# linyicheng1/keypoint_bench

Hardware: AMD Instinct MI355X
Metric: image-pairs/sec (extract+NMS+BF-match, 640x480, top_k=1000) (higher is better)
Workload: dtype f32

## Files before the change

include/kpb.h:

```cpp
#ifndef KPB_H
#define KPB_H

#include <stddef.h>
#include <stdint.h>

#ifdef __cplusplus
extern "C" {
#endif

#define KPB_VERSION 1

#define KPB_OK 0
#define KPB_E_INVALID (-1)
#define KPB_E_HIP (-2)
#define KPB_E_NOMEM (-3)
#define KPB_E_NEGATIVE (-4)
#define KPB_E_NOT_CONVERGED (-5)
#define KPB_E_WEIGHTS (-6)
#define KPB_E_UNSUPPORTED (-7)

#define KPB_MAX_NMS_DIST 16
#define KPB_MAX_TOPK 8192

typedef struct kpb_ctx kpb_ctx;
typedef struct kpb_net kpb_net;

typedef struct kpb_detect_params {
    int32_t nms_dist;
    float threshold;
    int32_t border_dist;
    int32_t top_k;
    float min_score;
} kpb_detect_params;

typedef struct kpb_match_params {
    double max_distance;
    int32_t cross_check;
} kpb_match_params;

int kpb_version(void);
const char* kpb_last_error(const kpb_ctx* ctx);

int kpb_ctx_create(int device, void* stream, kpb_ctx** out);
int kpb_ctx_set_stream(kpb_ctx* ctx, void* stream);
void kpb_ctx_destroy(kpb_ctx* ctx);
int kpb_sync(kpb_ctx* ctx);

#define KPB_OPT_COVIS_STORE_BYTES 1
int kpb_ctx_set_option(kpb_ctx* ctx, int option, int64_t value);

int kpb_prof_enable(kpb_ctx* ctx, int on);
int kpb_prof_report(kpb_ctx* ctx, char* buf, size_t cap);

int kpb_fast_nms(kpb_ctx* ctx, const float* score_dev, int batch, int H, int W, int nms_dist,
                 float* out_map_dev);

int kpb_detect(kpb_ctx* ctx, const float* score_dev, int batch, int H, int W,
               const kpb_detect_params* params, float* out_kps_dev, int32_t* out_idx_dev,
               int32_t* out_n_dev, int sync);
int kpb_detect_check(kpb_ctx* ctx);
int kpb_detect_counts(kpb_ctx* ctx, int32_t* out_n_host, int batch);

int kpb_sample(kpb_ctx* ctx, const float* desc_dev, int batch, int C, int Hd, int Wd, int64_t sb,
               int64_t sc, int64_t sh, int64_t sw, const float* pts_dev, int pts_cols, int max_n,
               const int32_t* n_dev, float* out_dev);

int kpb_match(kpb_ctx* ctx, const float* d0_dev, const float* d1_dev, int batch, int C, int max_n,
              int max_m, const int32_t* n_dev, const int32_t* m_dev, const kpb_match_params* params,
              int32_t* out_pairs_dev, double* out_dist_dev, int32_t* out_k_dev);

int kpb_match_counts(kpb_ctx* ctx, int32_t* out_k_host, int batch);

int kpb_gather_rows(kpb_ctx* ctx, const float* src_dev, int batch, int src_rows, int cols,
                    const int32_t* idx_dev, int idx_rows, int idx_stride, int idx_col,
                    const int32_t* k_dev, float* out_dev);

int kpb_warp_homography(kpb_ctx* ctx, const float* kps_dev, int batch, int max_n, int stride,
                        const int32_t* n_dev, const float* hmat_dev, const int32_t* wh_dev,
                        float* out_kps0_dev, float* out_kps01_dev, int32_t* out_ids_dev,
                        int32_t* out_n_dev);

int kpb_warp_se3(kpb_ctx* ctx, const float* kps_dev, int n, int stride, const float* depth0_dev, int H0, int W0,
                 const float* depth1_dev, int H1, int W1, const float* cam_dev, float* out_kps0_dev,
                 float* out_kps01_dev, int32_t* out_ids_dev, int32_t* out_ids_out_dev, int32_t* out_counts_dev);

int kpb_val_keypoints(kpb_ctx* ctx, const float* k0_dev, const float* k01_dev, const float* k1_dev,
                      const float* k10_dev, int batch, int max_m, int max_n, const int32_t* m_dev,
                      const int32_t* n_dev, const float* scale_dev, float th, int32_t* out_pairs_dev,
                      float* out_dist_dev, int cap, float* out_errors_dev, int32_t* out_counts_dev);

typedef struct kpb_lk_params {
    float distance;
    int32_t win_size, levels, iterations;
} kpb_lk_params;
int kpb_lk_track(kpb_ctx* ctx, const float* img1_dev, const float* img2_dev, int C, int H, int W,
                 const float* pts1_dev, const float* pts2_dev, int pts_stride, const float* unit_dev,
                 int n, const kpb_lk_params* params, float* out_pts_dev, float* out_err_dev);

int kpb_epipolar_error(kpb_ctx* ctx, const float* kps0_dev, int cols0, const float* kps1_dev, int cols1, int batch,
                       int max_k, const int32_t* k_dev, const float* fmat_dev, int W, int H, int mode1, float th,
                       float* out_err_dev, float* out_stats_dev);

typedef struct kpb_ransac_params {
    double threshold;
    double confidence;
    int32_t max_iters;
    int32_t refine;
} kpb_ransac_params;
int kpb_find_homography(kpb_ctx* ctx, const float* m0_dev, int cols0, const float* m1_dev, int cols1, int batch, int max_k,
                        const int32_t* k_dev, const float* scale_dev, const uint32_t* seed_dev, uint32_t seed,
                        const kpb_ransac_params* params, double* out_h_dev, uint8_t* out_mask_dev, int32_t* out_info_dev);

int kpb_find_essential(kpb_ctx* ctx, const float* m0_dev, int cols0, const float* m1_dev, int cols1, int batch, int max_k,
                       const int32_t* k_dev, const float* scale_dev, const double* cam_dev, int cam_f32, const double* thr_dev,
                       const uint32_t* seed_dev, uint32_t seed, double prob, int max_iters, double* out_e_dev,
                       uint8_t* out_mask_dev, int32_t* out_info_dev, double* out_pts_dev);
int kpb_recover_pose(kpb_ctx* ctx, const double* e_dev, const double* pts_dev, const uint8_t* mask_dev, int batch, int max_k,
                     const int32_t* k_dev, const int32_t* info_dev, double dist, double* out_rt_dev, uint8_t* out_mask_dev,
                     int32_t* out_good_dev);

int kpb_find_fundamental(kpb_ctx* ctx, const float* m0_dev, int cols0, const float* m1_dev, int cols1, int batch, int max_k,
                         const int32_t* k_dev, const float* scale_dev, const uint32_t* seed_dev, uint32_t seed,
                         const kpb_ransac_params* params, double* out_f_dev, uint8_t* out_mask_dev, int32_t* out_info_dev);

int kpb_preprocess(kpb_ctx* ctx, const uint8_t* src_dev, int batch, int Hs, int Ws, int swap_rb,
                   int Hd, int Wd, float* out_dev);

#define KPB_ARCH_ALIKE 1
#define KPB_ARCH_SUPERPOINT 2
#define KPB_ARCH_XFEAT 3
#define KPB_ARCH_DISK 4
#define KPB_ARCH_R2D2 6
int kpb_net_create(kpb_ctx* ctx, int arch, const void* blob, size_t len, kpb_net** out);
void kpb_net_destroy(kpb_net* net);
int kpb_net_desc_dim(const kpb_net* net);
int kpb_net_desc_div(const kpb_net* net);
int kpb_net_forward(kpb_net* net, const float* img_dev, int batch, int H, int W,
                    float* score_out_dev, float* desc_out_dev);
int kpb_net_desc_at(kpb_net* net, const float* pts_dev, int pts_cols, int max_n,
                    const int32_t* n_dev, float* out_dev);

#define KPB_ARCH_LIGHTGLUE 5
typedef struct kpb_lg kpb_lg;
typedef struct kpb_lg_params {
    float depth_confidence;
    float width_confidence;
    float filter_threshold;
    int32_t prune_min_kpts;
} kpb_lg_params;
int kpb_lg_create(kpb_ctx* ctx, const void* blob, size_t len, float desc_scale, kpb_lg** out);
void kpb_lg_destroy(kpb_lg* lg);
int kpb_lg_input_dim(const kpb_lg* lg);
int kpb_lg_set_attention(kpb_lg* lg, int mode);
int kpb_lg_match(kpb_lg* lg, const float* pts0_dev, const float* pts1_dev, const int32_t* n0_dev, const int32_t* n1_dev,
                 int batch, int max_k, const float* desc0_dev, const float* desc1_dev, int C, int Hd, int Wd,
                 int64_t sb, int64_t sc, int64_t sh, int64_t sw, int img_w, int img_h, const kpb_lg_params* params,
                 int32_t* out_pairs_dev, float* out_scores_dev, int32_t* out_k_dev, int32_t* out_stop_dev);

#ifdef __cplusplus
}
#endif
#endif
```

keypoint_bench_amd/_lib.py:

```python
import ctypes
import os

_HERE = os.path.dirname(os.path.abspath(__file__))
SO_PATH = os.environ.get("KPB_LIB_PATH") or os.path.join(_HERE, "libkpb.so")

c_int, c_float, c_double, c_void_p, c_int64, c_size_t = (ctypes.c_int, ctypes.c_float, ctypes.c_double,
                                                       ctypes.c_void_p, ctypes.c_int64, ctypes.c_size_t)


class DetectParams(ctypes.Structure):
    _fields_ = [("nms_dist", ctypes.c_int32), ("threshold", c_float), ("border_dist", ctypes.c_int32),
                ("top_k", ctypes.c_int32), ("min_score", c_float)]


class LgParams(ctypes.Structure):
    _fields_ = [("depth_confidence", c_float), ("width_confidence", c_float), ("filter_threshold", c_float),
                ("prune_min_kpts", ctypes.c_int32)]


class LkParams(ctypes.Structure):
    _fields_ = [("distance", ctypes.c_float), ("win_size", ctypes.c_int32), ("levels", ctypes.c_int32), ("iterations", ctypes.c_int32)]


class RansacParams(ctypes.Structure):
    _fields_ = [("threshold", ctypes.c_double), ("confidence", ctypes.c_double), ("max_iters", ctypes.c_int32), ("refine", ctypes.c_int32)]


class MatchParams(ctypes.Structure):
    _fields_ = [("max_distance", c_double), ("cross_check", ctypes.c_int32)]


SIGNATURES = {
    "kpb_version": (c_int, []),
    "kpb_last_error": (ctypes.c_char_p, [c_void_p]),
    "kpb_ctx_create": (c_int, [c_int, c_void_p, ctypes.POINTER(c_void_p)]),
    "kpb_ctx_set_stream": (c_int, [c_void_p, c_void_p]),
    "kpb_ctx_destroy": (None, [c_void_p]),
    "kpb_sync": (c_int, [c_void_p]),
    "kpb_ctx_set_option": (c_int, [c_void_p, c_int, c_int64]),
    "kpb_prof_enable": (c_int, [c_void_p, c_int]),
    "kpb_prof_report": (c_int, [c_void_p, ctypes.c_char_p, c_size_t]),
    "kpb_fast_nms": (c_int, [c_void_p, c_void_p, c_int, c_int, c_int, c_int, c_void_p]),
    "kpb_detect": (c_int, [c_void_p, c_void_p, c_int, c_int, c_int, ctypes.POINTER(DetectParams), c_void_p, c_void_p,
                           c_void_p, c_int]),
    "kpb_detect_check": (c_int, [c_void_p]),
    "kpb_detect_counts": (c_int, [c_void_p, c_void_p, c_int]),
    "kpb_match_counts": (c_int, [c_void_p, c_void_p, c_int]),
    "kpb_sample": (c_int, [c_void_p, c_void_p, c_int, c_int, c_int, c_int, c_int64, c_int64, c_int64, c_int64,
                           c_void_p, c_int, c_int, c_void_p, c_void_p]),
    "kpb_match": (c_int, [c_void_p, c_void_p, c_void_p, c_int, c_int, c_int, c_int, c_void_p, c_void_p,
                          ctypes.POINTER(MatchParams), c_void_p, c_void_p, c_void_p]),
    "kpb_gather_rows": (c_int, [c_void_p, c_void_p, c_int, c_int, c_int, c_void_p, c_int, c_int, c_int, c_void_p,
                                c_void_p]),
    "kpb_warp_homography": (c_int, [c_void_p, c_void_p, c_int, c_int, c_int, c_void_p, c_void_p, c_void_p, c_void_p,
                                    c_void_p, c_void_p, c_void_p]),
    "kpb_warp_se3": (c_int, [c_void_p, c_void_p, c_int, c_int, c_void_p, c_int, c_int, c_void_p, c_int, c_int, c_void_p, c_void_p,
                             c_void_p, c_void_p, c_void_p, c_void_p]),
    "kpb_val_keypoints": (c_int, [c_void_p, c_void_p, c_void_p, c_void_p, c_void_p, c_int, c_int, c_int, c_void_p, c_void_p,
                                  c_void_p, c_float, c_void_p, c_void_p, c_int, c_void_p, c_void_p]),
    "kpb_lk_track": (c_int, [c_void_p, c_void_p, c_void_p, c_int, c_int, c_int, c_void_p, c_void_p, c_int, c_void_p, c_int,
                             c_void_p, c_void_p, c_void_p]),
    "kpb_epipolar_error": (c_int, [c_void_p, c_void_p, c_int, c_void_p, c_int, c_int, c_int, c_void_p, c_void_p, c_int, c_int, c_int,
                                   c_float, c_void_p, c_void_p]),
    "kpb_find_homography": (c_int, [c_void_p, c_void_p, c_int, c_void_p, c_int, c_int, c_int, c_void_p, c_void_p, c_void_p, ctypes.c_uint32,
                                    ctypes.POINTER(RansacParams), c_void_p, c_void_p, c_void_p]),
    "kpb_find_fundamental": (c_int, [c_void_p, c_void_p, c_int, c_void_p, c_int, c_int, c_int, c_void_p, c_void_p, c_void_p, ctypes.c_uint32,
                                     ctypes.POINTER(RansacParams), c_void_p, c_void_p, c_void_p]),
    "kpb_find_essential": (c_int, [c_void_p, c_void_p, c_int, c_void_p, c_int, c_int, c_int, c_void_p, c_void_p, c_void_p, c_int, c_void_p, c_void_p,
                                   ctypes.c_uint32, c_double, c_int, c_void_p, c_void_p, c_void_p, c_void_p]),
    "kpb_recover_pose": (c_int, [c_void_p, c_void_p, c_void_p, c_void_p, c_int, c_int, c_void_p, c_void_p, c_double, c_void_p, c_void_p,
                                 c_void_p]),
    "kpb_preprocess": (c_int, [c_void_p, c_void_p, c_int, c_int, c_int, c_int, c_int, c_int, c_void_p]),
    "kpb_net_create": (c_int, [c_void_p, c_int, c_void_p, c_size_t, ctypes.POINTER(c_void_p)]),
    "kpb_net_destroy": (None, [c_void_p]),
    "kpb_net_desc_dim": (c_int, [c_void_p]),
    "kpb_net_desc_div": (c_int, [c_void_p]),
    "kpb_net_forward": (c_int, [c_void_p, c_void_p, c_int, c_int, c_int, c_void_p, c_void_p]),
    "kpb_net_desc_at": (c_int, [c_void_p, c_void_p, c_int, c_int, c_void_p, c_void_p]),
    "kpb_lg_create": (c_int, [c_void_p, c_void_p, c_size_t, c_float, ctypes.POINTER(c_void_p)]),
    "kpb_lg_destroy": (None, [c_void_p]),
    "kpb_lg_input_dim": (c_int, [c_void_p]),
    "kpb_lg_set_attention": (c_int, [c_void_p, c_int]),
    "kpb_lg_match": (c_int, [c_void_p, c_void_p, c_void_p, c_void_p, c_void_p, c_int, c_int, c_void_p, c_void_p, c_int, c_int, c_int,
                             c_int64, c_int64, c_int64, c_int64, c_int, c_int, ctypes.POINTER(LgParams), c_void_p, c_void_p,
                             c_void_p, c_void_p]),
}

_lib = None


class KpbError(RuntimeError):
    def __init__(self, code, msg):
        super().__init__("libkpb error %d: %s" % (code, msg))
        self.code = code


def load():
    global _lib
    if _lib is None:
        import torch
        if not os.path.exists(SO_PATH):
            raise RuntimeError("%s is missing: run `python -m keypoint_bench_amd.build` (hipcc, gfx950). "
                               "keypoint_bench_amd has no CPU fallback." % SO_PATH)
        L = ctypes.CDLL(SO_PATH)
        for name, (res, args) in SIGNATURES.items():
            fn = getattr(L, name)
            fn.restype = res
            fn.argtypes = args
        _lib = L
    return _lib


class Context:
    _instances = {}

    def __init__(self, device_index: int):
        import torch
        if not torch.cuda.is_available():
            raise RuntimeError("keypoint_bench_amd needs an MI355X (gfx950) GPU; none is visible and there is no "
                               "CPU fallback")
        self.lib = load()
        self.device_index = device_index
        stream = torch.cuda.current_stream(device_index).cuda_stream
        self.stream = stream
        h = c_void_p()
        rc = self.lib.kpb_ctx_create(device_index, c_void_p(stream), ctypes.byref(h))
        if rc != 0:
            raise KpbError(rc, self.lib.kpb_last_error(None).decode())
        self.handle = h

    @classmethod
    def get(cls, device):
        import torch
        idx = device.index if isinstance(device, torch.device) else int(device)
        if idx is None:
            idx = torch.cuda.current_device()
        if idx not in cls._instances:
            cls._instances[idx] = cls(idx)
        inst = cls._instances[idx]
        stream = torch.cuda.current_stream(idx).cuda_stream
        if stream != inst.stream:
            inst.check(inst.lib.kpb_ctx_set_stream(inst.handle, c_void_p(stream)))
            inst.stream = stream
        return inst

    def check(self, rc):
        if rc != 0:
            raise KpbError(rc, self.lib.kpb_last_error(self.handle).decode())

    def sync(self):
        self.check(self.lib.kpb_sync(self.handle))

    OPT_COVIS_STORE_BYTES = 1

    def set_option(self, option: int, value: int):
        self.check(self.lib.kpb_ctx_set_option(self.handle, int(option), int(value)))

    def prof_enable(self, on: bool):
        self.check(self.lib.kpb_prof_enable(self.handle, 1 if on else 0))

    def prof_report(self):
        buf = ctypes.create_string_buffer(1 << 16)
        self.check(self.lib.kpb_prof_report(self.handle, buf, len(buf)))
        out = {}
        for line in buf.value.decode().splitlines():
            name, calls, ms = line.split()
            out[name] = (int(calls), float(ms))
        return out


def ptr(t):
    return c_void_p(t.data_ptr()) if t is not None else c_void_p(0)
```

keypoint_bench_amd/csrc/alike.hip:

```cpp
#include "conv_mfma.h"

namespace {

typedef _Float16 h8v __attribute__((ext_vector_type(8)));
typedef _Float16 h2v __attribute__((ext_vector_type(2)));
typedef float f32x4v __attribute__((ext_vector_type(4)));

__device__ __forceinline__ float relu(float v);

__device__ __forceinline__ void split4(const float4 v, uint2& hi, uint2& lo) { cm_split4(v, hi, lo); }

__device__ __forceinline__ void amax_commit(float lane_max, float* slots, int slot, int lane)
{
    const float m = cm_wave_max(lane_max);
    if (lane == 0) slots[slot] = m;
}

__global__ __launch_bounds__(256) void amax_reduce(const float* slots, int n, unsigned* out)
{
    __shared__ float s[4];
    const int b = blockIdx.x, tid = threadIdx.x;
    float m = 0.0f;
    for (int i = tid; i < n; i += 256) {
        const float v = slots[(size_t)b * n + i];
        m = fmaxf(m, v < INFINITY ? v : 0.0f);
    }
    m = cm_wave_max(m);
    if ((tid & 63) == 0) s[tid >> 6] = m;
    __syncthreads();
    if (tid == 0) out[b] = __float_as_uint(fmaxf(fmaxf(s[0], s[1]), fmaxf(s[2], s[3])));
}

constexpr int B1_TH = 32, B1_TW = 32;

struct Block1Args {
    const float* img;
    float* x1;
    float* p1;
    const float* w1;
    const float* b1;
    const float* w2;
    const float* b2;
    int H, W;
};

__global__ __launch_bounds__(256) void alike_block1(Block1Args a)
{
    constexpr int IH = B1_TH + 4, IW = B1_TW + 4, MH = B1_TH + 2, MW = B1_TW + 2;
    __shared__ float in[3][IH][IW];
    __shared__ __attribute__((aligned(16))) float4 mid[2][MH][MW];
    const int tid = threadIdx.x, b = blockIdx.z;
    const int ty0 = blockIdx.y * B1_TH, tx0 = blockIdx.x * B1_TW;
    const size_t P = (size_t)a.H * a.W;
    const float* img = a.img + (size_t)b * 3 * P;
    {
        constexpr int N = 3 * IH * IW, PER = (N + 255) / 256;
        float buf[PER];
#pragma unroll
        for (int k = 0; k < PER; ++k) {
            const int i = tid + k * 256;
            const int c = i / (IH * IW), rem = i - c * IH * IW;
            const int y = rem / IW, x = rem - y * IW;
            const int gy = ty0 - 2 + y, gx = tx0 - 2 + x;
            buf[k] = 0.0f;
            if (i < N && gy >= 0 && gy < a.H && gx >= 0 && gx < a.W) buf[k] = img[c * P + (size_t)gy * a.W + gx];
        }
#pragma unroll
        for (int k = 0; k < PER; ++k) {
            const int i = tid + k * 256;
            if (i < N) (&in[0][0][0])[i] = buf[k];
        }
    }
    __syncthreads();
    for (int it = tid; it < MH * (MW / 2); it += 256) {
        const int my = it / (MW / 2), mx = (it - my * (MW / 2)) * 2;
        float acc[2][8];
#pragma unroll
        for (int q = 0; q < 2; ++q)
#pragma unroll
            for (int j = 0; j < 8; ++j) acc[q][j] = a.b1[j];
#pragma unroll 1
        for (int cky = 0; cky < 9; ++cky) {
                const int c = cky / 3, ky = cky - 3 * c;
                float v[4];
#pragma unroll
                for (int k = 0; k < 4; ++k) v[k] = in[c][my + ky][mx + k];
#pragma unroll
                for (int kx = 0; kx < 3; ++kx)
#pragma unroll
                    for (int j = 0; j < 8; ++j) {
                        const float w = a.w1[((c * 3 + ky) * 3 + kx) * 8 + j];
                        acc[0][j] = fmaf(v[kx], w, acc[0][j]);
                        acc[1][j] = fmaf(v[kx + 1], w, acc[1][j]);
                    }
            }
        const int gy = ty0 - 1 + my;
#pragma unroll
        for (int q = 0; q < 2; ++q) {
            const int gx = tx0 - 1 + mx + q;
            const bool inside = gy >= 0 && gy < a.H && gx >= 0 && gx < a.W;
            float4 lo = make_float4(0.f, 0.f, 0.f, 0.f), hi = lo;
            if (inside) {
                lo = make_float4(relu(acc[q][0]), relu(acc[q][1]), relu(acc[q][2]), relu(acc[q][3]));
                hi = make_float4(relu(acc[q][4]), relu(acc[q][5]), relu(acc[q][6]), relu(acc[q][7]));
            }
            mid[0][my][mx + q] = lo;
            mid[1][my][mx + q] = hi;
        }
    }
    __syncthreads();
    const int oy = tid >> 5, ox = tid & 31;
    float acc[4][8];
#pragma unroll
    for (int q = 0; q < 4; ++q)
#pragma unroll
        for (int j = 0; j < 8; ++j) acc[q][j] = a.b2[j];
#pragma unroll 1
    for (int tap = 0; tap < 9; ++tap) {
        const int ky = tap / 3, kx = tap - 3 * ky;
        float v[4][8];
#pragma unroll
        for (int q = 0; q < 4; ++q) {
            const float4 lo = mid[0][oy + 8 * q + ky][ox + kx];
            const float4 hi = mid[1][oy + 8 * q + ky][ox + kx];
            v[q][0] = lo.x; v[q][1] = lo.y; v[q][2] = lo.z; v[q][3] = lo.w;
            v[q][4] = hi.x; v[q][5] = hi.y; v[q][6] = hi.z; v[q][7] = hi.w;
        }
#pragma unroll
        for (int c = 0; c < 8; ++c)
#pragma unroll
            for (int j = 0; j < 8; ++j) {
                const float w = a.w2[(tap * 8 + c) * 8 + j];
#pragma unroll
                for (int q = 0; q < 4; ++q) acc[q][j] = fmaf(v[q][c], w, acc[q][j]);
            }
    }
    __syncthreads();
    float* stage = reinterpret_cast<float*>(&mid[0][0][0]);
#pragma unroll
    for (int q = 0; q < 4; ++q) {
        *reinterpret_cast<float4*>(stage + ((oy + 8 * q) * B1_TW + ox) * 8) = make_float4(relu(acc[q][0]), relu(acc[q][1]), relu(acc[q][2]), relu(acc[q][3]));
        *reinterpret_cast<float4*>(stage + ((oy + 8 * q) * B1_TW + ox) * 8 + 4) = make_float4(relu(acc[q][4]), relu(acc[q][5]), relu(acc[q][6]), relu(acc[q][7]));
    }
    __syncthreads();
#pragma unroll
    for (int k = 0; k < B1_TH * B1_TW * 8 / 4 / 256; ++k) {
        const int i = tid + k * 256;
        const int ry = i >> 6, rx4 = i & 63;
        const int gy = ty0 + ry, gx = tx0 + (rx4 >> 1);
        if (gy < a.H && gx < a.W)
            *reinterpret_cast<float4*>(a.x1 + ((size_t)b * P + (size_t)gy * a.W + tx0) * 8 + rx4 * 4) =
                *reinterpret_cast<const float4*>(stage + i * 4);
    }
    {
        const int H2 = a.H / 2, W2 = a.W / 2;
#pragma unroll
        for (int k = 0; k < (B1_TH / 2) * (B1_TW / 2) * 2 / 256; ++k) {
            const int i = tid + k * 256;
            const int q = i & 1, px = (i >> 1) & (B1_TW / 2 - 1), py = i >> 5;
            const float* s0 = stage + ((2 * py) * B1_TW + 2 * px) * 8 + 4 * q;
            const float4 v00 = *reinterpret_cast<const float4*>(s0), v01 = *reinterpret_cast<const float4*>(s0 + 8);
            const float4 v10 = *reinterpret_cast<const float4*>(s0 + B1_TW * 8), v11 = *reinterpret_cast<const float4*>(s0 + B1_TW * 8 + 8);
            const int gy = ty0 / 2 + py, gx = tx0 / 2 + px;
            if (gy < H2 && gx < W2)
                *reinterpret_cast<float4*>(a.p1 + (((size_t)b * H2 + gy) * W2 + gx) * 8 + 4 * q) =
                    make_float4(fmaxf(fmaxf(v00.x, v01.x), fmaxf(v10.x, v11.x)), fmaxf(fmaxf(v00.y, v01.y), fmaxf(v10.y, v11.y)),
                                fmaxf(fmaxf(v00.z, v01.z), fmaxf(v10.z, v11.z)), fmaxf(fmaxf(v00.w, v01.w), fmaxf(v10.w, v11.w)));
        }
    }
}

struct Block1HArgs {
    Block1Args b;
    const uint4* w1pk;
    const uint4* w2pk;
    float inv_ws1, inv_ws2;
    float l1_c1, bmax_c1;
    float* wmax_x1;
    int xcd_map;
};

constexpr int B1H_TH = 16;

__global__ __launch_bounds__(256) void alike_block1_h(Block1HArgs ha)
{
    const Block1Args& a = ha.b;
    constexpr int TH = B1H_TH, IH = TH + 4, IW = B1_TW + 4, MH = TH + 2, MW = B1_TW + 2, HW = MW / 2;
    constexpr int PLANE = MH * HW, REGION = 2 * PLANE, NIN = IH * IW;
    __shared__ __attribute__((aligned(16))) uint2 inh[2 * NIN + 2];
    __shared__ __attribute__((aligned(16))) uint4 mid[2 * REGION];
    const kpb_tile3 tile = kpb_xcd_tile(ha.xcd_map);
    const int tid = threadIdx.x, lane = tid & 63, wv = tid >> 6, b = tile.z;
    const int ty0 = tile.y * TH, tx0 = tile.x * B1_TW;
    const size_t P = (size_t)a.H * a.W;
    const float* img = a.img + (size_t)b * 3 * P;
    h8v c1hi[2], c1lo[2], bhi[3], blo[3];
#pragma unroll
    for (int kb = 0; kb < 2; ++kb) {
        c1hi[kb] = __builtin_bit_cast(h8v, ha.w1pk[(kb * 2 + 0) * 64 + lane]);
        c1lo[kb] = __builtin_bit_cast(h8v, ha.w1pk[(kb * 2 + 1) * 64 + lane]);
    }
#pragma unroll
    for (int kb = 0; kb < 3; ++kb) {
        bhi[kb] = __builtin_bit_cast(h8v, ha.w2pk[(kb * 2 + 0) * 64 + lane]);
        blo[kb] = __builtin_bit_cast(h8v, ha.w2pk[(kb * 2 + 1) * 64 + lane]);
    }
    const float4 bias1 = *reinterpret_cast<const float4*>(a.b1 + 4 * ((lane >> 4) & 1));
    const float4 bias2 = *reinterpret_cast<const float4*>(a.b2 + 4 * ((lane >> 4) & 1));
    __shared__ __attribute__((aligned(16))) float s_amax[4];
    int e_img;
    {
        constexpr int PER = (NIN + 255) / 256;
        float buf[PER][3];
        float am = 0.0f;
#pragma unroll
        for (int k = 0; k < PER; ++k) {
            const int i = tid + k * 256;
            const int y = i / IW, x = i - y * IW;
            const int gy = ty0 - 2 + y, gx = tx0 - 2 + x;
            const bool ok = i < NIN && gy >= 0 && gy < a.H && gx >= 0 && gx < a.W;
#pragma unroll
            for (int c = 0; c < 3; ++c) buf[k][c] = ok ? img[c * P + (size_t)gy * a.W + gx] : 0.0f;
            am = kpb_pmax(kpb_pmax(am, fabsf(buf[k][0])), kpb_pmax(fabsf(buf[k][1]), fabsf(buf[k][2])));
        }
        am = cm_wave_max(am);
        if (lane == 0) s_amax[wv] = am;
        __syncthreads();
        float4 q = *reinterpret_cast<const float4*>(s_amax);
        if (!(q.x < INFINITY && q.y < INFINITY && q.z < INFINITY && q.w < INFINITY)) {
            float fm = 0.0f;
#pragma unroll
            for (int k = 0; k < PER; ++k)
#pragma unroll
                for (int c = 0; c < 3; ++c) { const float v = fabsf(buf[k][c]); fm = fmaxf(fm, v < INFINITY ? v : 0.0f); }
            fm = cm_wave_max(fm);
            __syncthreads();
            if (lane == 0) s_amax[wv] = fm;
            __syncthreads();
            q = *reinterpret_cast<const float4*>(s_amax);
        }
        e_img = cm_exp_of(fmaxf(fmaxf(q.x, q.y), fmaxf(q.z, q.w)));
        const float sc = cm_scale_of(e_img);
#pragma unroll
        for (int k = 0; k < PER; ++k) {
            const int i = tid + k * 256;
            uint2 hi, lo;
            split4(make_float4(buf[k][0] * sc, buf[k][1] * sc, buf[k][2] * sc, 0.0f), hi, lo);
            if (i < NIN) { inh[i] = hi; inh[NIN + i] = lo; }
        }
        if (tid < 2) inh[2 * NIN + tid] = make_uint2(0u, 0u);
    }
    __syncthreads();
    const int e_mid = cm_exp_of(fmaf(__uint_as_float((unsigned)(e_img - 126 + 127) << 23), ha.l1_c1, ha.bmax_c1));
    const float un1 = ha.inv_ws1 * cm_unscale_of(e_img), sc_mid = cm_scale_of(e_mid), un2 = ha.inv_ws2 * cm_unscale_of(e_mid);
    const int pr = lane & 15, g = lane >> 4;
    const int sN = g >> 1, c0 = 4 * (g & 1);
    {
        const uint4* inq = reinterpret_cast<const uint4*>(inh);
        uint2* midh = reinterpret_cast<uint2*>(mid);
        static_assert((MH + 2) % 4 == 0 && MH % 4 == 2, "alike_block1_h: waves 2 and 3 take the two extra groups");
        {
            const int gxl = tx0 - 1 + 2 * pr + sN;
            const bool xin = gxl >= 0 && gxl < a.W;
            const float unm = xin ? un1 * sc_mid : 0.0f;
            const float4 bm = xin ? make_float4(bias1.x * sc_mid, bias1.y * sc_mid, bias1.z * sc_mid, bias1.w * sc_mid) : make_float4(0.f, 0.f, 0.f, 0.f);
            const bool has1 = g < 2;
            int at0 = (wv + (g >> 1)) * (IW / 2) + pr + (g & 1);
            int at1 = has1 ? (wv + 2) * (IW / 2) + pr + g : NIN;
            const int st1 = has1 ? 4 * (IW / 2) : 0, lo1 = has1 ? NIN / 2 : 0;
            int h8 = ((sN * PLANE + wv * HW + pr) << 1) + (g & 1);
#pragma unroll 1
            for (int y = wv; y < MH; y += 4, at0 += 4 * (IW / 2), at1 += st1, h8 += 8 * HW) {
                f32x4v acc = {0.f, 0.f, 0.f, 0.f};
                const h8v i0h = __builtin_bit_cast(h8v, inq[at0]), i0l = __builtin_bit_cast(h8v, inq[at0 + NIN / 2]);
                const h8v i1h = __builtin_bit_cast(h8v, inq[at1]), i1l = __builtin_bit_cast(h8v, inq[at1 + lo1]);
                acc = __builtin_amdgcn_mfma_f32_16x16x32_f16(c1hi[0], i0l, acc, 0, 0, 0);
                acc = __builtin_amdgcn_mfma_f32_16x16x32_f16(c1lo[0], i0h, acc, 0, 0, 0);
                acc = __builtin_amdgcn_mfma_f32_16x16x32_f16(c1hi[0], i0h, acc, 0, 0, 0);
                acc = __builtin_amdgcn_mfma_f32_16x16x32_f16(c1hi[1], i1l, acc, 0, 0, 0);
                acc = __builtin_amdgcn_mfma_f32_16x16x32_f16(c1lo[1], i1h, acc, 0, 0, 0);
                acc = __builtin_amdgcn_mfma_f32_16x16x32_f16(c1hi[1], i1h, acc, 0, 0, 0);
                const bool yin = (unsigned)(ty0 - 1 + y) < (unsigned)a.H;
                float4 v = make_float4(0.f, 0.f, 0.f, 0.f);
                if (yin) v = make_float4(relu(fmaf(acc[0], unm, bm.x)), relu(fmaf(acc[1], unm, bm.y)), relu(fmaf(acc[2], unm, bm.z)), relu(fmaf(acc[3], unm, bm.w)));
                uint2 hi, lo;
                split4(v, hi, lo);
                midh[h8] = hi;
                midh[h8 + 2 * REGION] = lo;
            }
        }
        if (wv >= 2) {
            const int gi = MH + wv - 2;
            const bool extra = true;
            const int y = extra ? 16 * (gi - MH) + pr : gi, pc = extra ? 16 : pr;
            const int my = min(y, MH - 1);
            f32x4v acc = {0.f, 0.f, 0.f, 0.f};
#pragma unroll
            for (int kb = 0; kb < 2; ++kb) {
                const int piece = 4 * kb + g;
                const int at = piece < 6 ? ((my + (piece >> 1)) * IW + 2 * pc + 2 * (piece & 1)) >> 1 : NIN;
                const h8v ihi = __builtin_bit_cast(h8v, inq[at]);
                const h8v ilo = __builtin_bit_cast(h8v, inq[piece < 6 ? at + NIN / 2 : NIN]);
                acc = __builtin_amdgcn_mfma_f32_16x16x32_f16(c1hi[kb], ilo, acc, 0, 0, 0);
                acc = __builtin_amdgcn_mfma_f32_16x16x32_f16(c1lo[kb], ihi, acc, 0, 0, 0);
                acc = __builtin_amdgcn_mfma_f32_16x16x32_f16(c1hi[kb], ihi, acc, 0, 0, 0);
            }
            const int gy = ty0 - 1 + y, gx = tx0 - 1 + 2 * pc + sN;
            const bool inside = gy >= 0 && gy < a.H && gx >= 0 && gx < a.W;
            float4 v = make_float4(relu(fmaf(acc[0], un1, bias1.x)) * sc_mid, relu(fmaf(acc[1], un1, bias1.y)) * sc_mid,
                                   relu(fmaf(acc[2], un1, bias1.z)) * sc_mid, relu(fmaf(acc[3], un1, bias1.w)) * sc_mid);
            if (!inside) v = make_float4(0.f, 0.f, 0.f, 0.f);
            uint2 hi, lo;
            split4(v, hi, lo);
            if (y < MH) {
                const int h8 = ((sN * PLANE + y * HW + pc) << 1) + (g & 1);
                midh[h8] = hi;
                midh[h8 + 2 * REGION] = lo;
            }
        }
    }
    __syncthreads();
    const int abase = (g & 1) * PLANE + pr + (g >> 1);
    const int H2 = a.H / 2, W2 = a.W / 2;
    float4 keep = make_float4(0.f, 0.f, 0.f, 0.f);
    float xmax = 0.0f;
    const int gx = tx0 + 2 * pr + sN;
#pragma unroll 1
    for (int rr = 0; rr < TH / 4; ++rr) {
        const int row = (TH / 4) * wv + rr;
        f32x4v acc = {0.f, 0.f, 0.f, 0.f};
#pragma unroll
        for (int kb = 0; kb < 3; ++kb) {
            const int at = abase + (row + kb) * HW;
            const h8v ihi = __builtin_bit_cast(h8v, mid[at]);
            const h8v ilo = __builtin_bit_cast(h8v, mid[REGION + at]);
            acc = __builtin_amdgcn_mfma_f32_16x16x32_f16(bhi[kb], ilo, acc, 0, 0, 0);
            acc = __builtin_amdgcn_mfma_f32_16x16x32_f16(blo[kb], ihi, acc, 0, 0, 0);
            acc = __builtin_amdgcn_mfma_f32_16x16x32_f16(bhi[kb], ihi, acc, 0, 0, 0);
        }
        const int gy = ty0 + row;
        const float4 v = make_float4(relu(fmaf(acc[0], un2, bias2.x)), relu(fmaf(acc[1], un2, bias2.y)), relu(fmaf(acc[2], un2, bias2.z)), relu(fmaf(acc[3], un2, bias2.w)));
        if (gy < a.H && gx < a.W) {
            {
                typedef float f4v __attribute__((ext_vector_type(4)));
                __builtin_nontemporal_store((f4v){v.x, v.y, v.z, v.w}, reinterpret_cast<f4v*>(a.x1 + ((size_t)b * P + (size_t)gy * a.W + gx) * 8 + c0));
            }
            xmax = kpb_pmax(kpb_pmax(xmax, kpb_pmax(v.x, v.y)), kpb_pmax(v.z, v.w));
        }
        if ((rr & 1) == 0) {
            keep = v;
        } else {
            float4 m = make_float4(kpb_pmax(keep.x, v.x), kpb_pmax(keep.y, v.y), kpb_pmax(keep.z, v.z), kpb_pmax(keep.w, v.w));
            m.x = kpb_pmax32(m.x); m.y = kpb_pmax32(m.y);
            m.z = kpb_pmax32(m.z); m.w = kpb_pmax32(m.w);
            const int py = gy >> 1, pxl = (tx0 >> 1) + pr;
            if (sN == 0 && py < H2 && pxl < W2) *reinterpret_cast<float4*>(a.p1 + (((size_t)b * H2 + py) * W2 + pxl) * 8 + c0) = m;
        }
    }
    amax_commit(xmax, ha.wmax_x1, ((b * gridDim.y + tile.y) * gridDim.x + tile.x) * 4 + wv, lane);
}

std::vector<float> pack_b1c1_pairs(const float* w, float scale)
{
    std::vector<uint16_t> hl((size_t)2 * 2 * 64 * 8, 0);
    for (int kb = 0; kb < 2; ++kb)
        for (int l = 0; l < 64; ++l)
            for (int j = 0; j < 8; ++j) {
                const int n = l & 15, g = l >> 4, s2 = n >> 3, co = n & 7, piece = 4 * kb + g;
                const int ky = piece >> 1, kx = 2 * (piece & 1) + (j >> 2) - s2, c = j & 3;
                const float v = (piece < 6 && c < 3 && kx >= 0 && kx <= 2) ? w[((size_t)co * 3 + c) * 9 + ky * 3 + kx] * scale : 0.0f;
                _Float16 hi = (_Float16)v;
                const _Float16 lo = (_Float16)(v - (float)hi);
                memcpy(&hl[(((size_t)kb * 2 + 0) * 64 + l) * 8 + j], &hi, 2);
                memcpy(&hl[(((size_t)kb * 2 + 1) * 64 + l) * 8 + j], &lo, 2);
            }
    std::vector<float> out(hl.size() / 2);
    memcpy(out.data(), hl.data(), hl.size() * 2);
    return out;
}

std::vector<float> pack_b1c2_pairs(const float* w, float scale)
{
    std::vector<uint16_t> hl((size_t)3 * 2 * 64 * 8, 0);
    for (int kb = 0; kb < 3; ++kb)
        for (int l = 0; l < 64; ++l)
            for (int j = 0; j < 8; ++j) {
                const int n = l & 15, g = l >> 4, s2 = n >> 3, co = n & 7, kx = g - s2;
                const float v = (kx >= 0 && kx <= 2) ? w[((size_t)co * 8 + j) * 9 + kb * 3 + kx] * scale : 0.0f;
                _Float16 hi = (_Float16)v;
                const _Float16 lo = (_Float16)(v - (float)hi);
                memcpy(&hl[(((size_t)kb * 2 + 0) * 64 + l) * 8 + j], &hi, 2);
                memcpy(&hl[(((size_t)kb * 2 + 1) * 64 + l) * 8 + j], &lo, 2);
            }
    std::vector<float> out(hl.size() / 2);
    memcpy(out.data(), hl.data(), hl.size() * 2);
    return out;
}

struct ConvArgs {
    const float* in;
    float* out;
    const float* w;
    const float* bias;
    const float* res_in;
    const float* ds_w;
    const float* ds_b;
    float* res_out;
    int H, W;
};

template <int CIN, int COUT, int POOL, bool RES, int CDS, int RPOOL, bool RELU, bool DSOUT = false, int TW = 32>
__global__ __launch_bounds__(256) void conv3x3_k(ConvArgs a)
{
    constexpr int G = COUT / 16, PG = 4 / G, RW = 64 / TW, TH = RW * PG, C4 = CIN / 4;
    constexpr int RP = TW == 16 ? 32 : TW + 2;
    constexpr int NPOS = (TH + 2) * RP, NPOSP = NPOS + ((4 - NPOS % 8) + 8) % 8;
    static_assert(COUT % 16 == 0 && (G == 1 || G == 2 || G == 4) && CIN % 4 == 0 && (TW == 16 || TW == 32), "channel config");
    __shared__ __attribute__((aligned(16))) float4 tile[C4 * NPOSP];
    const int tid = threadIdx.x, b = blockIdx.z;
    const int wv = __builtin_amdgcn_readfirstlane(tid >> 6), lane = tid & 63;
    const int cg = wv % G, pg = wv / G;
    const int ty0 = blockIdx.y * TH, tx0 = blockIdx.x * TW;
    const int Hi = a.H * POOL, Wi = a.W * POOL;
    const float* in = a.in + (size_t)b * Hi * Wi * CIN;

    for (int i = tid; i < (TH + 2) * (TW + 2) * C4; i += 256) {
        const int pos = i / C4, c4 = i - pos * C4;
        const int y = pos / (TW + 2), x = pos - y * (TW + 2);
        const int gy = ty0 - 1 + y, gx = tx0 - 1 + x;
        float4 v = make_float4(0.f, 0.f, 0.f, 0.f);
        if (gy >= 0 && gy < a.H && gx >= 0 && gx < a.W) {
            const float* p = in + ((size_t)(gy * POOL) * Wi + (size_t)gx * POOL) * CIN + c4 * 4;
            v = *reinterpret_cast<const float4*>(p);
#pragma unroll
            for (int dy = 0; dy < POOL; ++dy)
#pragma unroll
                for (int dx = 0; dx < POOL; ++dx) {
                    if (dy == 0 && dx == 0) continue;
                    const float4 q = *reinterpret_cast<const float4*>(p + ((size_t)dy * Wi + dx) * CIN);
                    v.x = fmaxf(v.x, q.x); v.y = fmaxf(v.y, q.y); v.z = fmaxf(v.z, q.z); v.w = fmaxf(v.w, q.w);
                }
        }
        tile[c4 * NPOSP + y * RP + x] = v;
    }
    __syncthreads();

    const int row = pg * RW + lane / TW, col = lane % TW;
    const int gy = ty0 + row, gx = tx0 + col;
    float acc[16];
    const float* bias = a.bias + cg * 16;
#pragma unroll
    for (int j = 0; j < 16; ++j) acc[j] = bias[j];
#pragma unroll
    for (int ky = 0; ky < 3; ++ky)
#pragma unroll
        for (int kx = 0; kx < 3; ++kx) {
            const float4* t = &tile[(row + ky) * RP + col + kx];
            const float* w = a.w + (size_t)((ky * 3 + kx) * CIN) * COUT + cg * 16;
#pragma unroll 2
            for (int c4 = 0; c4 < C4; ++c4) {
                const float4 v4 = t[c4 * NPOSP];
                const float v[4] = {v4.x, v4.y, v4.z, v4.w};
#pragma unroll
                for (int c = 0; c < 4; ++c)
#pragma unroll
                    for (int j = 0; j < 16; ++j) acc[j] = fmaf(v[c], w[(c4 * 4 + c) * COUT + j], acc[j]);
            }
        }
    if (gy >= a.H || gx >= a.W) return;
    if (DSOUT) {
        float ds[16];
        const float* db = a.ds_b + cg * 16;
#pragma unroll
        for (int j = 0; j < 16; ++j) ds[j] = db[j];
        const float4* t = &tile[(row + 1) * RP + col + 1];
        const float* dw = a.ds_w + cg * 16;
#pragma unroll 2
        for (int c4 = 0; c4 < C4; ++c4) {
            const float4 v4 = t[c4 * NPOSP];
            const float v[4] = {v4.x, v4.y, v4.z, v4.w};
#pragma unroll
            for (int c = 0; c < 4; ++c)
#pragma unroll
                for (int j = 0; j < 16; ++j) ds[j] = fmaf(v[c], dw[(c4 * 4 + c) * COUT + j], ds[j]);
        }
        float* ro = a.res_out + ((size_t)b * a.H * a.W + (size_t)gy * a.W + gx) * COUT + cg * 16;
#pragma unroll
        for (int q = 0; q < 4; ++q) *reinterpret_cast<float4*>(ro + 4 * q) = make_float4(ds[4 * q], ds[4 * q + 1], ds[4 * q + 2], ds[4 * q + 3]);
    }
    if (RES) {
        constexpr int D4 = CDS / 4;
        const int Hr = a.H * RPOOL, Wr = a.W * RPOOL;
        const float* p = a.res_in + ((size_t)b * Hr * Wr + (size_t)(gy * RPOOL) * Wr + (size_t)gx * RPOOL) * CDS;
        const float* dw = a.ds_w + cg * 16;
        const float* db = a.ds_b + cg * 16;
#pragma unroll
        for (int j = 0; j < 16; ++j) acc[j] += db[j];
        for (int c4 = 0; c4 < D4; ++c4) {
            float4 v4 = *reinterpret_cast<const float4*>(p + c4 * 4);
#pragma unroll
            for (int dy = 0; dy < RPOOL; ++dy)
#pragma unroll
                for (int dx = 0; dx < RPOOL; ++dx) {
                    if (dy == 0 && dx == 0) continue;
                    const float4 q = *reinterpret_cast<const float4*>(p + ((size_t)dy * Wr + dx) * CDS + c4 * 4);
                    v4.x = fmaxf(v4.x, q.x); v4.y = fmaxf(v4.y, q.y); v4.z = fmaxf(v4.z, q.z); v4.w = fmaxf(v4.w, q.w);
                }
            const float v[4] = {v4.x, v4.y, v4.z, v4.w};
#pragma unroll
            for (int c = 0; c < 4; ++c)
#pragma unroll
                for (int j = 0; j < 16; ++j) acc[j] = fmaf(v[c], dw[(c4 * 4 + c) * COUT + j], acc[j]);
        }
    }
    float* o = a.out + ((size_t)b * a.H * a.W + (size_t)gy * a.W + gx) * COUT + cg * 16;
#pragma unroll
    for (int q = 0; q < 4; ++q) {
        float4 v = make_float4(acc[4 * q], acc[4 * q + 1], acc[4 * q + 2], acc[4 * q + 3]);
        if (RELU) { v.x = relu(v.x); v.y = relu(v.y); v.z = relu(v.z); v.w = relu(v.w); }
        *reinterpret_cast<float4*>(o + 4 * q) = v;
    }
}

struct Block2Args {
    const float* p1;
    float* x2; float* a2; float* S2;
    float* p2;
    const uint4* w1pk;
    const uint4* w2pk;
    const uint4* wapk;
    const float* b1; const float* bsum; const float* wsg;
    int H, W;
    float inv_ws1, inv_ws2, inv_wsa, l1_c1, bmax_c1, l1_c2, l1_ds, bmax_sum;
    const unsigned* amax_x1;
    float* wmax_a2;
    int xcd_map;
};


__global__ __launch_bounds__(256, 4) void alike_block2(Block2Args a)
{
    constexpr int TH = 8, TW = 32, PH = TH + 4, PW = TW + 4, NP = PH * PW, MH = TH + 2, MW = TW + 2, NM = MH * MW;
    __shared__ __attribute__((aligned(16))) uint4 pin[2 * NP];
    __shared__ __attribute__((aligned(16))) uint4 mid[4 * NM];
    __shared__ __attribute__((aligned(16))) uint4 xs[4][2][2][16];
    __shared__ __attribute__((aligned(16))) uint4 zslot;
    const kpb_tile3 tile = kpb_xcd_tile(a.xcd_map);
    const int tid = threadIdx.x, lane = tid & 63, wv = tid >> 6, b = tile.z;
    const int ty0 = tile.y * TH, tx0 = tile.x * TW;
    const size_t P = (size_t)a.H * a.W;
    h8v w1h[3], w1l[3], w2h[5], w2l[5];
#pragma unroll
    for (int kb = 0; kb < 3; ++kb) { w1h[kb] = __builtin_bit_cast(h8v, a.w1pk[(kb * 2) * 64 + lane]); w1l[kb] = __builtin_bit_cast(h8v, a.w1pk[(kb * 2 + 1) * 64 + lane]); }
    const float4 b1v = *reinterpret_cast<const float4*>(a.b1 + 4 * (lane >> 4));
    const float4 bsum = *reinterpret_cast<const float4*>(a.bsum + 4 * (lane >> 4)), wsg = *reinterpret_cast<const float4*>(a.wsg + 4 * (lane >> 4));
    const float am_p = __uint_as_float(a.amax_x1[b]);
    const float bound1 = fmaf(am_p, a.l1_c1, a.bmax_c1);
    const int e1 = cm_exp_of(fmaxf(am_p, bound1));
    const int ex = cm_exp_of(fmaf(bound1, a.l1_c2, fmaf(am_p, a.l1_ds, a.bmax_sum)));
    const float sc1 = cm_scale_of(e1), un_c1s = a.inv_ws1, un_c2 = a.inv_ws2 * cm_unscale_of(e1);
    const bool edge = ty0 == 0 || tx0 == 0 || ty0 + TH >= a.H || tx0 + TW >= a.W;
    const float scx = cm_scale_of(ex), un_a = a.inv_wsa * cm_unscale_of(ex);
    {
        const float* in = a.p1 + (size_t)b * P * 8;
        constexpr int PER = (NP * 2 + 255) / 256;
        float4 ld[PER];
        unsigned okm = 0;
#pragma unroll
        for (int k = 0; k < PER; ++k) {
            const int i = min(tid + 256 * k, NP * 2 - 1);
            const int pos = i >> 1, q = i & 1;
            const int y = pos / PW, x = pos - y * PW;
            const int gy = ty0 - 2 + y, gx = tx0 - 2 + x;
            if (gy >= 0 && gy < a.H && gx >= 0 && gx < a.W) okm |= 1u << k;
            ld[k] = *reinterpret_cast<const float4*>(in + ((size_t)min(max(gy, 0), a.H - 1) * a.W + min(max(gx, 0), a.W - 1)) * 8 + 4 * q);
        }
#pragma unroll
        for (int k = 0; k < PER; ++k) {
            const int i = tid + 256 * k;
            const int pos = i >> 1, q = i & 1;
            float4 v = ((okm >> k) & 1u) ? ld[k] : make_float4(0.f, 0.f, 0.f, 0.f);
            v.x *= sc1; v.y *= sc1; v.z *= sc1; v.w *= sc1;
            uint2 hi, lo;
            split4(v, hi, lo);
            if (i < NP * 2) {
                uint2* d = reinterpret_cast<uint2*>(&pin[pos]) + q;
                d[0] = hi;
                d[2 * NP] = lo;
            }
        }
        if (tid == 0) zslot = make_uint4(0u, 0u, 0u, 0u);
    }
    __syncthreads();
    const int px = lane & 15, g = lane >> 4;
    const uint4* zp = &zslot;
    {
        float4 bias1 = b1v;
        bias1.x *= sc1; bias1.y *= sc1; bias1.z *= sc1; bias1.w *= sc1;
        uint2* midh = reinterpret_cast<uint2*>(mid);
        static_assert((2 * MH) % 4 == 0, "alike_block2: the regular conv1 groups split evenly over the four waves");
        {
            const int xl = 16 * (wv & 1) + px, y0 = wv >> 1;
            const int gxl = tx0 - 1 + xl;
            const bool xin = gxl >= 0 && gxl < a.W;
            const float unm = xin ? un_c1s : 0.0f;
            const float4 bm = xin ? bias1 : make_float4(0.f, 0.f, 0.f, 0.f);
            const bool has2 = 8 + g < 9;
            const uint4* q0 = &pin[(y0 + g / 3) * PW + xl + g % 3];
            const uint4* q1 = &pin[(y0 + (4 + g) / 3) * PW + xl + (4 + g) % 3];
            const uint4* q2 = has2 ? &pin[(y0 + 2) * PW + xl + 2] : zp;
            const int st2 = has2 ? 2 * PW : 0, lo2 = has2 ? NP : 0;
            int h8 = (((g >> 1) * NM + y0 * MW + xl) << 1) + (g & 1);
            constexpr int NIT = 2 * MH / 4;
            h8v i0h = __builtin_bit_cast(h8v, q0[0]), i0l = __builtin_bit_cast(h8v, q0[NP]);
            h8v i1h = __builtin_bit_cast(h8v, q1[0]), i1l = __builtin_bit_cast(h8v, q1[NP]);
            h8v i2h = __builtin_bit_cast(h8v, q2[0]), i2l = __builtin_bit_cast(h8v, q2[lo2]);
#pragma unroll 1
            for (int it = 0; it < NIT; ++it, h8 += 4 * MW) {
                f32x4v acc = {0.f, 0.f, 0.f, 0.f};
                __builtin_amdgcn_sched_barrier(0);
                acc = __builtin_amdgcn_mfma_f32_16x16x32_f16(w1h[0], i0l, acc, 0, 0, 0);
                acc = __builtin_amdgcn_mfma_f32_16x16x32_f16(w1l[0], i0h, acc, 0, 0, 0);
                acc = __builtin_amdgcn_mfma_f32_16x16x32_f16(w1h[0], i0h, acc, 0, 0, 0);
                acc = __builtin_amdgcn_mfma_f32_16x16x32_f16(w1h[1], i1l, acc, 0, 0, 0);
                acc = __builtin_amdgcn_mfma_f32_16x16x32_f16(w1l[1], i1h, acc, 0, 0, 0);
                acc = __builtin_amdgcn_mfma_f32_16x16x32_f16(w1h[1], i1h, acc, 0, 0, 0);
                acc = __builtin_amdgcn_mfma_f32_16x16x32_f16(w1h[2], i2l, acc, 0, 0, 0);
                acc = __builtin_amdgcn_mfma_f32_16x16x32_f16(w1l[2], i2h, acc, 0, 0, 0);
                acc = __builtin_amdgcn_mfma_f32_16x16x32_f16(w1h[2], i2h, acc, 0, 0, 0);
                __builtin_amdgcn_sched_barrier(0);
                if (it + 1 < NIT) {
                    q0 += 2 * PW; q1 += 2 * PW; q2 += st2;
                    i0h = __builtin_bit_cast(h8v, q0[0]); i0l = __builtin_bit_cast(h8v, q0[NP]);
                    i1h = __builtin_bit_cast(h8v, q1[0]); i1l = __builtin_bit_cast(h8v, q1[NP]);
                    i2h = __builtin_bit_cast(h8v, q2[0]); i2l = __builtin_bit_cast(h8v, q2[lo2]);
                }
                __builtin_amdgcn_sched_barrier(0);
                const bool yin = (unsigned)(ty0 - 1 + y0 + 2 * it) < (unsigned)a.H;
                float4 v = make_float4(0.f, 0.f, 0.f, 0.f);
                if (yin) v = make_float4(relu(fmaf(acc[0], unm, bm.x)), relu(fmaf(acc[1], unm, bm.y)), relu(fmaf(acc[2], unm, bm.z)), relu(fmaf(acc[3], unm, bm.w)));
                uint2 hi, lo;
                split4(v, hi, lo);
                midh[h8] = hi;
                midh[h8 + 4 * NM] = lo;
            }
        }
        if (wv < 2) {
            const int gi = 2 * MH + wv;
            const int k = 16 * (gi - 2 * MH) + px;
            const int y = k >> 1, x = 32 + (k & 1);
            const int my = min(y, MH - 1);
            f32x4v acc = {0.f, 0.f, 0.f, 0.f};
#pragma unroll
            for (int kb = 0; kb < 3; ++kb) {
                const int tap = 4 * kb + g;
                const bool has = tap < 9;
                const uint4* ph = has ? &pin[(my + tap / 3) * PW + x + tap % 3] : zp;
                const h8v ihi = __builtin_bit_cast(h8v, ph[0]);
                const h8v ilo = __builtin_bit_cast(h8v, has ? ph[NP] : zp[0]);
                acc = __builtin_amdgcn_mfma_f32_16x16x32_f16(w1h[kb], ilo, acc, 0, 0, 0);
                acc = __builtin_amdgcn_mfma_f32_16x16x32_f16(w1l[kb], ihi, acc, 0, 0, 0);
                acc = __builtin_amdgcn_mfma_f32_16x16x32_f16(w1h[kb], ihi, acc, 0, 0, 0);
            }
            const int gy = ty0 - 1 + y, gx = tx0 - 1 + x;
            const bool inside = gy >= 0 && gy < a.H && gx >= 0 && gx < a.W;
            float4 v = make_float4(relu(fmaf(acc[0], un_c1s, bias1.x)), relu(fmaf(acc[1], un_c1s, bias1.y)), relu(fmaf(acc[2], un_c1s, bias1.z)), relu(fmaf(acc[3], un_c1s, bias1.w)));
            if (edge && !inside) v = make_float4(0.f, 0.f, 0.f, 0.f);
            uint2 hi, lo;
            split4(v, hi, lo);
            if (y < MH) {
                const int h8 = (((g >> 1) * NM + y * MW + x) << 1) + (g & 1);
                midh[h8] = hi;
                midh[h8 + 4 * NM] = lo;
            }
        }
    }
    __builtin_amdgcn_sched_barrier(0);
#pragma unroll
    for (int kb = 0; kb < 5; ++kb) { w2h[kb] = __builtin_bit_cast(h8v, a.w2pk[(kb * 2) * 64 + lane]); w2l[kb] = __builtin_bit_cast(h8v, a.w2pk[(kb * 2 + 1) * 64 + lane]); }
    const h8v wah = __builtin_bit_cast(h8v, a.wapk[lane]), wal = __builtin_bit_cast(h8v, a.wapk[64 + lane]);
    __syncthreads();
    float* x2 = a.x2 + (size_t)b * P * 16;
    float* a2 = a.a2 + (size_t)b * P * 16;
    float* S2 = a.S2 + (size_t)b * P;
    uint2* xh = reinterpret_cast<uint2*>(&xs[wv][0][0][0]);
    float4 pm = make_float4(0.f, 0.f, 0.f, 0.f);
    float amx = 0.0f;
#pragma unroll 1
    for (int k4 = 0; k4 < 4; ++k4) {
        const int row = 4 * (wv >> 1) + k4, col0 = (wv & 1) * 16;
        const int mbase = row * MW + col0 + px;
        f32x4v acc = {0.f, 0.f, 0.f, 0.f};
        h8v ihi[5], ilo[5];
        auto fetch = [&](int kb) {
            const int kidx = 4 * kb + g;
            const uint4* ph;
            int lo_off;
            if (kidx < 18) { const int tap = kidx >> 1; ph = &mid[(kidx & 1) * NM + mbase + (tap / 3) * MW + tap % 3]; lo_off = 2 * NM; }
            else if (kidx == 18) { ph = &pin[(row + 2) * PW + col0 + px + 2]; lo_off = NP; }
            else { ph = zp; lo_off = 0; }
            ihi[kb] = __builtin_bit_cast(h8v, ph[0]);
            ilo[kb] = __builtin_bit_cast(h8v, ph[lo_off]);
        };
        auto mm = [&](int kb) {
            acc = __builtin_amdgcn_mfma_f32_16x16x32_f16(w2h[kb], ilo[kb], acc, 0, 0, 0);
            acc = __builtin_amdgcn_mfma_f32_16x16x32_f16(w2l[kb], ihi[kb], acc, 0, 0, 0);
            acc = __builtin_amdgcn_mfma_f32_16x16x32_f16(w2h[kb], ihi[kb], acc, 0, 0, 0);
        };
        fetch(0); fetch(1); fetch(2);
        __builtin_amdgcn_sched_barrier(0);
        mm(0); mm(1);
        __builtin_amdgcn_sched_barrier(0);
        fetch(3); fetch(4);
        __builtin_amdgcn_sched_barrier(0);
        mm(2);
        __builtin_amdgcn_sched_barrier(0);
        mm(3); mm(4);
        const int gy = ty0 + row, gx = tx0 + col0 + px;
        const bool ok = gy < a.H && gx < a.W;
        const float4 v = make_float4(relu(fmaf(acc[0], un_c2, bsum.x)), relu(fmaf(acc[1], un_c2, bsum.y)), relu(fmaf(acc[2], un_c2, bsum.z)), relu(fmaf(acc[3], un_c2, bsum.w)));
        if (ok && !a.p2) *reinterpret_cast<float4*>(x2 + ((size_t)gy * a.W + gx) * 16 + 4 * g) = v;
        pm = make_float4(kpb_pmax(pm.x, v.x), kpb_pmax(pm.y, v.y), kpb_pmax(pm.z, v.z), kpb_pmax(pm.w, v.w));
        {
            uint2 hi, lo;
            split4(make_float4(v.x * scx, v.y * scx, v.z * scx, v.w * scx), hi, lo);
            const int h8 = (((g >> 1) * 16 + px) << 1) + (g & 1);
            xh[h8] = hi;
            xh[h8 + 64] = lo;
        }
        f32x4v ag = {0.f, 0.f, 0.f, 0.f};
        {
            const uint4* ph = g < 2 ? &xs[wv][0][g][px] : zp;
            const h8v ihi = __builtin_bit_cast(h8v, ph[0]);
            const h8v ilo = __builtin_bit_cast(h8v, g < 2 ? ph[32] : zp[0]);
            ag = __builtin_amdgcn_mfma_f32_16x16x32_f16(wah, ilo, ag, 0, 0, 0);
            ag = __builtin_amdgcn_mfma_f32_16x16x32_f16(wal, ihi, ag, 0, 0, 0);
            ag = __builtin_amdgcn_mfma_f32_16x16x32_f16(wah, ihi, ag, 0, 0, 0);
        }
        const float4 av = make_float4(relu(ag[0] * un_a), relu(ag[1] * un_a), relu(ag[2] * un_a), relu(ag[3] * un_a));
        if (ok) {
            *reinterpret_cast<float4*>(a2 + ((size_t)gy * a.W + gx) * 16 + 4 * g) = av;
            amx = kpb_pmax(kpb_pmax(amx, kpb_pmax(av.x, av.y)), kpb_pmax(av.z, av.w));
        }
        float sg = fmaf(av.w, wsg.w, fmaf(av.z, wsg.z, fmaf(av.y, wsg.y, av.x * wsg.x)));
        sg = kpb_sum16(sg);
        sg = kpb_sum32(sg);
        if (g == 0 && ok) S2[(size_t)gy * a.W + gx] = sg;
    }
    if (a.p2) {
        pm.x = kpb_pmax(pm.x, kpb_xor1(pm.x)); pm.y = kpb_pmax(pm.y, kpb_xor1(pm.y));
        pm.z = kpb_pmax(pm.z, kpb_xor1(pm.z)); pm.w = kpb_pmax(pm.w, kpb_xor1(pm.w));
        pm.x = kpb_pmax(pm.x, kpb_xor2(pm.x)); pm.y = kpb_pmax(pm.y, kpb_xor2(pm.y));
        pm.z = kpb_pmax(pm.z, kpb_xor2(pm.z)); pm.w = kpb_pmax(pm.w, kpb_xor2(pm.w));
        const int gy = ty0 + 4 * (wv >> 1), gx = tx0 + (wv & 1) * 16 + px;
        if ((px & 3) == 0 && gy < a.H && gx < a.W)
            *reinterpret_cast<float4*>(a.p2 + (size_t)b * (P / 16) * 16 + ((size_t)(gy >> 2) * (a.W >> 2) + (gx >> 2)) * 16 + 4 * g) = pm;
    }
    amax_commit(amx, a.wmax_a2, ((b * gridDim.y + tile.y) * gridDim.x + tile.x) * 4 + wv, lane);
}

std::vector<float> pack_1x1_h16(const float* w, float scale)
{
    std::vector<uint16_t> hl((size_t)2 * 64 * 8, 0);
    for (int l = 0; l < 64; ++l)
        for (int j = 0; j < 8; ++j) {
            const int n = l & 15, g = l >> 4;
            const float v = g < 2 ? w[n * 16 + 8 * g + j] * scale : 0.0f;
            _Float16 hi = (_Float16)v;
            const _Float16 lo = (_Float16)(v - (float)hi);
            memcpy(&hl[((size_t)0 * 64 + l) * 8 + j], &hi, 2);
            memcpy(&hl[((size_t)1 * 64 + l) * 8 + j], &lo, 2);
        }
    std::vector<float> out(hl.size() / 2);
    memcpy(out.data(), hl.data(), hl.size() * 2);
    return out;
}

std::vector<float> pack_h16(const float* w, int CIN, const float* ds_w, float scale)
{
    const int OCT = CIN / 8, NK = 9 * OCT + (ds_w ? 1 : 0), KB = (NK + 3) / 4;
    std::vector<uint16_t> hl((size_t)KB * 2 * 64 * 8, 0);
    for (int kb = 0; kb < KB; ++kb)
        for (int l = 0; l < 64; ++l)
            for (int j = 0; j < 8; ++j) {
                const int n = l & 15, g = l >> 4, kidx = 4 * kb + g;
                float v = 0.0f;
                if (kidx < 9 * OCT) { const int tap = kidx / OCT, o = kidx - tap * OCT; v = w[((size_t)n * CIN + 8 * o + j) * 9 + tap]; }
                else if (ds_w && kidx == 9 * OCT) v = ds_w[n * 8 + j];
                v *= scale;
                _Float16 hi = (_Float16)v;
                const _Float16 lo = (_Float16)(v - (float)hi);
                memcpy(&hl[(((size_t)kb * 2 + 0) * 64 + l) * 8 + j], &hi, 2);
                memcpy(&hl[(((size_t)kb * 2 + 1) * 64 + l) * 8 + j], &lo, 2);
            }
    std::vector<float> out(hl.size() / 2);
    memcpy(out.data(), hl.data(), hl.size() * 2);
    return out;
}

constexpr int ESTRIDE = 68;

template <int CIN>
__device__ __forceinline__ void conv1x1_relu_body(const float* __restrict__ in, float* __restrict__ out, const float* __restrict__ w ,
                                                  const float* __restrict__ wsg , float* __restrict__ smap, size_t npix,
                                                  const float* __restrict__ wproj , float* __restrict__ E ,
                                                  const unsigned bx )
{
    const size_t p = (size_t)bx * 256 + threadIdx.x;
    const bool live = p < npix;
    constexpr bool STAGE_IN = CIN <= 32;
    constexpr int XP = CIN + 4;
    constexpr int WREG = STAGE_IN && 64 * XP > 16 * ESTRIDE ? 64 * XP : 16 * ESTRIDE;
    __shared__ __attribute__((aligned(16))) float wlds[4][WREG];
    float* wreg = wlds[threadIdx.x >> 6];
    float acc[16];
#pragma unroll
    for (int j = 0; j < 16; ++j) acc[j] = 0.0f;
    const float* x = in + (live ? p : 0) * CIN;
    if (STAGE_IN) {
        const int ln = threadIdx.x & 63;
        const size_t pw = (size_t)bx * 256 + (threadIdx.x >> 6) * 64;
        float4 ld[CIN / 4];
#pragma unroll
        for (int i = 0; i < CIN / 4; ++i) {
            const int j = ln + 64 * i, px = j / (CIN / 4);
            ld[i] = pw + px < npix ? *reinterpret_cast<const float4*>(in + pw * CIN + 4 * (size_t)j) : make_float4(0.f, 0.f, 0.f, 0.f);
        }
#pragma unroll
        for (int i = 0; i < CIN / 4; ++i) {
            const int j = ln + 64 * i, px = j / (CIN / 4), q = j - px * (CIN / 4);
            *reinterpret_cast<float4*>(wreg + px * XP + 4 * q) = ld[i];
        }
        x = wreg + ln * XP;
    }
#pragma unroll 2
    for (int c4 = 0; c4 < CIN / 4; ++c4) {
        const float4 v4 = *reinterpret_cast<const float4*>(x + c4 * 4);
        const float v[4] = {v4.x, v4.y, v4.z, v4.w};
#pragma unroll
        for (int c = 0; c < 4; ++c)
#pragma unroll
            for (int j = 0; j < 16; ++j) acc[j] = fmaf(v[c], w[(c4 * 4 + c) * 16 + j], acc[j]);
    }
    float sg = 0.0f;
#pragma unroll
    for (int j = 0; j < 16; ++j) { acc[j] = relu(acc[j]); sg = fmaf(acc[j], wsg[j], sg); }
    if (live) {
        float* o = out + p * 16;
#pragma unroll
        for (int q = 0; q < 4; ++q)
            *reinterpret_cast<float4*>(o + 4 * q) = make_float4(acc[4 * q], acc[4 * q + 1], acc[4 * q + 2], acc[4 * q + 3]);
        smap[p] = sg;
    }
    if (E) {
        const int lane = threadIdx.x & 63, wv = threadIdx.x >> 6;
        float* st = wreg;
        const size_t p0 = (size_t)bx * 256 + wv * 64;
        float4 r[17];
#pragma unroll
        for (int q = 0; q < 16; ++q) {
            r[q] = make_float4(0.f, 0.f, 0.f, 0.f);
#pragma unroll
            for (int c = 0; c < 16; ++c) {
                const float* wr = wproj + c * 64 + 4 * q;
                r[q].x = fmaf(acc[c], wr[0], r[q].x); r[q].y = fmaf(acc[c], wr[1], r[q].y);
                r[q].z = fmaf(acc[c], wr[2], r[q].z); r[q].w = fmaf(acc[c], wr[3], r[q].w);
            }
        }
        r[16] = make_float4(sg, 0.f, 0.f, 0.f);
        for (int g = 0; g < 4; ++g) {
            if ((lane >> 4) == g) {
                float* e = st + (lane & 15) * ESTRIDE;
#pragma unroll
                for (int q = 0; q < 17; ++q) *reinterpret_cast<float4*>(e + 4 * q) = r[q];
            }
            const size_t base = p0 + 16 * g;
            for (int j = lane; j < 16 * (ESTRIDE / 4); j += 64)
                if (base + j / (ESTRIDE / 4) < npix)
                    *reinterpret_cast<float4*>(E + base * ESTRIDE + 4 * j) = *reinterpret_cast<const float4*>(st + 4 * j);
        }
    }
}

template <int CIN>
__global__ __launch_bounds__(256) void conv1x1_relu(const float* __restrict__ in, float* __restrict__ out, const float* __restrict__ w,
                                                    const float* __restrict__ wsg, float* __restrict__ smap, size_t npix,
                                                    const float* __restrict__ wproj, float* __restrict__ E)
{
    conv1x1_relu_body<CIN>(in, out, w, wsg, smap, npix, wproj, E, blockIdx.x);
}

struct AggArgs { const float* in; float* out; const float* w; const float* wsg; float* smap; size_t npix; const float* wproj; float* E; };
__global__ __launch_bounds__(256) void conv1x1_relu_34(AggArgs a3, AggArgs a4, unsigned nb3)
{
    if (blockIdx.x < nb3) conv1x1_relu_body<32>(a3.in, a3.out, a3.w, a3.wsg, a3.smap, a3.npix, a3.wproj, a3.E, blockIdx.x);
    else conv1x1_relu_body<64>(a4.in, a4.out, a4.w, a4.wsg, a4.smap, a4.npix, a4.wproj, a4.E, blockIdx.x - nb3);
}

struct HeadArgs {
    const float* x1;
    const float* a2;
    const float* a3;
    const float* a4;
    const float* agg1;
    const float* whT;
    const float* wsc;
    float* score;
    float* desc;
    int H, W;
};


__device__ __forceinline__ void up8ch(const float* m, int Hs, int Ws, float sy, float sx, int y, int x, int c0, float* f)
{
    const float fy = sy * (float)y, fx = sx * (float)x;
    const int y0 = (int)fy, x0 = (int)fx;
    const int y1 = y0 + (y0 < Hs - 1 ? 1 : 0), x1 = x0 + (x0 < Ws - 1 ? 1 : 0);
    const float ly = fy - (float)y0, lx = fx - (float)x0, hy = 1.0f - ly, hx = 1.0f - lx;
    const float* p00 = m + ((size_t)y0 * Ws + x0) * 16 + c0;
    const float* p01 = m + ((size_t)y0 * Ws + x1) * 16 + c0;
    const float* p10 = m + ((size_t)y1 * Ws + x0) * 16 + c0;
    const float* p11 = m + ((size_t)y1 * Ws + x1) * 16 + c0;
#pragma unroll
    for (int q = 0; q < 2; ++q) {
        const float4 a = *reinterpret_cast<const float4*>(p00 + 4 * q), b = *reinterpret_cast<const float4*>(p01 + 4 * q);
        const float4 c = *reinterpret_cast<const float4*>(p10 + 4 * q), d = *reinterpret_cast<const float4*>(p11 + 4 * q);
        f[4 * q + 0] = hy * (hx * a.x + lx * b.x) + ly * (hx * c.x + lx * d.x);
        f[4 * q + 1] = hy * (hx * a.y + lx * b.y) + ly * (hx * c.y + lx * d.y);
        f[4 * q + 2] = hy * (hx * a.z + lx * b.z) + ly * (hx * c.z + lx * d.z);
        f[4 * q + 3] = hy * (hx * a.w + lx * b.w) + ly * (hx * c.w + lx * d.w);
    }
}

struct Up8Taps { float4 t[8]; float ly, lx; };
__device__ __forceinline__ void up8ch_lerp4(const Up8Taps& u, float* f, float sc)
{
    const float lx = u.lx, hx = 1.0f - lx, hy = (1.0f - u.ly) * sc, ly = u.ly * sc;
    const float w00 = hy * hx, w01 = hy * lx, w10 = ly * hx, w11 = ly * lx;
#pragma unroll
    for (int q = 0; q < 2; ++q) {
        const float4 a = u.t[4 * q], b = u.t[4 * q + 1], c = u.t[4 * q + 2], d = u.t[4 * q + 3];
        f[4 * q + 0] = fmaf(w11, d.x, fmaf(w10, c.x, fmaf(w01, b.x, w00 * a.x)));
        f[4 * q + 1] = fmaf(w11, d.y, fmaf(w10, c.y, fmaf(w01, b.y, w00 * a.y)));
        f[4 * q + 2] = fmaf(w11, d.z, fmaf(w10, c.z, fmaf(w01, b.z, w00 * a.z)));
        f[4 * q + 3] = fmaf(w11, d.w, fmaf(w10, c.w, fmaf(w01, b.w, w00 * a.w)));
    }
}

struct HybArgs {
    const float* x1;
    const float* a2;
    const float* E3;
    const float* E4;
    const float* agg1;
    const float* whT;
    const float* wsc;
    float* score; float* desc;
    int H, W;
    const unsigned* amax_x1; const unsigned* amax_a2;
    float l1_agg1;
    float ws_h, inv_ws_h;
    const uint4* a1h16;
    float inv_wa;
};

constexpr int SEG_TILES = 4;
constexpr int NT3 = 18, NT4 = 7;

template <int NT>
struct StripRegs { float4 u[(NT * (ESTRIDE / 4) + 63) / 64], d[(NT * (ESTRIDE / 4) + 63) / 64]; };

template <int NT>
__device__ __forceinline__ void strip_load(StripRegs<NT>& r, const float* E, int Hs, int Ws, float sy, int y, int tb, int lane)
{
    const float fy = sy * (float)y;
    const int y0 = (int)fy, y1 = y0 + (y0 < Hs - 1 ? 1 : 0);
#pragma unroll
    for (int k = 0; k < (NT * (ESTRIDE / 4) + 63) / 64; ++k) {
        const int i = min(lane + 64 * k, NT * (ESTRIDE / 4) - 1);
        const int t = i / (ESTRIDE / 4), q = i - t * (ESTRIDE / 4);
        const int xt = min(tb + t, Ws - 1);
        r.u[k] = *reinterpret_cast<const float4*>(E + ((size_t)y0 * Ws + xt) * ESTRIDE + 4 * q);
        r.d[k] = *reinterpret_cast<const float4*>(E + ((size_t)y1 * Ws + xt) * ESTRIDE + 4 * q);
    }
}

template <int NT>
__device__ __forceinline__ void strip_store(const StripRegs<NT>& r, float* V, int Hs, float sy, int y, int lane, float c)
{
    const float fy = sy * (float)y;
    const int y0 = (int)fy;
    const float ly = fy - (float)y0, hy = 1.0f - ly;
#pragma unroll
    for (int k = 0; k < (NT * (ESTRIDE / 4) + 63) / 64; ++k) {
        const int i = lane + 64 * k;
        const int t = i / (ESTRIDE / 4), q = i - t * (ESTRIDE / 4);
        const float cq = q < 16 ? c : 1.0f;
        const float4 u = r.u[k], d = r.d[k];
        float4 o;
        o.x = (hy * u.x + ly * d.x) * cq; o.y = (hy * u.y + ly * d.y) * cq; o.z = (hy * u.z + ly * d.z) * cq; o.w = (hy * u.w + ly * d.w) * cq;
        if (i < NT * (ESTRIDE / 4)) *reinterpret_cast<float4*>(V + t * ESTRIDE + 4 * q) = o;
    }
}

template <int NT>
__device__ __forceinline__ void build_strip(float* V, const float* E, int Hs, int Ws, float sy, int y, int tb, int lane, float c = 1.0f)
{
    StripRegs<NT> r;
    strip_load<NT>(r, E, Hs, Ws, sy, y, tb, lane);
    strip_store<NT>(r, V, Hs, sy, y, lane, c);
}

__global__ __launch_bounds__(256) void alike_head_hyb(HybArgs a)
{
    __shared__ __attribute__((aligned(16))) float Bl[16 * 2 * 64];
    __shared__ __attribute__((aligned(16))) float A1[2 * 8 * 8];
    __shared__ __attribute__((aligned(16))) float Ws[2 * 16];
    __shared__ __attribute__((aligned(16))) float V3[4][NT3 * ESTRIDE];
    __shared__ __attribute__((aligned(16))) float V4[4][NT4 * ESTRIDE];
    const int tid = threadIdx.x, lane = tid & 63, wv = tid >> 6;
    const int p = lane & 31, h = lane >> 5;
    const int b = blockIdx.y;
    for (int i = tid; i < 16 * 2 * 64; i += 256) {
        const int o = i & 63, hh = (i >> 6) & 1, s = i >> 7;
        Bl[i] = a.whT[(16 * (s >> 3) + 8 * hh + (s & 7)) * 64 + o];
    }
    if (tid < 128) { const int j = tid & 7, c = (tid >> 3) & 7, hh = tid >> 6; A1[tid] = a.agg1[c * 16 + 8 * hh + j]; }
    if (tid < 32) { const int s = tid & 15, hh = tid >> 4; Ws[tid] = a.wsc[16 * (s >> 3) + 8 * hh + (s & 7)]; }

    const int H2 = a.H / 2, W2 = a.W / 2, H8 = a.H / 8, W8 = a.W / 8, H32 = a.H / 32, W32 = a.W / 32;
    const float* a2 = a.a2 + (size_t)b * H2 * W2 * 16;
    const float* E3 = a.E3 + (size_t)b * H8 * W8 * ESTRIDE;
    const float* E4 = a.E4 + (size_t)b * H32 * W32 * ESTRIDE;
    const float sy2 = (float)(H2 - 1) / (float)(a.H - 1), sx2 = (float)(W2 - 1) / (float)(a.W - 1);
    const float sy8 = (float)(H8 - 1) / (float)(a.H - 1), sx8 = (float)(W8 - 1) / (float)(a.W - 1);
    const float sy32 = (float)(H32 - 1) / (float)(a.H - 1), sx32 = (float)(W32 - 1) / (float)(a.W - 1);
    const int tiles_per_row = a.W / 32, segs_per_row = (tiles_per_row + SEG_TILES - 1) / SEG_TILES;
    int y, xs;
    bool live;
    {
        const int w = blockIdx.x, band = w % segs_per_row, grp = w / segs_per_row;
        y = 4 * grp + wv; xs = band * (32 * SEG_TILES);
        live = y < a.H;
        if (!live) { y = 0; xs = 0; }
    }
    const int ntile = live ? min(SEG_TILES, tiles_per_row - xs / 32) : 0;
    const int tb3 = (int)(sx8 * (float)xs), tb4 = (int)(sx32 * (float)xs);
    if (live) {
        build_strip<NT3>(V3[wv], E3, H8, W8, sy8, y, tb3, lane);
        build_strip<NT4>(V4[wv], E4, H32, W32, sy32, y, tb4, lane);
    }
    __syncthreads();

    for (int t = 0; t < ntile; ++t) {
        const int x0 = xs + 32 * t, x = x0 + p;
        const size_t pix = (size_t)b * a.H * a.W + (size_t)y * a.W + x;
        int z = 0;
        asm volatile("" : "+v"(z));
        const float* Blz = Bl + z; const float* A1z = A1 + z; const float* Wsz = Ws + z;
        float f[16];
        {
            const float4 lo = *reinterpret_cast<const float4*>(a.x1 + pix * 8), hi = *reinterpret_cast<const float4*>(a.x1 + pix * 8 + 4);
            const float v[8] = {lo.x, lo.y, lo.z, lo.w, hi.x, hi.y, hi.z, hi.w};
#pragma unroll
            for (int j = 0; j < 8; ++j) f[j] = 0.0f;
#pragma unroll
            for (int c = 0; c < 8; ++c) {
                const float4 w0 = *reinterpret_cast<const float4*>(&A1z[(h * 8 + c) * 8]), w1 = *reinterpret_cast<const float4*>(&A1z[(h * 8 + c) * 8 + 4]);
                f[0] = fmaf(v[c], w0.x, f[0]); f[1] = fmaf(v[c], w0.y, f[1]); f[2] = fmaf(v[c], w0.z, f[2]); f[3] = fmaf(v[c], w0.w, f[3]);
                f[4] = fmaf(v[c], w1.x, f[4]); f[5] = fmaf(v[c], w1.y, f[5]); f[6] = fmaf(v[c], w1.z, f[6]); f[7] = fmaf(v[c], w1.w, f[7]);
            }
#pragma unroll
            for (int j = 0; j < 8; ++j) f[j] = relu(f[j]);
        }
        up8ch(a2, H2, W2, sy2, sx2, y, x, 8 * h, f + 8);

        const float fx3 = sx8 * (float)x, fx4 = sx32 * (float)x;
        const int rb3 = (int)(sx8 * (float)x0) - tb3, rb4 = (int)(sx32 * (float)x0) - tb4;
        const int t3 = (int)fx3 - tb3 - rb3, t4 = (int)fx4 - tb4 - rb4;
        const float lx3 = fx3 - (float)(int)fx3, lx4 = fx4 - (float)(int)fx4;
        const float* v3 = V3[wv] + rb3 * ESTRIDE;
        const float* v4 = V4[wv] + rb4 * ESTRIDE;

        float sc = 0.0f;
#pragma unroll
        for (int q = 0; q < 4; ++q) {
            const float4 w = *reinterpret_cast<const float4*>(&Wsz[h * 16 + 4 * q]);
            sc = fmaf(f[4 * q], w.x, sc); sc = fmaf(f[4 * q + 1], w.y, sc); sc = fmaf(f[4 * q + 2], w.z, sc); sc = fmaf(f[4 * q + 3], w.w, sc);
        }
        sc = kpb_sum32(sc);
        sc += (1.0f - lx3) * v3[t3 * ESTRIDE + 64] + lx3 * v3[(t3 + 1) * ESTRIDE + 64];
        sc += (1.0f - lx4) * v4[t4 * ESTRIDE + 64] + lx4 * v4[(t4 + 1) * ESTRIDE + 64];
        if (h == 0) a.score[pix] = __fdiv_rn(1.0f, 1.0f + expf(-sc));

        f32x16 acc0 = {0}, acc1 = {0};
#define HEAD_MFMA(fv, w0, w1)                                                       \
        acc0 = __builtin_amdgcn_mfma_f32_32x32x2f32(fv, w0, acc0, 0, 0, 0);            \
        acc1 = __builtin_amdgcn_mfma_f32_32x32x2f32(fv, w1, acc1, 0, 0, 0);
#pragma unroll
        for (int s = 0; s < 16; ++s) {
            const float b0 = Blz[(s * 2 + h) * 64 + p], b1 = Blz[(s * 2 + h) * 64 + 32 + p];
            HEAD_MFMA(f[s], b0, b1)
        }
#pragma unroll
        for (int s = 0; s < 3; ++s) {
            const int k = 2 * s + h;
            const float w = k == t3 ? 1.0f - lx3 : (k == t3 + 1 ? lx3 : 0.0f);
            const float b0 = v3[k * ESTRIDE + p], b1 = v3[k * ESTRIDE + 32 + p];
            HEAD_MFMA(w, b0, b1)
        }
#pragma unroll
        for (int s = 0; s < 2; ++s) {
            const int k = 2 * s + h;
            const float w = k == t4 ? 1.0f - lx4 : (k == t4 + 1 ? lx4 : 0.0f);
            const float b0 = v4[k * ESTRIDE + p], b1 = v4[k * ESTRIDE + 32 + p];
            HEAD_MFMA(w, b0, b1)
        }
#undef HEAD_MFMA
        float* d = a.desc + ((size_t)b * a.H * a.W + (size_t)y * a.W + x0) * 64;
#pragma unroll
        for (int r = 0; r < 16; ++r) {
            const int rowp = (r & 3) + 8 * (r >> 2) + 4 * h;
            __builtin_nontemporal_store(acc0[r], d + (size_t)rowp * 64 + p);
            __builtin_nontemporal_store(acc1[r], d + (size_t)rowp * 64 + 32 + p);
        }
    }
}

__device__ __forceinline__ void split8(const float* f, h8v& hi, h8v& lo)
{
    uint4 a, b;
    cm_split2(f[0], f[1], a.x, b.x); cm_split2(f[2], f[3], a.y, b.y);
    cm_split2(f[4], f[5], a.z, b.z); cm_split2(f[6], f[7], a.w, b.w);
    hi = __builtin_bit_cast(h8v, a); lo = __builtin_bit_cast(h8v, b);
}

constexpr int HP_TILES = 2, HP_BW = 32 * HP_TILES;
constexpr int HP_A2C = 34, HP_A2R = 8, HP_A2S = HP_A2C * 4;
constexpr int HP_NT3 = 10, HP_NT4 = 5, HP_ER = 4;
constexpr int HP_E3S = HP_NT3 * (ESTRIDE / 4), HP_E4S = HP_NT4 * (ESTRIDE / 4);
constexpr int HP_LA = 2;

inline bool hp_ring_rows_ok(int H, int Hs, int ring_rows)
{
    const float s = (float)(Hs - 1) / (float)(H - 1);
    for (int g = 0; g < H / 4; ++g) {
        const int lo = (int)(s * (float)(4 * g));
        const int last = std::min(H / 4 - 1, g + HP_LA);
        const int r = (int)(s * (float)(4 * last + 3));
        const int hi = r + (r < Hs - 1 ? 1 : 0);
        if (hi - lo + 1 > ring_rows) return false;
    }
    return true;
}

template <bool NT = false>
__device__ __forceinline__ void hp_dma16(const void* gsrc, const void* lds_wave_base)
{
    const unsigned m0v = __builtin_amdgcn_readfirstlane((unsigned)reinterpret_cast<uintptr_t>(lds_wave_base));
    unsigned keep;
    if (NT)
        asm volatile("s_mov_b32 %0, m0\n\ts_mov_b32 m0, %1\n\ts_nop 0\n\tglobal_load_lds_dwordx4 %2, off nt\n\ts_mov_b32 m0, %0"
                     : "=&s"(keep) : "s"(m0v), "v"(gsrc) : "memory");
    else
        asm volatile("s_mov_b32 %0, m0\n\ts_mov_b32 m0, %1\n\ts_nop 0\n\tglobal_load_lds_dwordx4 %2, off\n\ts_mov_b32 m0, %0"
                     : "=&s"(keep) : "s"(m0v), "v"(gsrc) : "memory");
}

__device__ __forceinline__ void hp_dma16s(const void* sbase, unsigned voff_bytes, const void* lds_wave_base)
{
    const unsigned m0v = __builtin_amdgcn_readfirstlane((unsigned)reinterpret_cast<uintptr_t>(lds_wave_base));
    const unsigned long long sb = (unsigned long long)reinterpret_cast<uintptr_t>(sbase);
    const unsigned lo = __builtin_amdgcn_readfirstlane((unsigned)sb), hi = __builtin_amdgcn_readfirstlane((unsigned)(sb >> 32));
    const unsigned long long sbu = ((unsigned long long)hi << 32) | lo;
    unsigned keep;
    asm volatile("s_mov_b32 %0, m0\n\ts_mov_b32 m0, %1\n\ts_nop 0\n\tglobal_load_lds_dwordx4 %2, %3\n\ts_mov_b32 m0, %0"
                 : "=&s"(keep) : "s"(m0v), "v"(voff_bytes), "s"(sbu) : "memory");
}

#ifdef KPB_STAMPS
__device__ unsigned long long kpb_stamp_buf[256 * 32];
__device__ unsigned kpb_stamp_slots;
#define KPB_STAMP(i) do { if (stamp_on) { unsigned long long t_; asm volatile("s_memtime %0\n\ts_waitcnt lgkmcnt(0)" : "=s"(t_) :: "memory"); \
                          if (lane == 0) kpb_stamp_buf[stamp_slot * 32 + (i)] = t_; } } while (0)
extern "C" __attribute__((visibility("default"))) int kpb_debug_head_stamps(unsigned long long* out_host, unsigned* slots_host)
{
    if (hipMemcpyFromSymbol(out_host, HIP_SYMBOL(kpb_stamp_buf), sizeof(unsigned long long) * 256 * 32) != hipSuccess) return -1;
    if (hipMemcpyFromSymbol(slots_host, HIP_SYMBOL(kpb_stamp_slots), sizeof(unsigned)) != hipSuccess) return -1;
    const unsigned zero = 0;
    return hipMemcpyToSymbol(HIP_SYMBOL(kpb_stamp_slots), &zero, sizeof(unsigned)) == hipSuccess ? 0 : -1;
}
#else
#define KPB_STAMP(i) do { } while (0)
#endif

__global__ __launch_bounds__(256, 3) void alike_head_f16p(HybArgs a, const uint4* __restrict__ wh16, int groups_per_wg)
{
    __shared__ __attribute__((aligned(16))) uint4 Bh[2][256];
    __shared__ __attribute__((aligned(16))) uint4 A1h[2][64];
    __shared__ __attribute__((aligned(16))) float Ws[2 * 16];
    __shared__ __attribute__((aligned(16))) float4 A2r[HP_A2R * HP_A2S];
    __shared__ __attribute__((aligned(16))) float E3r[HP_ER][HP_NT3 * ESTRIDE];
    __shared__ __attribute__((aligned(16))) float E4r[HP_ER][HP_NT4 * ESTRIDE];
    __shared__ __attribute__((aligned(16))) float4 X1r[4][2][64];
    const int tid = threadIdx.x, lane = tid & 63, wv = __builtin_amdgcn_readfirstlane(tid >> 6);
    const int p = lane & 31, h = lane >> 5;
    const int b = blockIdx.y;
    const int ef = cm_exp_of(fmaxf(__uint_as_float(a.amax_x1[b]) * a.l1_agg1, __uint_as_float(a.amax_a2[b])));
    auto uf = [](float v) { return __int_as_float(__builtin_amdgcn_readfirstlane(__float_as_int(v))); };
    auto ui = [](int v) { return __builtin_amdgcn_readfirstlane(v); };
    const float scf = uf(cm_scale_of(ef)), unf = cm_unscale_of(ef);
    const float cacc = uf(scf * a.ws_h), unacc = uf(unf * a.inv_ws_h);
    Bh[0][tid] = wh16[tid];
    Bh[1][tid] = wh16[256 + tid];
    if (tid < 128) A1h[tid >> 6][tid & 63] = a.a1h16[tid];
    if (tid < 32) { const int s = tid & 15, hh = tid >> 4; Ws[tid] = a.wsc[s < 8 ? (s < 4 ? s : s + 4) + 4 * hh : 16 + 8 * hh + (s & 7)] * unf; }
    const int ex1 = cm_exp_of(__uint_as_float(a.amax_x1[b]));
    const float sx1 = uf(cm_scale_of(ex1)), una1 = uf((cm_unscale_of(ex1) * scf) * a.inv_wa);

    const int H2 = a.H / 2, W2 = a.W / 2, H8 = a.H / 8, W8 = a.W / 8, H32 = a.H / 32, W32 = a.W / 32;
    const float* a2 = a.a2 + (size_t)b * H2 * W2 * 16;
    const float* E3 = a.E3 + (size_t)b * H8 * W8 * ESTRIDE;
    const float* E4 = a.E4 + (size_t)b * H32 * W32 * ESTRIDE;
    const float sy2 = uf((float)(H2 - 1) / (float)(a.H - 1)), sx2 = uf((float)(W2 - 1) / (float)(a.W - 1));
    const float sy8 = uf((float)(H8 - 1) / (float)(a.H - 1)), sx8 = uf((float)(W8 - 1) / (float)(a.W - 1));
    const float sy32 = uf((float)(H32 - 1) / (float)(a.H - 1)), sx32 = uf((float)(W32 - 1) / (float)(a.W - 1));
    const int tiles_per_row = a.W / 32, bands = (tiles_per_row + HP_TILES - 1) / HP_TILES, ngroups = a.H / 4;
    const int band = (int)blockIdx.x % bands, seg = (int)blockIdx.x / bands;
    const int g0 = seg * groups_per_wg, g1 = min(g0 + groups_per_wg, ngroups);
    const int xs = band * HP_BW;
    const int ntile = min(HP_TILES, tiles_per_row - xs / 32);
    const int c_lo = ui((int)(sx2 * (float)xs)), tb3 = ui((int)(sx8 * (float)xs)), tb4 = ui((int)(sx32 * (float)xs));

    auto hi_row = [&](float s, int G, int Hs) { const int r = ui((int)(s * (float)(4 * G + 3))); return r + (r < Hs - 1 ? 1 : 0); };
    int a2next = ui((int)(sy2 * (float)(4 * g0))), e3next = ui((int)(sy8 * (float)(4 * g0))), e4next = ui((int)(sy32 * (float)(4 * g0)));
    unsigned offA[(HP_A2S + 63) / 64], off3[(HP_E3S + 63) / 64], off4[(HP_E4S + 63) / 64];
#pragma unroll
    for (int j = 0; j < (HP_A2S + 63) / 64; ++j) {
        const int q = min(64 * j + lane, HP_A2S - 1), col = q >> 2, sl = (q & 3) ^ ((col >> 2) & 3), gc = min(c_lo + col, W2 - 1);
        offA[j] = (unsigned)(gc * 16 + 4 * sl) * 4u;
    }
#pragma unroll
    for (int j = 0; j < (HP_E3S + 63) / 64; ++j) {
        const int q = min(64 * j + lane, HP_E3S - 1), t = q / (ESTRIDE / 4), quad = q - t * (ESTRIDE / 4);
        off3[j] = (unsigned)(min(tb3 + t, W8 - 1) * ESTRIDE + 4 * quad) * 4u;
    }
#pragma unroll
    for (int j = 0; j < (HP_E4S + 63) / 64; ++j) {
        const int q = min(64 * j + lane, HP_E4S - 1), t = q / (ESTRIDE / 4), quad = q - t * (ESTRIDE / 4);
        off4[j] = (unsigned)(min(tb4 + t, W32 - 1) * ESTRIDE + 4 * quad) * 4u;
    }
    auto request = [&](const int G) {
        int u = 0;
        const int h2 = hi_row(sy2, G, H2), h3 = hi_row(sy8, G, H8), h4 = hi_row(sy32, G, H32);
        for (int r = a2next; r <= h2; ++r) {
            const float* row = a2 + (size_t)r * W2 * 16;
#pragma unroll
            for (int j = 0; j < (HP_A2S + 63) / 64; ++j, ++u)
                if ((u & 3) == wv && 64 * j + lane < HP_A2S) hp_dma16s(row, offA[j], &A2r[(r & (HP_A2R - 1)) * HP_A2S + 64 * j]);
        }
        a2next = max(a2next, h2 + 1);
        for (int r = e3next; r <= h3; ++r) {
            const float* row = E3 + (size_t)r * W8 * ESTRIDE;
#pragma unroll
            for (int j = 0; j < (HP_E3S + 63) / 64; ++j, ++u)
                if ((u & 3) == wv && 64 * j + lane < HP_E3S) hp_dma16s(row, off3[j], &E3r[r & (HP_ER - 1)][64 * j * 4]);
        }
        e3next = max(e3next, h3 + 1);
        for (int r = e4next; r <= h4; ++r) {
            const float* row = E4 + (size_t)r * W32 * ESTRIDE;
#pragma unroll
            for (int j = 0; j < (HP_E4S + 63) / 64; ++j, ++u)
                if ((u & 3) == wv && 64 * j + lane < HP_E4S) hp_dma16s(row, off4[j], &E4r[r & (HP_ER - 1)][64 * j * 4]);
        }
        e4next = max(e4next, h4 + 1);
    };

    f32x16 pend = {0}, pendB = {0};
    float* pend_d = nullptr;
    auto fetch = [&](int y, int t, int slot) {
        const size_t pix = (size_t)b * a.H * a.W + (size_t)y * a.W + (xs + 32 * t + p);
        hp_dma16<true>(a.x1 + pix * 8 + 4 * h, &X1r[wv][slot][0]);
    };
    if (g0 < g1) {
        fetch(4 * g0 + wv, 0, 0);
        if (ntile == 2) fetch(4 * g0 + wv, 1, 1);
        else if (g0 + 1 < g1) fetch(4 * (g0 + 1) + wv, 0, 1);
    }
    for (int G = g0; G < min(g0 + HP_LA, g1); ++G) request(G);
    int ktile = 0;
#ifdef KPB_STAMPS
    bool stamp_on = false;
    unsigned stamp_slot = 0;
    const bool stamp_wg = (blockIdx.x % 61) == 7 && (blockIdx.y % 16) == 3 && ntile == 2;
#endif

    int U3 = 0, D3 = 0, U4 = 0, D4 = 0;
    float hy3 = 0.f, ly3 = 0.f, hy4 = 0.f, ly4 = 0.f, hy3c = 0.f, ly3c = 0.f, hy4c = 0.f, ly4c = 0.f;

    float w3t[HP_TILES][3], w4t[HP_TILES][2], lx3t[HP_TILES], lx4t[HP_TILES];
#pragma unroll
    for (int t = 0; t < HP_TILES; ++t) {
        const int x0 = xs + 32 * t, x = x0 + p;
        const float fx3 = sx8 * (float)x, fx4 = sx32 * (float)x;
        const int rb3 = (int)(sx8 * (float)x0) - tb3, rb4 = (int)(sx32 * (float)x0) - tb4;
        const int t3 = (int)fx3 - tb3 - rb3, t4 = (int)fx4 - tb4 - rb4;
        lx3t[t] = fx3 - (float)(int)fx3; lx4t[t] = fx4 - (float)(int)fx4;
#pragma unroll
        for (int s = 0; s < 3; ++s) { const int kk = 2 * s + h; w3t[t][s] = kk == t3 ? 1.0f - lx3t[t] : (kk == t3 + 1 ? lx3t[t] : 0.0f); }
#pragma unroll
        for (int s = 0; s < 2; ++s) { const int kk = 2 * s + h; w4t[t][s] = kk == t4 ? 1.0f - lx4t[t] : (kk == t4 + 1 ? lx4t[t] : 0.0f); }
    }
    int xso = xs;
    auto body = [&](auto first_tag, const int y, const int t, const int ny, const int nt) {
        constexpr bool FIRST = decltype(first_tag)::value;
        const int x0 = xso + 32 * t, x = x0 + p;
        const size_t pix = (size_t)b * a.H * a.W + (size_t)y * a.W + x;
        if (ktile < 3) asm volatile("s_waitcnt vmcnt(0)" ::: "memory"); else asm volatile("s_waitcnt vmcnt(63)" ::: "memory");
        KPB_STAMP(4 + 8 * t);
        const int slot = ktile & 1;
        const float4 x1lo = X1r[wv][slot][p], x1hi = X1r[wv][slot][32 + p];
        asm volatile("s_waitcnt lgkmcnt(0)" ::: "memory");
        if (ny >= 0) fetch(ny, nt, slot);
        ++ktile;
        KPB_STAMP(5 + 8 * t);
        Up8Taps taps;
        {
            const float fy = sy2 * (float)y, fx = sx2 * (float)x;
            const int gy0 = (int)fy, gx0 = (int)fx;
            const int gy1 = gy0 + (gy0 < H2 - 1 ? 1 : 0);
            const int rx0 = gx0 - c_lo, rx1 = rx0 + (gx0 < W2 - 1 ? 1 : 0);
            taps.ly = fy - (float)gy0; taps.lx = fx - (float)gx0;
            const float4* r0 = A2r + (gy0 & (HP_A2R - 1)) * HP_A2S;
            const float4* r1 = A2r + (gy1 & (HP_A2R - 1)) * HP_A2S;
            const int s0 = (rx0 >> 2) & 3, s1 = (rx1 >> 2) & 3;
#pragma unroll
            for (int q = 0; q < 2; ++q) {
                taps.t[4 * q + 0] = r0[rx0 * 4 + ((2 * h + q) ^ s0)]; taps.t[4 * q + 1] = r0[rx1 * 4 + ((2 * h + q) ^ s1)];
                taps.t[4 * q + 2] = r1[rx0 * 4 + ((2 * h + q) ^ s0)]; taps.t[4 * q + 3] = r1[rx1 * 4 + ((2 * h + q) ^ s1)];
            }
        }
        if constexpr (!FIRST) {
#pragma unroll
            for (int r = 0; r < 16; ++r) __builtin_nontemporal_store(pend[r], pend_d + ((r & 3) + 8 * (r >> 2)) * 64);
        }
        KPB_STAMP(6 + 8 * t);
        int z = 0;
        asm volatile("" : "+v"(z));
        const uint4* Bhz = &Bh[0][0] + z; const uint4* A1z = &A1h[0][0] + z; const float* Wsz = Ws + z;
        float f[16];
        {
            const float xs[8] = {x1lo.x * sx1, x1lo.y * sx1, x1lo.z * sx1, x1lo.w * sx1, x1hi.x * sx1, x1hi.y * sx1, x1hi.z * sx1, x1hi.w * sx1};
            h8v xh, xl;
            split8(xs, xh, xl);
            const h8v wh = __builtin_bit_cast(h8v, A1z[lane]), wl = __builtin_bit_cast(h8v, A1z[64 + lane]);
            f32x16 aa = {0};
            aa = __builtin_amdgcn_mfma_f32_32x32x16_f16(wl, xh, aa, 0, 0, 0);
            aa = __builtin_amdgcn_mfma_f32_32x32x16_f16(wh, xl, aa, 0, 0, 0);
            aa = __builtin_amdgcn_mfma_f32_32x32x16_f16(wh, xh, aa, 0, 0, 0);
#pragma unroll
            for (int j = 0; j < 8; ++j) f[j] = relu(aa[j] * una1);
        }
        up8ch_lerp4(taps, f + 8, scf);

        const float fx3 = sx8 * (float)x, fx4 = sx32 * (float)x;
        const int rb3 = (int)(sx8 * (float)x0) - tb3, rb4 = (int)(sx32 * (float)x0) - tb4;
        const int t3 = (int)fx3 - tb3 - rb3, t4 = (int)fx4 - tb4 - rb4;
        const float lx3 = t == 0 ? lx3t[0] : lx3t[1], lx4 = t == 0 ? lx4t[0] : lx4t[1];
        const float *u3 = &E3r[0][0] + (U3 + rb3 * ESTRIDE + z), *d3 = &E3r[0][0] + (D3 + rb3 * ESTRIDE + z);
        const float *u4 = &E4r[0][0] + (U4 + rb4 * ESTRIDE + z), *d4 = &E4r[0][0] + (D4 + rb4 * ESTRIDE + z);
        auto e3 = [&](int k, int c) { return fmaf(ly3c, d3[k * ESTRIDE + c], hy3c * u3[k * ESTRIDE + c]); };
        auto e4 = [&](int k, int c) { return fmaf(ly4c, d4[k * ESTRIDE + c], hy4c * u4[k * ESTRIDE + c]); };

        float sc = 0.0f;
#pragma unroll
        for (int q = 0; q < 4; ++q) {
            const float4 w = *reinterpret_cast<const float4*>(&Wsz[h * 16 + 4 * q]);
            sc = fmaf(f[4 * q], w.x, sc); sc = fmaf(f[4 * q + 1], w.y, sc); sc = fmaf(f[4 * q + 2], w.z, sc); sc = fmaf(f[4 * q + 3], w.w, sc);
        }
        sc = kpb_sum32(sc);
        sc += (1.0f - lx3) * (hy3 * u3[t3 * ESTRIDE + 64] + ly3 * d3[t3 * ESTRIDE + 64]) + lx3 * (hy3 * u3[(t3 + 1) * ESTRIDE + 64] + ly3 * d3[(t3 + 1) * ESTRIDE + 64]);
        sc += (1.0f - lx4) * (hy4 * u4[t4 * ESTRIDE + 64] + ly4 * d4[t4 * ESTRIDE + 64]) + lx4 * (hy4 * u4[(t4 + 1) * ESTRIDE + 64] + ly4 * d4[(t4 + 1) * ESTRIDE + 64]);
        if (h == 0) a.score[pix] = __fdiv_rn(1.0f, 1.0f + expf(-sc));
        KPB_STAMP(7 + 8 * t);

        float* d = a.desc + ((size_t)b * a.H * a.W + (size_t)y * a.W + x0) * 64;
        f32x16 acc0 = {0}, acc1 = {0};
        h8v ahi[2], alo[2];
        split8(f, ahi[0], alo[0]);
        split8(f + 8, ahi[1], alo[1]);
        float w3[3], w4[2];
#pragma unroll
        for (int s = 0; s < 3; ++s) w3[s] = t == 0 ? w3t[0][s] : w3t[1][s];
#pragma unroll
        for (int s = 0; s < 2; ++s) w4[s] = t == 0 ? w4t[0][s] : w4t[1][s];
#pragma unroll
        for (int kb = 0; kb < 2; ++kb) {
            const h8v b0h = __builtin_bit_cast(h8v, Bhz[((kb * 2 + 0) * 2 + h) * 32 + p]), b0l = __builtin_bit_cast(h8v, Bhz[256 + ((kb * 2 + 0) * 2 + h) * 32 + p]);
            acc0 = __builtin_amdgcn_mfma_f32_32x32x16_f16(alo[kb], b0h, acc0, 0, 0, 0);
            acc0 = __builtin_amdgcn_mfma_f32_32x32x16_f16(ahi[kb], b0l, acc0, 0, 0, 0);
            acc0 = __builtin_amdgcn_mfma_f32_32x32x16_f16(ahi[kb], b0h, acc0, 0, 0, 0);
        }
#pragma unroll
        for (int s = 0; s < 3; ++s) acc0 = __builtin_amdgcn_mfma_f32_32x32x2f32(w3[s], e3(2 * s + h, p), acc0, 0, 0, 0);
#pragma unroll
        for (int s = 0; s < 2; ++s) acc0 = __builtin_amdgcn_mfma_f32_32x32x2f32(w4[s], e4(2 * s + h, p), acc0, 0, 0, 0);
        KPB_STAMP(8 + 8 * t);
        h8v b1h[2], b1l[2];
        float t3b[3], t4b[2];
#pragma unroll
        for (int kb = 0; kb < 2; ++kb) { b1h[kb] = __builtin_bit_cast(h8v, Bhz[((kb * 2 + 1) * 2 + h) * 32 + p]); b1l[kb] = __builtin_bit_cast(h8v, Bhz[256 + ((kb * 2 + 1) * 2 + h) * 32 + p]); }
#pragma unroll
        for (int s = 0; s < 3; ++s) t3b[s] = e3(2 * s + h, 32 + p);
#pragma unroll
        for (int s = 0; s < 2; ++s) t4b[s] = e4(2 * s + h, 32 + p);
        int r = 0;
        float* pb = pend_d + 4 * 64;
#define HP_ST1() { if constexpr (!FIRST) __builtin_nontemporal_store(pendB[r], pb + ((r & 3) + 8 * (r >> 2)) * 64); ++r; }
#define HP_ST2() { HP_ST1() HP_ST1() }
        acc1 = __builtin_amdgcn_mfma_f32_32x32x16_f16(alo[0], b1h[0], acc1, 0, 0, 0); HP_ST2()
        acc1 = __builtin_amdgcn_mfma_f32_32x32x16_f16(ahi[0], b1l[0], acc1, 0, 0, 0); HP_ST2()
        acc1 = __builtin_amdgcn_mfma_f32_32x32x16_f16(ahi[0], b1h[0], acc1, 0, 0, 0); HP_ST2()
        acc1 = __builtin_amdgcn_mfma_f32_32x32x16_f16(alo[1], b1h[1], acc1, 0, 0, 0); HP_ST2()
        acc1 = __builtin_amdgcn_mfma_f32_32x32x16_f16(ahi[1], b1l[1], acc1, 0, 0, 0); HP_ST2()
        acc1 = __builtin_amdgcn_mfma_f32_32x32x16_f16(ahi[1], b1h[1], acc1, 0, 0, 0); HP_ST2()
        acc1 = __builtin_amdgcn_mfma_f32_32x32x2f32(w3[0], t3b[0], acc1, 0, 0, 0); HP_ST2()
        acc1 = __builtin_amdgcn_mfma_f32_32x32x2f32(w3[1], t3b[1], acc1, 0, 0, 0); HP_ST2()
        acc1 = __builtin_amdgcn_mfma_f32_32x32x2f32(w3[2], t3b[2], acc1, 0, 0, 0);
        acc1 = __builtin_amdgcn_mfma_f32_32x32x2f32(w4[0], t4b[0], acc1, 0, 0, 0);
        acc1 = __builtin_amdgcn_mfma_f32_32x32x2f32(w4[1], t4b[1], acc1, 0, 0, 0);
#undef HP_ST2
#undef HP_ST1
        if constexpr (!FIRST) {
            __builtin_amdgcn_sched_group_barrier(0x008, 11, 0);
#pragma unroll
            for (int g = 0; g < 8; ++g) { __builtin_amdgcn_sched_group_barrier(0x008, 1, 0); __builtin_amdgcn_sched_group_barrier(0x040, 2, 0); }
            __builtin_amdgcn_sched_group_barrier(0x008, 3, 0);
        }
        KPB_STAMP(9 + 8 * t);
#pragma unroll
        for (int q = 0; q < 16; ++q) {
            const auto sw = __builtin_amdgcn_permlane32_swap(__float_as_uint(acc0[q] * unacc), __float_as_uint(acc1[q] * unacc), false, false);
            pend[q] = __uint_as_float(sw[0]); pendB[q] = __uint_as_float(sw[1]);
        }
        pend_d = d + lane;
        KPB_STAMP(10 + 8 * t);
    };

    for (int g = g0; g < g1; ++g) {
#ifdef KPB_STAMPS
        stamp_on = false;
        if (stamp_wg && g == g0 + 10) {
            unsigned sl = 0;
            if (lane == 0) sl = atomicAdd(&kpb_stamp_slots, 1u);
            stamp_slot = __builtin_amdgcn_readfirstlane(sl);
            stamp_on = stamp_slot < 256;
        }
#endif
        KPB_STAMP(0);
        if (ktile < 3) asm volatile("s_waitcnt vmcnt(0)" ::: "memory"); else asm volatile("s_waitcnt vmcnt(63)" ::: "memory");
        KPB_STAMP(1);
        __syncthreads();
        KPB_STAMP(2);
        if (g + HP_LA < g1) request(g + HP_LA);
        KPB_STAMP(3);
        const int y = 4 * g + wv;
        {
            const float fy3 = sy8 * (float)y, fy4 = sy32 * (float)y;
            const int y03 = (int)fy3, y04 = (int)fy4;
            const int y13 = y03 + (y03 < H8 - 1 ? 1 : 0), y14 = y04 + (y04 < H32 - 1 ? 1 : 0);
            ly3 = uf(fy3 - (float)y03); hy3 = uf(1.0f - ly3); ly4 = uf(fy4 - (float)y04); hy4 = uf(1.0f - ly4);
            hy3c = uf(hy3 * cacc); ly3c = uf(ly3 * cacc); hy4c = uf(hy4 * cacc); ly4c = uf(ly4 * cacc);
            U3 = ui((y03 & (HP_ER - 1)) * (HP_NT3 * ESTRIDE)); D3 = ui((y13 & (HP_ER - 1)) * (HP_NT3 * ESTRIDE));
            U4 = ui((y04 & (HP_ER - 1)) * (HP_NT4 * ESTRIDE)); D4 = ui((y14 & (HP_ER - 1)) * (HP_NT4 * ESTRIDE));
        }
        asm volatile("" : "+s"(xso));
        if (ntile == 2) {
            const int ny = g + 1 < g1 ? y + 4 : -1;
            if (g == g0) body(std::true_type{}, y, 0, ny, 0);
            else body(std::false_type{}, y, 0, ny, 0);
            body(std::false_type{}, y, 1, ny, 1);
        } else {
            const int ny = g + 2 < g1 ? y + 8 : -1;
            if (g == g0) body(std::true_type{}, y, 0, ny, 0);
            else body(std::false_type{}, y, 0, ny, 0);
        }
        KPB_STAMP(20);
    }
    if (g0 < g1) {
#pragma unroll
        for (int r = 0; r < 16; ++r) __builtin_nontemporal_store(pend[r], pend_d + ((r & 3) + 8 * (r >> 2)) * 64);
#pragma unroll
        for (int r = 0; r < 16; ++r) __builtin_nontemporal_store(pendB[r], pend_d + ((r & 3) + 8 * (r >> 2) + 4) * 64);
    }
}

struct LinArgs {
    const float* x1;
    const float* S2; const float* S3; const float* S4;
    const float* agg1;
    const float* wsc;
    float* score;
    int H, W;
    float sy2, sx2, sy3, sx3, sy4, sx4;
};

__device__ __forceinline__ float lerp_scalar(const float* m, int Hs, int Ws, float sy, float sx, int y, int x)
{
    const float fy = sy * (float)y, fx = sx * (float)x;
    const int y0 = (int)fy, x0 = (int)fx;
    const int y1 = y0 + (y0 < Hs - 1 ? 1 : 0), x1 = x0 + (x0 < Ws - 1 ? 1 : 0);
    const float ly = fy - (float)y0, lx = fx - (float)x0, hy = 1.0f - ly, hx = 1.0f - lx;
    return hy * (hx * m[(size_t)y0 * Ws + x0] + lx * m[(size_t)y0 * Ws + x1]) + ly * (hx * m[(size_t)y1 * Ws + x0] + lx * m[(size_t)y1 * Ws + x1]);
}

__global__ __launch_bounds__(256) void alike_score_lin(LinArgs a)
{
    const int b = blockIdx.y;
    const int pix = blockIdx.x * 256 + threadIdx.x;
    const int P = a.H * a.W;
    if (pix >= P) return;
    const int y = pix / a.W, x = pix - y * a.W;
    const float* px = a.x1 + ((size_t)b * P + pix) * 8;
    const float4 lo = *reinterpret_cast<const float4*>(px), hi = *reinterpret_cast<const float4*>(px + 4);
    const float v[8] = {lo.x, lo.y, lo.z, lo.w, hi.x, hi.y, hi.z, hi.w};
    typedef float f2v __attribute__((ext_vector_type(2)));
    f2v f[8];
#pragma unroll
    for (int j = 0; j < 8; ++j) f[j] = (f2v){0.0f, 0.0f};
#pragma unroll
    for (int c = 0; c < 8; ++c)
#pragma unroll
        for (int j = 0; j < 8; ++j) {
            const f2v w = {a.agg1[c * 16 + 2 * j], a.agg1[c * 16 + 2 * j + 1]};
            f[j] = __builtin_elementwise_fma((f2v){v[c], v[c]}, w, f[j]);
        }
    float sc = 0.0f;
#pragma unroll
    for (int j = 0; j < 16; ++j) sc = fmaf(relu(f[j >> 1][j & 1]), a.wsc[j], sc);
    const int H2 = a.H / 2, W2 = a.W / 2, H8 = a.H / 8, W8 = a.W / 8, H32 = a.H / 32, W32 = a.W / 32;
    sc += lerp_scalar(a.S2 + (size_t)b * H2 * W2, H2, W2, a.sy2, a.sx2, y, x);
    sc += lerp_scalar(a.S3 + (size_t)b * H8 * W8, H8, W8, a.sy3, a.sx3, y, x);
    sc += lerp_scalar(a.S4 + (size_t)b * H32 * W32, H32, W32, a.sy4, a.sx4, y, x);
    a.score[(size_t)b * P + pix] = __fdiv_rn(1.0f, 1.0f + expf(-sc));
}

struct DescAtArgs {
    HeadArgs h;
    const float* pts; const int* n; float* out;
    int pts_cols, max_n;
    int kpw;
};

constexpr int DA_PITCH = 68;
__global__ __launch_bounds__(256) void alike_desc_at(DescAtArgs a)
{
    __shared__ __attribute__((aligned(16))) float wh[64 * DA_PITCH];
    __shared__ __attribute__((aligned(16))) float fs[4][64];
    const int b = blockIdx.y, lane = threadIdx.x & 63, wv = threadIdx.x >> 6;
    const int n = a.n ? min(a.n[b], a.max_n) : a.max_n;
    const int i0 = (blockIdx.x * 4 + wv) * a.kpw;
    if (blockIdx.x * 4 * a.kpw >= n) return;
#pragma unroll
    for (int k = 0; k < 16; ++k) {
        const int i = threadIdx.x + 256 * k;
        wh[(i & 63) * DA_PITCH + (i >> 6)] = a.h.whT[i];
    }
    __syncthreads();
    const int H = a.h.H, W = a.h.W;
    const int g = lane >> 4, j = lane & 15;
    for (int kk = 0; kk < a.kpw; ++kk) {
        const int i = i0 + kk;
        if (i >= n) break;
        const float* pt = a.pts + ((size_t)b * a.max_n + i) * a.pts_cols;
        const float gx = (pt[0] - 0.5f) * 2.0f, gy = (pt[1] - 0.5f) * 2.0f;
        const float x = (gx + 1.0f) * ((float)(W - 1) / 2.0f), y = (gy + 1.0f) * ((float)(H - 1) / 2.0f);
        const float xw = floorf(x), yn = floorf(y);
        const float w = x - xw, e = 1.0f - w, nn = y - yn, s = 1.0f - nn;
        const float cw[4] = {s * e, s * w, nn * e, nn * w};
        const int x0 = (int)xw, y0 = (int)yn;
        float acc = 0.0f;
#pragma unroll
        for (int t = 0; t < 4; ++t) {
            const int tx = x0 + (t & 1), ty = y0 + (t >> 1);
            if (tx < 0 || tx >= W || ty < 0 || ty >= H) continue;
            float v;
            if (g == 0) {
                const float* px = a.h.x1 + ((size_t)b * H * W + (size_t)ty * W + tx) * 8;
                v = 0.0f;
#pragma unroll
                for (int c = 0; c < 8; ++c) v = fmaf(px[c], a.h.agg1[c * 16 + j], v);
                v = relu(v);
            } else {
                const int sh = g == 1 ? 2 : (g == 2 ? 8 : 32);
                const int Hs = H / sh, Ws = W / sh;
                const float* m = (g == 1 ? a.h.a2 : (g == 2 ? a.h.a3 : a.h.a4)) + (size_t)b * Hs * Ws * 16;
                const float fy = ((float)(Hs - 1) / (float)(H - 1)) * (float)ty, fx = ((float)(Ws - 1) / (float)(W - 1)) * (float)tx;
                const int sy0 = (int)fy, sx0 = (int)fx;
                const int sy1 = sy0 + (sy0 < Hs - 1 ? 1 : 0), sx1 = sx0 + (sx0 < Ws - 1 ? 1 : 0);
                const float ly = fy - (float)sy0, lx = fx - (float)sx0, hy = 1.0f - ly, hx = 1.0f - lx;
                v = hy * (hx * m[((size_t)sy0 * Ws + sx0) * 16 + j] + lx * m[((size_t)sy0 * Ws + sx1) * 16 + j]) +
                    ly * (hx * m[((size_t)sy1 * Ws + sx0) * 16 + j] + lx * m[((size_t)sy1 * Ws + sx1) * 16 + j]);
            }
            acc = fmaf(cw[t], v, acc);
        }
        __builtin_amdgcn_wave_barrier();
        fs[wv][lane] = acc;
        __builtin_amdgcn_wave_barrier();
        float o = 0.0f;
        const float4* wr = reinterpret_cast<const float4*>(wh + lane * DA_PITCH);
        const float4* fr = reinterpret_cast<const float4*>(fs[wv]);
#pragma unroll
        for (int c4 = 0; c4 < 16; ++c4) {
            const float4 f4 = fr[c4], w4 = wr[c4];
            o = fmaf(f4.x, w4.x, o); o = fmaf(f4.y, w4.y, o); o = fmaf(f4.z, w4.z, o); o = fmaf(f4.w, w4.w, o);
        }
        a.out[((size_t)b * a.max_n + i) * 64 + lane] = o;
    }
}

}

namespace {

struct AlikeNet : kpb_net {
    float *p1 = nullptr, *x1 = nullptr, *t2 = nullptr, *x2 = nullptr, *a2 = nullptr, *t3 = nullptr, *x3 = nullptr, *a3 = nullptr,
          *t4 = nullptr, *x4 = nullptr, *a4 = nullptr, *S2 = nullptr, *S3 = nullptr, *S4 = nullptr, *E3 = nullptr, *E4 = nullptr;
    std::map<std::string, float> k;
    HeadArgs head_args(float* score, float* desc)
    {
        HeadArgs h;
        h.x1 = x1; h.a2 = a2; h.a3 = a3; h.a4 = a4;
        h.agg1 = wp("agg1.w"); h.whT = wp("head.wT"); h.wsc = wp("head.ws");
        h.score = score; h.desc = desc; h.H = H; h.W = W;
        return h;
    }
    int forward(const float* img_dev, int batch, int H_, int W_, float* score_out_dev, float* desc_out_dev) override;
    int desc_at(const float* pts_dev, int pts_cols, int max_n, const int32_t* n_dev, float* out_dev) override;
};

void repack3x3(const float* w, int co, int ci, std::vector<float>& out)
{
    out.resize((size_t)9 * ci * co);
    for (int o = 0; o < co; ++o)
        for (int c = 0; c < ci; ++c)
            for (int k = 0; k < 9; ++k) out[((size_t)k * ci + c) * co + o] = w[((size_t)o * ci + c) * 9 + k];
}
void transpose(const float* w, int co, int ci, std::vector<float>& out)
{
    out.resize((size_t)ci * co);
    for (int o = 0; o < co; ++o)
        for (int c = 0; c < ci; ++c) out[(size_t)c * co + o] = w[(size_t)o * ci + c];
}
float l1_rows(const float* w, int co, int per)
{
    float m = 0.0f;
    for (int o = 0; o < co; ++o) {
        double s = 0.0;
        for (int i = 0; i < per; ++i) s += std::fabs((double)w[(size_t)o * per + i]);
        m = std::max(m, (float)(s * (1.0 + 1e-6)));
    }
    return m;
}
float max_abs(const float* b, int n)
{
    float m = 0.0f;
    for (int i = 0; i < n; ++i) m = std::max(m, std::fabs(b[i]));
    return m;
}

constexpr CmForm CM_C16{.ks = 3, .s = 1, .cc = 16, .ntb = 1, .mt = 2, .wn = 2}, CM_C32{.ks = 3, .s = 1, .cc = 32, .ntb = 1, .mt = 4, .wn = 2},
                 CM_C32_1T{.ks = 3, .s = 1, .cc = 32, .ntb = 1}, CM_C16_LAT{.ks = 3, .s = 1, .cc = 16, .wpre = true},
                 CM_C32_LAT{.ks = 3, .s = 1, .cc = 32, .ntb = 1, .wpre = true}, CM_P4_LAT{.ks = 3, .s = 1, .cc = 32, .pool_in = true, .ntb = 1, .pf = 4, .wpre = true};

template <int CIN, int COUT, int POOL, bool RES, int CDS, int RPOOL, bool DSOUT = false, int TW = 32>
void launch_conv(kpb_ctx* ctx, const char* name, hipStream_t st, const ConvArgs& a, int B)
{
    constexpr int G = COUT / 16, TH = (64 / TW) * (4 / G);
    KPB_LAUNCH(ctx, name, (conv3x3_k<CIN, COUT, POOL, RES, CDS, RPOOL, true, DSOUT, TW>), dim3(cdiv(a.W, TW), cdiv(a.H, TH), B), dim3(256), 0, st, a);
}

__global__ __launch_bounds__(256) void maxpool4_nhwc(const float* __restrict__ in, float* __restrict__ out, int Ho, int Wo, int C)
{
    const int C4 = C / 4;
    const size_t i = (size_t)blockIdx.x * 256 + threadIdx.x, b = blockIdx.y;
    if (i >= (size_t)Ho * Wo * C4) return;
    const int c = (int)(i % C4) * 4;
    const size_t pix = i / C4;
    const int y = (int)(pix / Wo), x = (int)(pix - (size_t)y * Wo);
    const float* s = in + ((b * 4 * Ho + 4 * y) * (size_t)(4 * Wo) + 4 * x) * C + c;
    float4 m = *reinterpret_cast<const float4*>(s);
#pragma unroll
    for (int py = 0; py < 4; ++py)
#pragma unroll
        for (int px = 0; px < 4; ++px) {
            if (py == 0 && px == 0) continue;
            const float4 v = *reinterpret_cast<const float4*>(s + ((size_t)py * 4 * Wo + px) * C);
            m.x = fmaxf(m.x, v.x); m.y = fmaxf(m.y, v.y); m.z = fmaxf(m.z, v.z); m.w = fmaxf(m.w, v.w);
        }
    *reinterpret_cast<float4*>(out + ((b * Ho + y) * (size_t)Wo + x) * C + c) = m;
}

int AlikeNet::forward(const float* img_dev, int batch, int H_, int W_, float* score_out_dev, float* desc_out_dev)
{
    if ((H_ % 32) || (W_ % 32))
        return kpb_fail(ctx, KPB_E_INVALID, "kpb_net_forward: ALIKE needs H and W multiples of 32 (got %dx%d)", H_, W_);
    const int H = H_, W = W_;
    const size_t P = (size_t)H * W, B = batch;
    const bool h16 = conv_mfma_use_h16();
    const size_t n_x1 = B * P * 8, n_2 = B * (P / 4) * 16, n_3 = B * (P / 64) * 32, n_a3 = B * (P / 64) * 16,
                 n_4 = B * (P / 1024) * 64, n_a4 = B * (P / 1024) * 16;
    const size_t n_s = B * (P / 4 + P / 64 + P / 1024) + 64;
    const size_t n_e = desc_out_dev ? B * (P / 64 + P / 1024) * ESTRIDE : 0;
    const size_t n_p1 = B * (P / 4) * 8;
    const int nw1 = cdiv(W, B1_TW) * cdiv(H, B1H_TH) * 4, nw2 = cdiv(W / 2, 32) * cdiv(H / 2, 8) * 4;
    const size_t n_rng = (2 * B + B * (nw1 + nw2) + 63) / 64 * 64;
    const size_t total = n_x1 + n_p1 + 3 * n_2 + 6 * n_3 + n_a3 + 5 * n_4 + n_4 / 2 + n_a4 + n_s + n_e + n_rng;
    if (int rc = kpb_reserve(ctx, act, total * sizeof(float))) return rc;
    float* p = static_cast<float*>(act.p);
    x1 = p; p += n_x1;
    p1 = p; p += n_p1;
    t2 = p; p += n_2; x2 = p; p += n_2; a2 = p; p += n_2;
    t3 = p; p += n_3; x3 = p; p += n_3; a3 = p; p += n_a3;
    t4 = p; p += n_4; x4 = p; p += n_4; a4 = p; p += n_a4;
    float* r3 = p; p += n_3;
    float* r4 = p; p += n_4;
    float* t3r3 = p; p += 2 * n_3;
    float* t4r4 = p; p += 2 * n_4;
    float* p2 = p; p += n_3 / 2;
    float* p3 = p; p += n_4 / 2;
    S2 = p; p += B * (P / 4); S3 = p; p += B * (P / 64); S4 = p; p += B * (P / 1024) + 64;
    E3 = E4 = nullptr;
    if (desc_out_dev) { E3 = p; p += B * (P / 64) * ESTRIDE; E4 = p; p += B * (P / 1024) * ESTRIDE; }
    unsigned* amax_x1 = reinterpret_cast<unsigned*>(p);
    unsigned* amax_a2 = amax_x1 + B;
    float* wmax_x1 = p + 2 * B;
    float* wmax_a2 = wmax_x1 + B * nw1;
    p += n_rng;
    this->B = batch; this->H = H; this->W = W;
    hipStream_t st = ctx->stream;

    Block1Args b1{img_dev, x1, p1, wp("b1c1.w"), wp("b1c1.b"), wp("b1c2.w"), wp("b1c2.b"), H, W};
    ConvArgs c;
    if (h16) {
        Block1HArgs hb{b1, reinterpret_cast<const uint4*>(wp("b1c1.pairs")), reinterpret_cast<const uint4*>(wp("b1c2.pairs")),
                       k.at("b1c1.inv_ws"), k.at("b1c2.inv_ws"), k.at("b1c1.l1"), k.at("b1c1.bmax"), wmax_x1, 0};
        KPB_LAUNCH(ctx, "alike_block1", alike_block1_h, dim3(cdiv(W, B1_TW), cdiv(H, B1H_TH), batch), dim3(256), 0, st, hb);
        KPB_LAUNCH(ctx, "amax_reduce", amax_reduce, dim3(batch), dim3(256), 0, st, wmax_x1, nw1, amax_x1);
        Block2Args b2{p1, x2, a2, S2, p2, reinterpret_cast<const uint4*>(wp("b2c1.h16")), reinterpret_cast<const uint4*>(wp("b2c2.h16")),
                      reinterpret_cast<const uint4*>(wp("agg2.h16")), wp("b2c1.b"), wp("b2c2.bsum"), wp("head.ws") + 16, H / 2, W / 2,
                      k.at("b2c1.inv_ws"), k.at("b2c2.inv_ws"), k.at("agg2.inv_ws"), k.at("b2c1.l1"), k.at("b2c1.bmax"), k.at("b2c2.l1"), k.at("b2ds.l1"),
                      k.at("b2c2.bsummax"), amax_x1, wmax_a2, 1};
        KPB_LAUNCH(ctx, "alike_block2", alike_block2, dim3(cdiv(W / 2, 32), cdiv(H / 2, 8), batch), dim3(256), 0, st, b2);
        KPB_LAUNCH(ctx, "amax_reduce", amax_reduce, dim3(batch), dim3(256), 0, st, wmax_a2, nw2, amax_a2);
        auto block_h = [&](const char* n1, const char* n2, const float* in, float* tr, float* xo, int cin, int cout, int Hi, int Wi, bool prepooled) {
            const std::string k1 = std::string(n1) + ".h", k2 = std::string(n2) + ".wp";
            ConvM m{.in = in, .out = tr, .wp = wp(k1.c_str()), .bias = wp((std::string(n1) + ".hb").c_str()), .Hi = prepooled ? Hi / 4 : Hi, .Wi = prepooled ? Wi / 4 : Wi,
                    .H = Hi / 4, .W = Wi / 4, .CIN = cin, .COUT = 2 * cout, .NCH = 1, .relu = 2, .nblk = cout / 32, .istride = cin, .ostride = 2 * cout,
                    .unscale = 1.0f / wscale.at(k1), .relu_nt = cout / 32};
            auto launch = [&](const char* n, const CmForm& f, const ConvM& cm) {
                return launch_conv_mfma_h<CM_C16, CM_C32, CM_C32_1T, CM_C16_LAT, CM_C32_LAT, CM_P4_LAT>(ctx, ("conv3x3_" + std::string(n)).c_str(), f, cm, batch); };
            if (batch < 16 && !prepooled) m.nblk = 2 * cout / 32;
            const CmForm f1 = !prepooled ? CM_P4_LAT : batch < 16 ? CM_C16_LAT : cin == 32 ? CM_C32 : CM_C16;
            if (int rc = launch(n1, f1, m)) return rc;
            const ConvM c2{.in = tr, .out = xo, .wp = wp(k2.c_str()), .bias = wp((std::string(n2) + ".bp").c_str()), .res = tr + cout, .Hi = Hi / 4, .Wi = Wi / 4,
                           .H = Hi / 4, .W = Wi / 4, .CIN = cout, .COUT = cout, .NCH = cout / 32, .nblk = batch < 16 ? cout / 32 : 1, .istride = 2 * cout,
                           .ostride = cout, .unscale = 1.0f / wscale.at(k2), .rstride = 2 * cout};
            return launch(n2, batch < 16 ? CM_C32_LAT : cout == 32 ? CM_C32_1T : CM_C32, c2);
        };
        if (int rc = block_h("b3c1", "b3c2", p2, t3r3, x3, 16, 32, H / 2, W / 2, true)) return rc;
        if (batch >= 16) {
            KPB_LAUNCH(ctx, "maxpool4_x3", maxpool4_nhwc, dim3((unsigned)(((size_t)(H / 32) * (W / 32) * 8 + 255) / 256), batch), dim3(256), 0, st, x3, p3, H / 32, W / 32, 32);
            if (int rc = block_h("b4c1", "b4c2", p3, t4r4, x4, 32, 64, H / 8, W / 8, true)) return rc;
        } else if (int rc = block_h("b4c1", "b4c2", x3, t4r4, x4, 32, 64, H / 8, W / 8, false))
            return rc;
    } else {
        auto conv2 = [&](const char* n, const float* in, float* out, const float* res, int h, int w, int c) {
            const std::string k = n;
            const ConvM m{.in = in, .out = out, .wp = wp((k + ".wp").c_str()), .bias = wp((k + ".bp").c_str()), .res = res, .Hi = h, .Wi = w, .H = h, .W = w,
                          .CIN = c, .COUT = c, .NCH = c / 32, .nblk = 1, .istride = c, .ostride = c};
            return launch_conv_mfma<CmForm{.ks = 3, .s = 1, .cc = 32, .ntb = 1}, CmForm{.ks = 3, .s = 1, .cc = 32}>(
                ctx, ("conv3x3_" + k).c_str(), CmForm{.ks = 3, .s = 1, .cc = 32, .ntb = c / 32}, m, batch);
        };
        KPB_LAUNCH(ctx, "alike_block1", alike_block1, dim3(cdiv(W, B1_TW), cdiv(H, B1_TH), batch), dim3(256), 0, st, b1);
        c = ConvArgs{p1, t2, wp("b2c1.w"), wp("b2c1.b"), nullptr, nullptr, nullptr, nullptr, H / 2, W / 2};
        launch_conv<8, 16, 1, false, 4, 1>(ctx, "conv3x3_b2c1", st, c, batch);
        c = ConvArgs{t2, x2, wp("b2c2.w"), wp("b2c2.b"), p1, wp("b2ds.w"), wp("b2ds.b"), nullptr, H / 2, W / 2};
        launch_conv<16, 16, 1, true, 8, 1>(ctx, "conv3x3_b2c2", st, c, batch);
        c = ConvArgs{x2, t3, wp("b3c1.w"), wp("b3c1.b"), nullptr, wp("b3ds.w"), wp("b3ds.b"), r3, H / 8, W / 8};
        launch_conv<16, 32, 4, false, 4, 1, true, 16>(ctx, "conv3x3_b3c1", st, c, batch);
        if (int rc = conv2("b3c2", t3, x3, r3, H / 8, W / 8, 32)) return rc;
        c = ConvArgs{x3, t4, wp("b4c1.w"), wp("b4c1.b"), nullptr, wp("b4ds.w"), wp("b4ds.b"), r4, H / 32, W / 32};
        launch_conv<32, 64, 4, false, 4, 1, true, 16>(ctx, "conv3x3_b4c1", st, c, batch);
        if (int rc = conv2("b4c2", t4, x4, r4, H / 32, W / 32, 64)) return rc;
        KPB_LAUNCH(ctx, "conv1x1_agg2", conv1x1_relu<16>, dim3((unsigned)((B * P / 4 + 255) / 256)), dim3(256), 0, st, x2, a2, wp("agg2.w"), wp("head.ws") + 16, S2, B * P / 4, nullptr, nullptr);
    }
    if (batch < 16) {
        const AggArgs g3{x3, a3, wp("agg3.w"), wp("head.ws") + 32, S3, B * P / 64, wp("head.wT") + 32 * 64, E3};
        const AggArgs g4{x4, a4, wp("agg4.w"), wp("head.ws") + 48, S4, B * P / 1024, wp("head.wT") + 48 * 64, E4};
        const unsigned nb3 = (unsigned)((B * P / 64 + 255) / 256), nb4 = (unsigned)((B * P / 1024 + 255) / 256);
        KPB_LAUNCH(ctx, "conv1x1_agg34", conv1x1_relu_34, dim3(nb3 + nb4), dim3(256), 0, st, g3, g4, nb3);
    } else {
        KPB_LAUNCH(ctx, "conv1x1_agg3", conv1x1_relu<32>, dim3((unsigned)((B * P / 64 + 255) / 256)), dim3(256), 0, st, x3, a3, wp("agg3.w"), wp("head.ws") + 32, S3, B * P / 64, wp("head.wT") + 32 * 64, E3);
        KPB_LAUNCH(ctx, "conv1x1_agg4", conv1x1_relu<64>, dim3((unsigned)((B * P / 1024 + 255) / 256)), dim3(256), 0, st, x4, a4, wp("agg4.w"), wp("head.ws") + 48, S4, B * P / 1024, wp("head.wT") + 48 * 64, E4);
    }
    if (desc_out_dev) {
        HybArgs hy{x1, a2, E3, E4, wp("agg1.w"), wp("head.wT"), wp("head.ws"), score_out_dev, desc_out_dev, H, W, amax_x1, amax_a2, 0.f, 1.f, 1.f, nullptr, 1.f};
        const int work4 = cdiv(H, 4) * cdiv(W / 32, SEG_TILES);
        if (h16) {
            hy.l1_agg1 = k.at("agg1.l1"); hy.inv_ws_h = k.at("head.inv_ws"); hy.ws_h = 1.0f / hy.inv_ws_h;
            hy.a1h16 = reinterpret_cast<const uint4*>(wp("agg1.h16")); hy.inv_wa = k.at("agg1.inv_wa");
            if (!hp_ring_rows_ok(H, H / 2, HP_A2R) || !hp_ring_rows_ok(H, H / 8, HP_ER) || !hp_ring_rows_ok(H, H / 32, HP_ER))
                return kpb_fail(ctx, KPB_E_UNSUPPORTED, "alike head: the LDS rings cannot hold the source rows of %d row groups at height %d", HP_LA + 1, H);
            const int bands_ = cdiv(W / 32, HP_TILES), groups_ = H / 4;
            const int hp = std::max(2, std::min(30, (int)(((long long)bands_ * groups_ * batch) / 1536)));
            KPB_LAUNCH(ctx, "alike_head_dense", alike_head_f16p, dim3(cdiv(W / 32, HP_TILES) * cdiv(H / 4, hp), batch), dim3(256), 0, st, hy,
                       reinterpret_cast<const uint4*>(wp("head.wh16")), hp);
        } else
            KPB_LAUNCH(ctx, "alike_head_dense", alike_head_hyb, dim3(work4, batch), dim3(256), 0, st, hy);
    } else {
        LinArgs la{x1, S2, S3, S4, wp("agg1.w"), wp("head.ws"), score_out_dev, H, W,
                   (float)(H / 2 - 1) / (float)(H - 1), (float)(W / 2 - 1) / (float)(W - 1), (float)(H / 8 - 1) / (float)(H - 1), (float)(W / 8 - 1) / (float)(W - 1),
                   (float)(H / 32 - 1) / (float)(H - 1), (float)(W / 32 - 1) / (float)(W - 1)};
        KPB_LAUNCH(ctx, "alike_head_score", alike_score_lin, dim3(cdiv(H * W, 256), batch), dim3(256), 0, st, la);
    }
    KPB_HIP(ctx, hipGetLastError());
    return KPB_OK;
}

int AlikeNet::desc_at(const float* pts_dev, int pts_cols, int max_n, const int32_t* n_dev, float* out_dev)
{
    if (B == 0) return kpb_fail(ctx, KPB_E_INVALID, "kpb_net_desc_at: no forward has run");
    const int kpw = (long long)B * max_n >= 32768 ? 8 : 1;
    DescAtArgs a{head_args(nullptr, nullptr), pts_dev, n_dev, out_dev, pts_cols, max_n, kpw};
    KPB_LAUNCH(ctx, "alike_desc_at", alike_desc_at, dim3(cdiv(max_n, 4 * kpw), B), dim3(256), 0, ctx->stream, a);
    KPB_HIP(ctx, hipGetLastError());
    return KPB_OK;
}

}

int alike_create(kpb_ctx* ctx, const KpbwBlob& bl, kpb_net** out)
{
    const uint32_t c1 = 8, c2 = 16, c3 = 32, c4 = 64, dim = 64;
    struct { const char* n; std::vector<uint32_t> d; } need[] = {
        {"b1c1.w", {c1, 3, 3, 3}}, {"b1c1.b", {c1}}, {"b1c2.w", {c1, c1, 3, 3}}, {"b1c2.b", {c1}},
        {"b2c1.w", {c2, c1, 3, 3}}, {"b2c1.b", {c2}}, {"b2c2.w", {c2, c2, 3, 3}}, {"b2c2.b", {c2}}, {"b2ds.w", {c2, c1}}, {"b2ds.b", {c2}},
        {"b3c1.w", {c3, c2, 3, 3}}, {"b3c1.b", {c3}}, {"b3c2.w", {c3, c3, 3, 3}}, {"b3c2.b", {c3}}, {"b3ds.w", {c3, c2}}, {"b3ds.b", {c3}},
        {"b4c1.w", {c4, c3, 3, 3}}, {"b4c1.b", {c4}}, {"b4c2.w", {c4, c4, 3, 3}}, {"b4c2.b", {c4}}, {"b4ds.w", {c4, c3}}, {"b4ds.b", {c4}},
        {"agg1.w", {dim / 4, c1}}, {"agg2.w", {dim / 4, c2}}, {"agg3.w", {dim / 4, c3}}, {"agg4.w", {dim / 4, c4}},
        {"head.w", {dim + 1, dim}}};
    for (auto& nd : need)
        if (!bl.get(nd.n, nd.d))
            return kpb_fail(ctx, KPB_E_WEIGHTS, "kpb_net_create: tensor %s missing or not ALIKE-t shaped "
                            "(this build supports c1..c4 = 8,16,32,64, dim = 64)", nd.n);
    AlikeNet* net = new AlikeNet();
    net->ctx = ctx; net->arch = KPB_ARCH_ALIKE; net->dim = dim; net->desc_div = 1;
    WeightStage ws;
    std::vector<float> tmp;
    {
        const float* w = bl.get("b1c1.w", {c1, 3, 3, 3});
        tmp.assign(27 * 8, 0.f);
        for (int o = 0; o < 8; ++o) for (int k = 0; k < 27; ++k) tmp[k * 8 + o] = w[o * 27 + k];
        ws.put("b1c1.w", tmp);
        ws.put_raw("b1c1.b", bl.get("b1c1.b", {c1}), 8);
        repack3x3(bl.get("b1c2.w", {c1, c1, 3, 3}), 8, 8, tmp); ws.put("b1c2.w", tmp);
        {
            const float* w1 = bl.get("b1c1.w", {c1, 3, 3, 3});
            const float* w2 = bl.get("b1c2.w", {c1, c1, 3, 3});
            const float s1 = weight_scale_h(w1, 8 * 27), s2 = weight_scale_h(w2, 8 * 72);
            ws.put("b1c1.pairs", pack_b1c1_pairs(w1, s1));
            ws.put("b1c2.pairs", pack_b1c2_pairs(w2, s2));
            net->k["b1c1.inv_ws"] = 1.0f / s1; net->k["b1c2.inv_ws"] = 1.0f / s2;
            net->k["b1c1.l1"] = l1_rows(w1, 8, 27); net->k["b1c1.bmax"] = max_abs(bl.get("b1c1.b", {c1}), 8);
        }
        ws.put_raw("b1c2.b", bl.get("b1c2.b", {c1}), 8);
    }
    const uint32_t ch[5] = {0, c1, c2, c3, c4};
    for (int i = 2; i <= 4; ++i) {
        char nm[16];
        const uint32_t ci = ch[i - 1], co = ch[i];
        snprintf(nm, 16, "b%dc1.w", i); repack3x3(bl.get(nm, {co, ci, 3, 3}), co, ci, tmp); ws.put(nm, tmp);
        snprintf(nm, 16, "b%dc1.b", i); ws.put_raw(nm, bl.get(nm, {co}), co);
        snprintf(nm, 16, "b%dc2.w", i); repack3x3(bl.get(nm, {co, co, 3, 3}), co, co, tmp); ws.put(nm, tmp);
        snprintf(nm, 16, "b%dc2.b", i); ws.put_raw(nm, bl.get(nm, {co}), co);
        snprintf(nm, 16, "b%dds.w", i); transpose(bl.get(nm, {co, ci}), co, ci, tmp); ws.put(nm, tmp);
        snprintf(nm, 16, "b%dds.b", i); ws.put_raw(nm, bl.get(nm, {co}), co);
    }
    {
        const float* w1 = bl.get("b2c1.w", {c2, c1, 3, 3});
        const float* w2 = bl.get("b2c2.w", {c2, c2, 3, 3});
        const float* wd = bl.get("b2ds.w", {c2, c1});
        const float* wa = bl.get("agg2.w", {dim / 4, c2});
        const float s1 = weight_scale_h(w1, 16 * 72);
        const float s2 = std::min(weight_scale_h(w2, 16 * 144), weight_scale_h(wd, 16 * 8));
        const float sa = weight_scale_h(wa, 16 * 16);
        ws.put("b2c1.h16", pack_h16(w1, 8, nullptr, s1));
        ws.put("b2c2.h16", pack_h16(w2, 16, wd, s2));
        const float* b2 = bl.get("b2c2.b", {c2});
        const float* bd = bl.get("b2ds.b", {c2});
        tmp.assign(16, 0.f);
        for (int i = 0; i < 16; ++i) tmp[i] = b2[i] + bd[i];
        ws.put("b2c2.bsum", tmp);
        ws.put("agg2.h16", pack_1x1_h16(wa, sa));
        net->k["b2c1.inv_ws"] = 1.0f / s1; net->k["b2c2.inv_ws"] = 1.0f / s2; net->k["agg2.inv_ws"] = 1.0f / sa;
        net->k["b2c1.l1"] = l1_rows(w1, 16, 72); net->k["b2c1.bmax"] = max_abs(bl.get("b2c1.b", {c2}), 16);
        net->k["b2c2.l1"] = l1_rows(w2, 16, 144); net->k["b2ds.l1"] = l1_rows(wd, 16, 8); net->k["b2c2.bsummax"] = max_abs(tmp.data(), 16);
        net->k["agg1.l1"] = l1_rows(bl.get("agg1.w", {dim / 4, c1}), 16, 8);
    }
    auto put_mfma = [&](const char* name, const float* w, int cout, int cin, int ntb) {
        if (conv_mfma_use_h16()) {
            const float sc = weight_scale_h(w, (size_t)cout * cin * 9);
            ws.put(name, pack_mfma_h(w, cout, cin, 3, 32, ntb, sc));
            ws.wscale[name] = sc;
        } else {
            ws.put(name, pack_mfma(w, cout, cin, 3, 32, ntb));
        }
    };
    auto put_c1ds = [&](const char* name, const float* w1, const float* b1, const float* wds, const float* bds, int cout, int cin) {
        std::vector<float> w((size_t)2 * cout * cin * 9, 0.0f), bb(2 * cout);
        memcpy(w.data(), w1, (size_t)cout * cin * 9 * sizeof(float));
        for (int o = 0; o < cout; ++o) {
            for (int c = 0; c < cin; ++c) w[((size_t)(cout + o) * cin + c) * 9 + 4] = wds[(size_t)o * cin + c];
            bb[o] = b1[o]; bb[cout + o] = bds[o];
        }
        const float sc = weight_scale_h(w.data(), w.size());
        const std::string k = std::string(name) + ".h";
        ws.put(k, pack_mfma_h(w.data(), 2 * cout, cin, 3, cin == 16 ? 16 : 32, 2, sc));
        ws.wscale[k] = sc;
        ws.put(std::string(name) + ".hb", bb);
    };
    if (conv_mfma_use_h16()) {
        put_c1ds("b3c1", bl.get("b3c1.w", {c3, c2, 3, 3}), bl.get("b3c1.b", {c3}), bl.get("b3ds.w", {c3, c2}), bl.get("b3ds.b", {c3}), 32, 16);
        put_c1ds("b4c1", bl.get("b4c1.w", {c4, c3, 3, 3}), bl.get("b4c1.b", {c4}), bl.get("b4ds.w", {c4, c3}), bl.get("b4ds.b", {c4}), 64, 32);
    }
    put_mfma("b3c2.wp", bl.get("b3c2.w", {c3, c3, 3, 3}), 32, 32, 1);
    ws.put("b3c2.bp", pad_bias(bl.get("b3c2.b", {c3}), 32, 32));
    put_mfma("b4c2.wp", bl.get("b4c2.w", {c4, c4, 3, 3}), 64, 64, 2);
    ws.put("b4c2.bp", pad_bias(bl.get("b4c2.b", {c4}), 64, 64));
    for (int i = 1; i <= 4; ++i) {
        char nm[16];
        snprintf(nm, 16, "agg%d.w", i);
        transpose(bl.get(nm, {dim / 4, ch[i]}), dim / 4, ch[i], tmp); ws.put(nm, tmp);
    }
    {
        const float* hw = bl.get("head.w", {dim + 1, dim});
        transpose(hw, 64, 64, tmp); ws.put("head.wT", tmp);
        ws.put_raw("head.ws", hw + 64 * 64, 64);
        float hmax = 0.0f;
        for (int o = 0; o < 64; ++o) for (int cc = 0; cc < 32; ++cc) hmax = std::max(hmax, std::fabs(hw[o * 64 + cc]));
        const float sh = weight_scale_h(&hmax, 1);
        net->k["head.inv_ws"] = 1.0f / sh;
        std::vector<uint16_t> hl(2 * 2 * 2 * 2 * 32 * 8);
        for (int kb = 0; kb < 2; ++kb) for (int nh = 0; nh < 2; ++nh) for (int hh = 0; hh < 2; ++hh) for (int n = 0; n < 32; ++n) for (int j = 0; j < 8; ++j) {
            const int cch = kb == 0 ? (j < 4 ? j : j + 4) + 4 * hh : 16 + 8 * hh + j;
            const float w = hw[(32 * nh + n) * 64 + cch] * sh;
            const _Float16 hi = (_Float16)w;
            const _Float16 lo = (_Float16)(w - (float)hi);
            const size_t at = ((((size_t)kb * 2 + nh) * 2 + hh) * 32 + n) * 8 + j;
            memcpy(&hl[at], &hi, 2);
            memcpy(&hl[2048 + at], &lo, 2);
        }
        tmp.assign(2048, 0.f);
        memcpy(tmp.data(), hl.data(), 8192);
        ws.put("head.wh16", tmp);
        {
            const float* a1w = bl.get("agg1.w", {dim / 4, c1});
            const float sa1 = weight_scale_h(a1w, 16 * 8);
            net->k["agg1.inv_wa"] = 1.0f / sa1;
            std::vector<uint16_t> fr(2 * 64 * 8, 0);
            for (int o = 0; o < 16; ++o) for (int c = 0; c < 8; ++c) {
                const float w = a1w[o * 8 + c] * sa1;
                const _Float16 hi = (_Float16)w;
                const _Float16 lo = (_Float16)(w - (float)hi);
                memcpy(&fr[(size_t)o * 8 + c], &hi, 2);
                memcpy(&fr[(size_t)(64 + o) * 8 + c], &lo, 2);
            }
            tmp.assign(512, 0.f);
            memcpy(tmp.data(), fr.data(), 2048);
            ws.put("agg1.h16", tmp);
        }
    }
    if (int rc = ws.upload(net)) { delete net; return rc; }
    *out = net;
    return KPB_OK;
}
```

keypoint_bench_amd/csrc/api.hip:

```cpp
#include "kpb_common.h"

char g_kpb_err[512] = {0};

extern "C" __attribute__((visibility("default"))) int kpb_version(void) { return KPB_VERSION; }

extern "C" __attribute__((visibility("default"))) const char* kpb_last_error(const kpb_ctx* ctx) { return ctx ? ctx->err : g_kpb_err; }

extern "C" __attribute__((visibility("default"))) int kpb_ctx_create(int device, void* stream, kpb_ctx** out)
{
    if (!out) return kpb_fail(nullptr, KPB_E_INVALID, "kpb_ctx_create: null out pointer");
    *out = nullptr;
    int count = 0;
    if (hipGetDeviceCount(&count) != hipSuccess || count == 0)
        return kpb_fail(nullptr, KPB_E_HIP, "kpb_ctx_create: no HIP device visible (this library has no CPU path)");
    if (device < 0 || device >= count)
        return kpb_fail(nullptr, KPB_E_INVALID, "kpb_ctx_create: device %d out of range (0..%d)", device, count - 1);
    hipDeviceProp_t prop;
    KPB_HIP(nullptr, hipGetDeviceProperties(&prop, device));
    if (strncmp(prop.gcnArchName, "gfx950", 6) != 0)
        return kpb_fail(nullptr, KPB_E_HIP, "kpb_ctx_create: device %d is %s; libkpb.so is built for gfx950 only", device,
                        prop.gcnArchName);
    KPB_HIP(nullptr, hipSetDevice(device));
    kpb_ctx* c = new kpb_ctx();
    c->device = device;
    c->stream = static_cast<hipStream_t>(stream);
    *out = c;
    return KPB_OK;
}

extern "C" __attribute__((visibility("default"))) void kpb_ctx_destroy(kpb_ctx* ctx)
{
    if (!ctx) return;
    (void)hipSetDevice(ctx->device);
    (void)hipStreamSynchronize(ctx->stream);
    for (kpb_buf* b : {&ctx->ws_nms_state, &ctx->ws_nms_map, &ctx->ws_nms_list, &ctx->ws_cand, &ctx->ws_match, &ctx->ws_misc, &ctx->ws_sel})
        if (b->p) (void)hipFree(b->p);
    if (ctx->wait_ev) (void)hipEventDestroy(ctx->wait_ev);
    if (ctx->host_det) (void)hipHostFree(ctx->host_det);
    if (ctx->host_match) (void)hipHostFree(ctx->host_match);
    if (ctx->own_stream) (void)hipStreamDestroy(ctx->stream);
    if (ctx->det_state && ctx->det_state_free) ctx->det_state_free(ctx->det_state);
    for (hipEvent_t e : ctx->prof_pool) (void)hipEventDestroy(e);
    delete ctx;
}

extern "C" __attribute__((visibility("default"))) int kpb_ctx_set_stream(kpb_ctx* ctx, void* stream)
{
    if (!ctx) return kpb_fail(nullptr, KPB_E_INVALID, "kpb_ctx_set_stream: null context");
    KPB_HIP(ctx, hipStreamSynchronize(ctx->stream));
    ctx->stream = static_cast<hipStream_t>(stream);
    return KPB_OK;
}

extern "C" __attribute__((visibility("default"))) int kpb_ctx_set_option(kpb_ctx* ctx, int option, int64_t value)
{
    if (!ctx) return kpb_fail(nullptr, KPB_E_INVALID, "kpb_ctx_set_option: null context");
    if (value < 0) return kpb_fail(ctx, KPB_E_INVALID, "kpb_ctx_set_option: negative value");
    switch (option) {
    case KPB_OPT_COVIS_STORE_BYTES: ctx->covis_store_bytes = (size_t)value; return KPB_OK;
    default: return kpb_fail(ctx, KPB_E_INVALID, "kpb_ctx_set_option: unknown option %d", option);
    }
}

extern "C" __attribute__((visibility("default"))) int kpb_sync(kpb_ctx* ctx)
{
    if (!ctx) return kpb_fail(nullptr, KPB_E_INVALID, "kpb_sync: null context");
    KPB_HIP(ctx, hipStreamSynchronize(ctx->stream));
    return KPB_OK;
}

extern "C" __attribute__((visibility("default"))) int kpb_prof_enable(kpb_ctx* ctx, int on)
{
    if (!ctx) return kpb_fail(nullptr, KPB_E_INVALID, "kpb_prof_enable: null context");
    ctx->prof = on != 0;
    return KPB_OK;
}

extern "C" __attribute__((visibility("default"))) int kpb_prof_report(kpb_ctx* ctx, char* buf, size_t cap)
{
    if (!ctx || !buf || cap == 0) return kpb_fail(ctx, KPB_E_INVALID, "kpb_prof_report: bad argument");
    KPB_HIP(ctx, hipStreamSynchronize(ctx->stream));
    std::vector<std::string> names;
    std::vector<double> ms;
    std::vector<long> calls;
    for (auto& r : ctx->prof_recs) {
        float t = 0.f;
        (void)hipEventElapsedTime(&t, r.e0, r.e1);
        size_t i = 0;
        for (; i < names.size(); ++i) if (names[i] == r.name) break;
        if (i == names.size()) { names.push_back(r.name); ms.push_back(0.0); calls.push_back(0); }
        ms[i] += t; calls[i] += 1;
        ctx->prof_pool.push_back(r.e0);
        ctx->prof_pool.push_back(r.e1);
    }
    ctx->prof_recs.clear();
    size_t off = 0;
    buf[0] = 0;
    for (size_t i = 0; i < names.size(); ++i) {
        int n = snprintf(buf + off, cap - off, "%s %ld %.6f\n", names[i].c_str(), calls[i], ms[i]);
        if (n < 0 || (size_t)n >= cap - off) break;
        off += (size_t)n;
    }
    return KPB_OK;
}
```

keypoint_bench_amd/csrc/kpb_common.h:

```cpp
#pragma once
#include <hip/hip_runtime.h>

#include <cstdarg>
#include <cstdint>
#include <cstdio>
#include <cstdlib>
#include <cstring>
#include <set>
#include <string>
#include <vector>
#include <type_traits>

#include "../../include/kpb.h"
#include <chrono>

__device__ __forceinline__ void kpb_halves32(float v, float& lo, float& hi)
{
    const auto r = __builtin_amdgcn_permlane32_swap(__float_as_uint(v), __float_as_uint(v), false, false);
    lo = __uint_as_float(r[0]);
    hi = __uint_as_float(r[1]);
}
struct kpb_tile3 { int x, y, z; };
__device__ __forceinline__ kpb_tile3 kpb_xcd_tile(int enable)
{
    const unsigned gx = gridDim.x, gy = gridDim.y, total = gx * gy * gridDim.z;
    unsigned L = blockIdx.x + gx * (blockIdx.y + gy * blockIdx.z);
    if (enable && (total & 7u) == 0u) L = (L & 7u) * (total >> 3) + (L >> 3);
    kpb_tile3 t;
    t.x = (int)(L % gx); t.y = (int)((L / gx) % gy); t.z = (int)(L / (gx * gy));
    return t;
}

__device__ __forceinline__ float kpb_pmax(float a, float b) { return __uint_as_float(max(__float_as_uint(a), __float_as_uint(b))); }
__device__ __forceinline__ float kpb_pmax32(float v) { float a, b; kpb_halves32(v, a, b); return kpb_pmax(a, b); }
__device__ __forceinline__ float kpb_sum16(float v)
{
    const auto r = __builtin_amdgcn_permlane16_swap(__float_as_uint(v), __float_as_uint(v), false, false);
    return __uint_as_float(r[0]) + __uint_as_float(r[1]);
}
__device__ __forceinline__ float kpb_xor1(float v) { return __int_as_float(__builtin_amdgcn_update_dpp(0, __float_as_int(v), 0xB1, 0xF, 0xF, true)); }
__device__ __forceinline__ float kpb_xor2(float v) { return __int_as_float(__builtin_amdgcn_update_dpp(0, __float_as_int(v), 0x4E, 0xF, 0xF, true)); }
template <int N>
__device__ __forceinline__ float kpb_shfl_xor(float v);
template <int N>
__device__ __forceinline__ int kpb_shfl_xor(int v) { return __float_as_int(kpb_shfl_xor<N>(__int_as_float(v))); }
template <int N>
__device__ __forceinline__ float kpb_shfl_xor(float v)
{
    static_assert(N == 1 || N == 2 || N == 4 || N == 8 || N == 16 || N == 32, "butterfly distances only");
    const int x = __float_as_int(v);
    if constexpr (N == 1) return __int_as_float(__builtin_amdgcn_update_dpp(x, x, 0xB1, 0xF, 0xF, false));
    else if constexpr (N == 2) return __int_as_float(__builtin_amdgcn_update_dpp(x, x, 0x4E, 0xF, 0xF, false));
    else if constexpr (N == 4) {
        const int t = __builtin_amdgcn_update_dpp(x, x, 0x104, 0xF, 0x5, false);
        return __int_as_float(__builtin_amdgcn_update_dpp(t, x, 0x114, 0xF, 0xA, false));
    } else if constexpr (N == 8) return __int_as_float(__builtin_amdgcn_update_dpp(x, x, 0x128, 0xF, 0xF, false));
    else if constexpr (N == 16) {
        const auto r = __builtin_amdgcn_permlane16_swap((unsigned)x, (unsigned)x, false, false);
        return __uint_as_float((__lane_id() & 16) ? r[0] : r[1]);
    } else {
        const auto r = __builtin_amdgcn_permlane32_swap((unsigned)x, (unsigned)x, false, false);
        return __uint_as_float((__lane_id() & 32) ? r[0] : r[1]);
    }
}
template <class F>
__device__ __forceinline__ void kpb_butterfly(F&& f)
{
    f(std::integral_constant<int, 32>{}); f(std::integral_constant<int, 16>{}); f(std::integral_constant<int, 8>{});
    f(std::integral_constant<int, 4>{}); f(std::integral_constant<int, 2>{}); f(std::integral_constant<int, 1>{});
}
__device__ __forceinline__ float kpb_wave_sum(float v)
{
    v += kpb_shfl_xor<32>(v); v += kpb_shfl_xor<16>(v); v += kpb_shfl_xor<8>(v);
    v += kpb_shfl_xor<4>(v); v += kpb_shfl_xor<2>(v); v += kpb_shfl_xor<1>(v);
    return v;
}
__device__ __forceinline__ float kpb_wave_fmax(float v)
{
    v = fmaxf(v, kpb_shfl_xor<32>(v)); v = fmaxf(v, kpb_shfl_xor<16>(v)); v = fmaxf(v, kpb_shfl_xor<8>(v));
    v = fmaxf(v, kpb_shfl_xor<4>(v)); v = fmaxf(v, kpb_shfl_xor<2>(v)); v = fmaxf(v, kpb_shfl_xor<1>(v));
    return v;
}
__device__ __forceinline__ float kpb_wave_fmin(float v)
{
    v = fminf(v, kpb_shfl_xor<32>(v)); v = fminf(v, kpb_shfl_xor<16>(v)); v = fminf(v, kpb_shfl_xor<8>(v));
    v = fminf(v, kpb_shfl_xor<4>(v)); v = fminf(v, kpb_shfl_xor<2>(v)); v = fminf(v, kpb_shfl_xor<1>(v));
    return v;
}
__device__ __forceinline__ int kpb_wave_incl_scan(int v)
{
    v += __builtin_amdgcn_update_dpp(0, v, 0x111, 0xF, 0xF, false);
    v += __builtin_amdgcn_update_dpp(0, v, 0x112, 0xF, 0xF, false);
    v += __builtin_amdgcn_update_dpp(0, v, 0x114, 0xF, 0xF, false);
    v += __builtin_amdgcn_update_dpp(0, v, 0x118, 0xF, 0xF, false);
    v += __builtin_amdgcn_update_dpp(0, v, 0x142, 0xA, 0xF, false);
    v += __builtin_amdgcn_update_dpp(0, v, 0x143, 0xC, 0xF, false);
    return v;
}
__device__ __forceinline__ float kpb_max32(float v) { float a, b; kpb_halves32(v, a, b); return fmaxf(a, b); }
__device__ __forceinline__ float kpb_min32(float v) { float a, b; kpb_halves32(v, a, b); return fminf(a, b); }
__device__ __forceinline__ float kpb_sum32(float v) { float a, b; kpb_halves32(v, a, b); return a + b; }

struct kpb_buf {
    void* p = nullptr;
    size_t cap = 0;
};

struct kpb_prof_rec {
    const char* name;
    hipEvent_t e0, e1;
};

struct kpb_ctx {
    int device = 0;
    bool prof = false;
    std::vector<kpb_prof_rec> prof_recs;
    std::vector<hipEvent_t> prof_pool;
    std::set<std::string> prof_names;
    hipStream_t stream = nullptr;
    bool own_stream = false;
    char err[512] = {0};
    kpb_buf ws_nms_state;
    kpb_buf ws_nms_map;
    kpb_buf ws_nms_list;
    kpb_buf ws_cand;
    kpb_buf ws_match;
    kpb_buf ws_misc;
    kpb_buf ws_sel;
    int* host_flags = nullptr;
    int* host_det = nullptr;
    int host_det_cap = 0;
    hipEvent_t wait_ev = nullptr;
    int* host_match = nullptr;
    int host_match_cap = 0, host_match_n = 0;
    void* det_state = nullptr;
    void (*det_state_free)(void*) = nullptr;
    int det_pending = 0;
    int det_counts_valid = 0, match_counts_valid = 0;
    unsigned lds_attr_done = 0;
    size_t covis_store_bytes = (size_t)4 << 30;
};
enum { KPB_ATTR_NMS = 1u, KPB_ATTR_HOMOGRAPHY = 2u, KPB_ATTR_ESSENTIAL = 4u, KPB_ATTR_FUNDAMENTAL = 8u };

extern char g_kpb_err[512];

inline int kpb_fail(kpb_ctx* ctx, int code, const char* fmt, ...)
{
    char* dst = ctx ? ctx->err : g_kpb_err;
    va_list ap;
    va_start(ap, fmt);
    vsnprintf(dst, 512, fmt, ap);
    va_end(ap);
    return code;
}

#define KPB_HIP(ctx, call)                                                                             \
    do {                                                                                               \
        hipError_t e_ = (call);                                                                        \
        if (e_ != hipSuccess)                                                                          \
            return kpb_fail(ctx, KPB_E_HIP, "%s failed: %s (%s:%d)", #call, hipGetErrorString(e_),     \
                            __FILE__, __LINE__);                                                       \
    } while (0)

inline hipError_t kpb_wait_stream(kpb_ctx* ctx, bool small)
{
    if (!small) return hipStreamSynchronize(ctx->stream);
    if (!ctx->wait_ev) {
        const hipError_t e = hipEventCreateWithFlags(&ctx->wait_ev, hipEventDisableTiming);
        if (e != hipSuccess) return e;
    }
    hipError_t e = hipEventRecord(ctx->wait_ev, ctx->stream);
    if (e != hipSuccess) return e;
    const auto t0 = std::chrono::steady_clock::now();
    while ((e = hipEventQuery(ctx->wait_ev)) == hipErrorNotReady)
        if (std::chrono::steady_clock::now() - t0 > std::chrono::milliseconds(5)) return hipStreamSynchronize(ctx->stream);
    return e;
}

inline int kpb_reserve(kpb_ctx* ctx, kpb_buf& b, size_t bytes)
{
    if (bytes <= b.cap) return KPB_OK;
    if (b.p) {
        (void)hipStreamSynchronize(ctx->stream);
        (void)hipFree(b.p);
        b.p = nullptr;
        b.cap = 0;
    }
    size_t want = bytes + bytes / 8;
    if (hipMalloc(&b.p, want) != hipSuccess) {
        b.p = nullptr;
        return kpb_fail(ctx, KPB_E_NOMEM, "workspace allocation of %zu bytes failed", want);
    }
    b.cap = want;
    static const bool log_alloc = getenv("KPB_LOG_ALLOC") && *getenv("KPB_LOG_ALLOC") == '1';
    if (log_alloc) fprintf(stderr, "kpb_alloc %p %zu\n", b.p, want);
    return KPB_OK;
}

static inline int cdiv(int a, int b) { return (a + b - 1) / b; }

static inline int kpb_env_int(const char* name, int dflt)
{
    const char* v = getenv(name);
    return (v && *v) ? atoi(v) : dflt;
}

struct ProfScope {
    kpb_ctx* ctx;
    hipEvent_t e1 = nullptr;
    ProfScope(kpb_ctx* c, const char* name) : ctx(c)
    {
        if (!c->prof) return;
        hipEvent_t ev[2];
        for (int i = 0; i < 2; ++i) {
            if (!c->prof_pool.empty()) { ev[i] = c->prof_pool.back(); c->prof_pool.pop_back(); }
            else if (hipEventCreate(&ev[i]) != hipSuccess) return;
        }
        c->prof_recs.push_back({c->prof_names.insert(name).first->c_str(), ev[0], ev[1]});
        e1 = ev[1];
        (void)hipEventRecord(ev[0], c->stream);
    }
    ~ProfScope() { if (e1) (void)hipEventRecord(e1, ctx->stream); }
};

#define KPB_LAUNCH(ctx_, name_, ...)            \
    do {                                        \
        ProfScope ps_(ctx_, name_);             \
        hipLaunchKernelGGL(__VA_ARGS__);        \
    } while (0)
```

Measured before the change: 15770.

## Recompute ALIKE block1 features inside the dense head instead of storing x1

When a descriptor map is requested with the f16 path, block1 no longer writes the full-resolution 8-channel x1 tensor. It stores only a per-tile exponent. The dense head kernel DMAs a raw image window per tile and recomputes the two block1 convolutions with MFMA in LDS. This trades the x1 write and re-read traffic for extra compute, more dynamic LDS, and lower occupancy (launch bounds drop from 3 to 2 waves per EU). An option restores the old in-memory behaviour, and desc_at now fails when x1 was not kept.

```diff
diff --git a/include/kpb.h b/include/kpb.h
--- a/include/kpb.h
+++ b/include/kpb.h
@@ -47,6 +47,7 @@
 int kpb_sync(kpb_ctx* ctx);
 
 #define KPB_OPT_COVIS_STORE_BYTES 1
+#define KPB_OPT_ALIKE_X1_IN_MEMORY 2
 int kpb_ctx_set_option(kpb_ctx* ctx, int option, int64_t value);
 
 int kpb_prof_enable(kpb_ctx* ctx, int on);
diff --git a/keypoint_bench_amd/_lib.py b/keypoint_bench_amd/_lib.py
--- a/keypoint_bench_amd/_lib.py
+++ b/keypoint_bench_amd/_lib.py
@@ -152,6 +152,7 @@
         self.check(self.lib.kpb_sync(self.handle))
 
     OPT_COVIS_STORE_BYTES = 1
+    OPT_ALIKE_X1_IN_MEMORY = 2
 
     def set_option(self, option: int, value: int):
         self.check(self.lib.kpb_ctx_set_option(self.handle, int(option), int(value)))
diff --git a/keypoint_bench_amd/csrc/alike.hip b/keypoint_bench_amd/csrc/alike.hip
--- a/keypoint_bench_amd/csrc/alike.hip
+++ b/keypoint_bench_amd/csrc/alike.hip
@@ -178,9 +178,88 @@
     float l1_c1, bmax_c1;
     float* wmax_x1;
     int xcd_map;
+    int* eimg;
 };
 
 constexpr int B1H_TH = 16;
+
+struct B1hScales { float un1, sc_mid, un2; };
+
+__device__ __forceinline__ B1hScales b1h_scales(int e_img, float inv_ws1, float inv_ws2, float l1_c1, float bmax_c1)
+{
+    const int e_mid = cm_exp_of(fmaf(__uint_as_float((unsigned)(e_img - 126 + 127) << 23), l1_c1, bmax_c1));
+    return {inv_ws1 * cm_unscale_of(e_img), cm_scale_of(e_mid), inv_ws2 * cm_unscale_of(e_mid)};
+}
+
+__device__ __forceinline__ void b1h_split_px(float c0, float c1, float c2, float sc, uint2& hi, uint2& lo)
+{
+    split4(make_float4(c0 * sc, c1 * sc, c2 * sc, 0.0f), hi, lo);
+}
+
+__device__ __forceinline__ void b1h_conv1_row(const uint4* inq, uint2* midh, int at0, int at1, int lo0, int lo1, int h8, int hlo,
+                                              const h8v (&c1hi)[2], const h8v (&c1lo)[2], float unm, const float4 bm, bool yin)
+{
+    f32x4v acc = {0.f, 0.f, 0.f, 0.f};
+    const h8v i0h = __builtin_bit_cast(h8v, inq[at0]), i0l = __builtin_bit_cast(h8v, inq[at0 + lo0]);
+    const h8v i1h = __builtin_bit_cast(h8v, inq[at1]), i1l = __builtin_bit_cast(h8v, inq[at1 + lo1]);
+    acc = __builtin_amdgcn_mfma_f32_16x16x32_f16(c1hi[0], i0l, acc, 0, 0, 0);
+    acc = __builtin_amdgcn_mfma_f32_16x16x32_f16(c1lo[0], i0h, acc, 0, 0, 0);
+    acc = __builtin_amdgcn_mfma_f32_16x16x32_f16(c1hi[0], i0h, acc, 0, 0, 0);
+    acc = __builtin_amdgcn_mfma_f32_16x16x32_f16(c1hi[1], i1l, acc, 0, 0, 0);
+    acc = __builtin_amdgcn_mfma_f32_16x16x32_f16(c1lo[1], i1h, acc, 0, 0, 0);
+    acc = __builtin_amdgcn_mfma_f32_16x16x32_f16(c1hi[1], i1h, acc, 0, 0, 0);
+    float4 v = make_float4(0.f, 0.f, 0.f, 0.f);
+    if (yin) v = make_float4(relu(fmaf(acc[0], unm, bm.x)), relu(fmaf(acc[1], unm, bm.y)), relu(fmaf(acc[2], unm, bm.z)), relu(fmaf(acc[3], unm, bm.w)));
+    uint2 hi, lo;
+    split4(v, hi, lo);
+    midh[h8] = hi;
+    midh[h8 + hlo] = lo;
+}
+
+template <int MH, int IW, int NIN, int HW, int PLANE, int REGION>
+__device__ __forceinline__ void b1h_conv1_pair16(const uint4* inq, uint2* midh, int y, int g, int sN, bool inside,
+                                                 const h8v (&c1hi)[2], const h8v (&c1lo)[2], float un1, const float4 bias1, float sc_mid)
+{
+    constexpr int pc = 16;
+    const int my = min(y, MH - 1);
+    f32x4v acc = {0.f, 0.f, 0.f, 0.f};
+#pragma unroll
+    for (int kb = 0; kb < 2; ++kb) {
+        const int piece = 4 * kb + g;
+        const int at = piece < 6 ? ((my + (piece >> 1)) * IW + 2 * pc + 2 * (piece & 1)) >> 1 : NIN;
+        const h8v ihi = __builtin_bit_cast(h8v, inq[at]);
+        const h8v ilo = __builtin_bit_cast(h8v, inq[piece < 6 ? at + NIN / 2 : NIN]);
+        acc = __builtin_amdgcn_mfma_f32_16x16x32_f16(c1hi[kb], ilo, acc, 0, 0, 0);
+        acc = __builtin_amdgcn_mfma_f32_16x16x32_f16(c1lo[kb], ihi, acc, 0, 0, 0);
+        acc = __builtin_amdgcn_mfma_f32_16x16x32_f16(c1hi[kb], ihi, acc, 0, 0, 0);
+    }
+    float4 v = make_float4(relu(fmaf(acc[0], un1, bias1.x)) * sc_mid, relu(fmaf(acc[1], un1, bias1.y)) * sc_mid,
+                           relu(fmaf(acc[2], un1, bias1.z)) * sc_mid, relu(fmaf(acc[3], un1, bias1.w)) * sc_mid);
+    if (!inside) v = make_float4(0.f, 0.f, 0.f, 0.f);
+    uint2 hi, lo;
+    split4(v, hi, lo);
+    if (y < MH) {
+        const int h8 = ((sN * PLANE + y * HW + pc) << 1) + (g & 1);
+        midh[h8] = hi;
+        midh[h8 + 2 * REGION] = lo;
+    }
+}
+
+__device__ __forceinline__ float4 b1h_conv2_row(const uint4* mid, int at, int HW, int REGION, const h8v (&bhi)[3], const h8v (&blo)[3], float un2, const float4 bias2)
+{
+    f32x4v acc = {0.f, 0.f, 0.f, 0.f};
+#pragma unroll
+    for (int kb = 0; kb < 3; ++kb) {
+        const h8v ihi = __builtin_bit_cast(h8v, mid[at + kb * HW]);
+        const h8v ilo = __builtin_bit_cast(h8v, mid[REGION + at + kb * HW]);
+        acc = __builtin_amdgcn_mfma_f32_16x16x32_f16(bhi[kb], ilo, acc, 0, 0, 0);
+        acc = __builtin_amdgcn_mfma_f32_16x16x32_f16(blo[kb], ihi, acc, 0, 0, 0);
+        acc = __builtin_amdgcn_mfma_f32_16x16x32_f16(bhi[kb], ihi, acc, 0, 0, 0);
+    }
+    return make_float4(relu(fmaf(acc[0], un2, bias2.x)), relu(fmaf(acc[1], un2, bias2.y)), relu(fmaf(acc[2], un2, bias2.z)), relu(fmaf(acc[3], un2, bias2.w)));
+}
+
+template <bool STORE_X1>
 
 __global__ __launch_bounds__(256) void alike_block1_h(Block1HArgs ha)
 {
@@ -245,14 +324,15 @@
         for (int k = 0; k < PER; ++k) {
             const int i = tid + k * 256;
             uint2 hi, lo;
-            split4(make_float4(buf[k][0] * sc, buf[k][1] * sc, buf[k][2] * sc, 0.0f), hi, lo);
+            b1h_split_px(buf[k][0], buf[k][1], buf[k][2], sc, hi, lo);
             if (i < NIN) { inh[i] = hi; inh[NIN + i] = lo; }
         }
         if (tid < 2) inh[2 * NIN + tid] = make_uint2(0u, 0u);
     }
     __syncthreads();
-    const int e_mid = cm_exp_of(fmaf(__uint_as_float((unsigned)(e_img - 126 + 127) << 23), ha.l1_c1, ha.bmax_c1));
-    const float un1 = ha.inv_ws1 * cm_unscale_of(e_img), sc_mid = cm_scale_of(e_mid), un2 = ha.inv_ws2 * cm_unscale_of(e_mid);
+    const B1hScales scl = b1h_scales(e_img, ha.inv_ws1, ha.inv_ws2, ha.l1_c1, ha.bmax_c1);
+    const float un1 = scl.un1, sc_mid = scl.sc_mid, un2 = scl.un2;
+    if constexpr (!STORE_X1) { if (tid == 0) ha.eimg[(b * gridDim.y + tile.y) * gridDim.x + tile.x] = e_img; }
     const int pr = lane & 15, g = lane >> 4;
     const int sN = g >> 1, c0 = 4 * (g & 1);
     {
@@ -271,52 +351,15 @@
             int h8 = ((sN * PLANE + wv * HW + pr) << 1) + (g & 1);
 #pragma unroll 1
             for (int y = wv; y < MH; y += 4, at0 += 4 * (IW / 2), at1 += st1, h8 += 8 * HW) {
-                f32x4v acc = {0.f, 0.f, 0.f, 0.f};
-                const h8v i0h = __builtin_bit_cast(h8v, inq[at0]), i0l = __builtin_bit_cast(h8v, inq[at0 + NIN / 2]);
-                const h8v i1h = __builtin_bit_cast(h8v, inq[at1]), i1l = __builtin_bit_cast(h8v, inq[at1 + lo1]);
-                acc = __builtin_amdgcn_mfma_f32_16x16x32_f16(c1hi[0], i0l, acc, 0, 0, 0);
-                acc = __builtin_amdgcn_mfma_f32_16x16x32_f16(c1lo[0], i0h, acc, 0, 0, 0);
-                acc = __builtin_amdgcn_mfma_f32_16x16x32_f16(c1hi[0], i0h, acc, 0, 0, 0);
-                acc = __builtin_amdgcn_mfma_f32_16x16x32_f16(c1hi[1], i1l, acc, 0, 0, 0);
-                acc = __builtin_amdgcn_mfma_f32_16x16x32_f16(c1lo[1], i1h, acc, 0, 0, 0);
-                acc = __builtin_amdgcn_mfma_f32_16x16x32_f16(c1hi[1], i1h, acc, 0, 0, 0);
                 const bool yin = (unsigned)(ty0 - 1 + y) < (unsigned)a.H;
-                float4 v = make_float4(0.f, 0.f, 0.f, 0.f);
-                if (yin) v = make_float4(relu(fmaf(acc[0], unm, bm.x)), relu(fmaf(acc[1], unm, bm.y)), relu(fmaf(acc[2], unm, bm.z)), relu(fmaf(acc[3], unm, bm.w)));
-                uint2 hi, lo;
-                split4(v, hi, lo);
-                midh[h8] = hi;
-                midh[h8 + 2 * REGION] = lo;
+                b1h_conv1_row(inq, midh, at0, at1, NIN / 2, lo1, h8, 2 * REGION, c1hi, c1lo, unm, bm, yin);
             }
         }
         if (wv >= 2) {
-            const int gi = MH + wv - 2;
-            const bool extra = true;
-            const int y = extra ? 16 * (gi - MH) + pr : gi, pc = extra ? 16 : pr;
-            const int my = min(y, MH - 1);
-            f32x4v acc = {0.f, 0.f, 0.f, 0.f};
-#pragma unroll
-            for (int kb = 0; kb < 2; ++kb) {
-                const int piece = 4 * kb + g;
-                const int at = piece < 6 ? ((my + (piece >> 1)) * IW + 2 * pc + 2 * (piece & 1)) >> 1 : NIN;
-                const h8v ihi = __builtin_bit_cast(h8v, inq[at]);
-                const h8v ilo = __builtin_bit_cast(h8v, inq[piece < 6 ? at + NIN / 2 : NIN]);
-                acc = __builtin_amdgcn_mfma_f32_16x16x32_f16(c1hi[kb], ilo, acc, 0, 0, 0);
-                acc = __builtin_amdgcn_mfma_f32_16x16x32_f16(c1lo[kb], ihi, acc, 0, 0, 0);
-                acc = __builtin_amdgcn_mfma_f32_16x16x32_f16(c1hi[kb], ihi, acc, 0, 0, 0);
-            }
-            const int gy = ty0 - 1 + y, gx = tx0 - 1 + 2 * pc + sN;
+            const int y = 16 * (wv - 2) + pr;
+            const int gy = ty0 - 1 + y, gx = tx0 - 1 + 2 * 16 + sN;
             const bool inside = gy >= 0 && gy < a.H && gx >= 0 && gx < a.W;
-            float4 v = make_float4(relu(fmaf(acc[0], un1, bias1.x)) * sc_mid, relu(fmaf(acc[1], un1, bias1.y)) * sc_mid,
-                                   relu(fmaf(acc[2], un1, bias1.z)) * sc_mid, relu(fmaf(acc[3], un1, bias1.w)) * sc_mid);
-            if (!inside) v = make_float4(0.f, 0.f, 0.f, 0.f);
-            uint2 hi, lo;
-            split4(v, hi, lo);
-            if (y < MH) {
-                const int h8 = ((sN * PLANE + y * HW + pc) << 1) + (g & 1);
-                midh[h8] = hi;
-                midh[h8 + 2 * REGION] = lo;
-            }
+            b1h_conv1_pair16<MH, IW, NIN, HW, PLANE, REGION>(inq, midh, y, g, sN, inside, c1hi, c1lo, un1, bias1, sc_mid);
         }
     }
     __syncthreads();
@@ -328,20 +371,10 @@
 #pragma unroll 1
     for (int rr = 0; rr < TH / 4; ++rr) {
         const int row = (TH / 4) * wv + rr;
-        f32x4v acc = {0.f, 0.f, 0.f, 0.f};
-#pragma unroll
-        for (int kb = 0; kb < 3; ++kb) {
-            const int at = abase + (row + kb) * HW;
-            const h8v ihi = __builtin_bit_cast(h8v, mid[at]);
-            const h8v ilo = __builtin_bit_cast(h8v, mid[REGION + at]);
-            acc = __builtin_amdgcn_mfma_f32_16x16x32_f16(bhi[kb], ilo, acc, 0, 0, 0);
-            acc = __builtin_amdgcn_mfma_f32_16x16x32_f16(blo[kb], ihi, acc, 0, 0, 0);
-            acc = __builtin_amdgcn_mfma_f32_16x16x32_f16(bhi[kb], ihi, acc, 0, 0, 0);
-        }
         const int gy = ty0 + row;
-        const float4 v = make_float4(relu(fmaf(acc[0], un2, bias2.x)), relu(fmaf(acc[1], un2, bias2.y)), relu(fmaf(acc[2], un2, bias2.z)), relu(fmaf(acc[3], un2, bias2.w)));
+        const float4 v = b1h_conv2_row(mid, abase + row * HW, HW, REGION, bhi, blo, un2, bias2);
         if (gy < a.H && gx < a.W) {
-            {
+            if constexpr (STORE_X1) {
                 typedef float f4v __attribute__((ext_vector_type(4)));
                 __builtin_nontemporal_store((f4v){v.x, v.y, v.z, v.w}, reinterpret_cast<f4v*>(a.x1 + ((size_t)b * P + (size_t)gy * a.W + gx) * 8 + c0));
             }
@@ -962,6 +995,10 @@
     float ws_h, inv_ws_h;
     const uint4* a1h16;
     float inv_wa;
+    const float* img = nullptr;
+    const int* eimg = nullptr;
+    const uint4* w1pk = nullptr; const uint4* w2pk = nullptr; const float* b1b = nullptr; const float* b2b = nullptr;
+    float inv_ws1 = 0.f, inv_ws2 = 0.f, l1_c1 = 0.f, bmax_c1 = 0.f;
 };
 
 constexpr int SEG_TILES = 4;
@@ -1167,6 +1204,14 @@
                      : "=&s"(keep) : "s"(m0v), "v"(gsrc) : "memory");
 }
 
+__device__ __forceinline__ void hp_dma4(const void* gsrc, const void* lds_wave_base)
+{
+    const unsigned m0v = __builtin_amdgcn_readfirstlane((unsigned)reinterpret_cast<uintptr_t>(lds_wave_base));
+    unsigned keep;
+    asm volatile("s_mov_b32 %0, m0\n\ts_mov_b32 m0, %1\n\ts_nop 0\n\tglobal_load_lds_dword %2, off\n\ts_mov_b32 m0, %0"
+                 : "=&s"(keep) : "s"(m0v), "v"(gsrc) : "memory");
+}
+
 __device__ __forceinline__ void hp_dma16s(const void* sbase, unsigned voff_bytes, const void* lds_wave_base)
 {
     const unsigned m0v = __builtin_amdgcn_readfirstlane((unsigned)reinterpret_cast<uintptr_t>(lds_wave_base));
@@ -1194,7 +1239,15 @@
 #define KPB_STAMP(i) do { } while (0)
 #endif
 
-__global__ __launch_bounds__(256, 3) void alike_head_f16p(HybArgs a, const uint4* __restrict__ wh16, int groups_per_wg)
+constexpr int HX_IH = 5, HX_IW = B1_TW + 4, HX_NIN = HX_IH * HX_IW, HX_MH = 3, HX_HW = (B1_TW + 2) / 2, HX_PLANE = HX_MH * HX_HW, HX_REGION = 2 * HX_PLANE;
+constexpr int HX_INQ = (2 * HX_NIN + 2) / 2;
+constexpr int HX_WAVE = HX_INQ + 2 * HX_REGION;
+constexpr int HX_FRAG = (2 + 3) * 2 * 64;
+static_assert(HX_NIN % 2 == 0 && HX_NIN <= 3 * 64 && HX_INQ >= 64, "alike_head_f16p: three window positions per lane; the x1 slot fits the window");
+inline size_t hp_dyn_bytes(bool x1mem) { return (size_t)(x1mem ? 4 * 2 * 64 : HX_FRAG + 4 * HX_WAVE) * 16; }
+
+template <bool X1MEM>
+__global__ __launch_bounds__(256, X1MEM ? 3 : 2) void alike_head_f16p(HybArgs a, const uint4* __restrict__ wh16, int groups_per_wg)
 {
     __shared__ __attribute__((aligned(16))) uint4 Bh[2][256];
     __shared__ __attribute__((aligned(16))) uint4 A1h[2][64];
@@ -1202,8 +1255,12 @@
     __shared__ __attribute__((aligned(16))) float4 A2r[HP_A2R * HP_A2S];
     __shared__ __attribute__((aligned(16))) float E3r[HP_ER][HP_NT3 * ESTRIDE];
     __shared__ __attribute__((aligned(16))) float E4r[HP_ER][HP_NT4 * ESTRIDE];
-    __shared__ __attribute__((aligned(16))) float4 X1r[4][2][64];
+    extern __shared__ __attribute__((aligned(16))) uint4 hp_dyn[];
     const int tid = threadIdx.x, lane = tid & 63, wv = __builtin_amdgcn_readfirstlane(tid >> 6);
+    uint4* const wmid = hp_dyn + wv * 2 * HX_REGION;
+    uint4* const wscr = hp_dyn + (X1MEM ? wv * 2 * 64 : 4 * 2 * HX_REGION + wv * HX_INQ);
+    uint4* const wfrag = hp_dyn + 4 * HX_WAVE;
+    float4* const X1w = reinterpret_cast<float4*>(wscr);
     const int p = lane & 31, h = lane >> 5;
     const int b = blockIdx.y;
     const int ef = cm_exp_of(fmaxf(__uint_as_float(a.amax_x1[b]) * a.l1_agg1, __uint_as_float(a.amax_a2[b])));
@@ -1280,12 +1337,37 @@
     float* pend_d = nullptr;
     auto fetch = [&](int y, int t, int slot) {
         const size_t pix = (size_t)b * a.H * a.W + (size_t)y * a.W + (xs + 32 * t + p);
-        hp_dma16<true>(a.x1 + pix * 8 + 4 * h, &X1r[wv][slot][0]);
+        hp_dma16<true>(a.x1 + pix * 8 + 4 * h, X1w + 64 * slot);
     };
+    float* const raw = reinterpret_cast<float*>(wmid);
+    static_assert((3 * 192 + 64) * 4 <= 2 * HX_REGION * 16, "alike_head_f16p: the raw window fits the intermediate rows");
+    const float* img = a.img + (size_t)b * 3 * a.H * a.W;
+    auto prefetch = [&](int y, int t) {
+        const int x0 = xs + 32 * t;
+        hp_dma4(a.eimg + ui((b * (a.H / B1H_TH) + (y / B1H_TH)) * tiles_per_row + (x0 >> 5)), raw + 3 * 192);
+#pragma unroll
+        for (int k = 0; k < 3; ++k) {
+            const int i = lane + 64 * k;
+            const int wy = i / HX_IW, wx = i - wy * HX_IW;
+            const int gy = y - 2 + wy, gx = x0 - 2 + wx;
+            const size_t at = (size_t)min(max(gy, 0), a.H - 1) * a.W + min(max(gx, 0), a.W - 1);
+#pragma unroll
+            for (int c = 0; c < 3; ++c) hp_dma4(img + (size_t)c * a.H * a.W + at, raw + c * 192 + 64 * k);
+        }
+    };
+    float4 bias1 = make_float4(0.f, 0.f, 0.f, 0.f), bias2 = bias1;
+    if constexpr (!X1MEM) {
+        for (int i = tid; i < HX_FRAG; i += 256) wfrag[i] = i < 2 * 2 * 64 ? a.w1pk[i] : a.w2pk[i - 2 * 2 * 64];
+        bias1 = *reinterpret_cast<const float4*>(a.b1b + 4 * ((lane >> 4) & 1));
+        bias2 = *reinterpret_cast<const float4*>(a.b2b + 4 * ((lane >> 4) & 1));
+    }
     if (g0 < g1) {
-        fetch(4 * g0 + wv, 0, 0);
-        if (ntile == 2) fetch(4 * g0 + wv, 1, 1);
-        else if (g0 + 1 < g1) fetch(4 * (g0 + 1) + wv, 0, 1);
+        if constexpr (X1MEM) {
+            fetch(4 * g0 + wv, 0, 0);
+            if (ntile == 2) fetch(4 * g0 + wv, 1, 1);
+            else if (g0 + 1 < g1) fetch(4 * (g0 + 1) + wv, 0, 1);
+        } else
+            prefetch(4 * g0 + wv, 0);
     }
     for (int G = g0; G < min(g0 + HP_LA, g1); ++G) request(G);
     int ktile = 0;
@@ -1312,16 +1394,83 @@
         for (int s = 0; s < 2; ++s) { const int kk = 2 * s + h; w4t[t][s] = kk == t4 ? 1.0f - lx4t[t] : (kk == t4 + 1 ? lx4t[t] : 0.0f); }
     }
     int xso = xs;
-    auto body = [&](auto first_tag, const int y, const int t, const int ny, const int nt) {
+    auto body = [&](auto first_tag, const int y, const int t, const int ny, const int nt, const int n1y, const int n1t) {
         constexpr bool FIRST = decltype(first_tag)::value;
         const int x0 = xso + 32 * t, x = x0 + p;
         const size_t pix = (size_t)b * a.H * a.W + (size_t)y * a.W + x;
-        if (ktile < 3) asm volatile("s_waitcnt vmcnt(0)" ::: "memory"); else asm volatile("s_waitcnt vmcnt(63)" ::: "memory");
+        if (ktile < 3) asm volatile("s_waitcnt vmcnt(0)" ::: "memory");
+        else if constexpr (X1MEM) asm volatile("s_waitcnt vmcnt(63)" ::: "memory");
+        else asm volatile("s_waitcnt vmcnt(32)" ::: "memory");
         KPB_STAMP(4 + 8 * t);
         const int slot = ktile & 1;
-        const float4 x1lo = X1r[wv][slot][p], x1hi = X1r[wv][slot][32 + p];
-        asm volatile("s_waitcnt lgkmcnt(0)" ::: "memory");
-        if (ny >= 0) fetch(ny, nt, slot);
+        float4 x1lo, x1hi;
+        if constexpr (X1MEM) {
+            x1lo = X1w[64 * slot + p]; x1hi = X1w[64 * slot + 32 + p];
+            asm volatile("s_waitcnt lgkmcnt(0)" ::: "memory");
+            if (ny >= 0) fetch(ny, nt, slot);
+        } else {
+            uint2* const inh = reinterpret_cast<uint2*>(wscr);
+            const uint4* const inq = wscr;
+            uint4* const mid = wmid;
+            uint2* const midh = reinterpret_cast<uint2*>(mid);
+            int zf = 0;
+            asm volatile("" : "+v"(zf));
+            const uint4* const frag = wfrag + zf;
+            h8v c1hi[2], c1lo[2], bhi[3], blo[3];
+#pragma unroll
+            for (int kb = 0; kb < 2; ++kb) {
+                c1hi[kb] = __builtin_bit_cast(h8v, frag[(kb * 2 + 0) * 64 + lane]);
+                c1lo[kb] = __builtin_bit_cast(h8v, frag[(kb * 2 + 1) * 64 + lane]);
+            }
+            const int e_img = ui(reinterpret_cast<const int*>(raw)[3 * 192 + lane]);
+            const float sc = cm_scale_of(e_img);
+#pragma unroll
+            for (int k = 0; k < 3; ++k) {
+                const int i = lane + 64 * k;
+                const int wy = i / HX_IW, wx = i - wy * HX_IW;
+                const int gy = y - 2 + wy, gx = x0 - 2 + wx;
+                const bool ok = i < HX_NIN && gy >= 0 && gy < a.H && gx >= 0 && gx < a.W;
+                const float r0 = raw[i], r1 = raw[192 + i], r2 = raw[2 * 192 + i];
+                uint2 hi, lo;
+                b1h_split_px(ok ? r0 : 0.0f, ok ? r1 : 0.0f, ok ? r2 : 0.0f, sc, hi, lo);
+                if (i < HX_NIN) { inh[i] = hi; inh[HX_NIN + i] = lo; }
+            }
+            if (lane < 2) inh[2 * HX_NIN + lane] = make_uint2(0u, 0u);
+            asm volatile("s_waitcnt lgkmcnt(0)" ::: "memory");
+            const B1hScales scl = b1h_scales(e_img, a.inv_ws1, a.inv_ws2, a.l1_c1, a.bmax_c1);
+            const int pr = lane & 15, g = lane >> 4, sN = g >> 1;
+            {
+                const int gxl = x0 - 1 + 2 * pr + sN;
+                const bool xin = gxl >= 0 && gxl < a.W;
+                const float unm = xin ? scl.un1 * scl.sc_mid : 0.0f;
+                const float4 bm = xin ? make_float4(bias1.x * scl.sc_mid, bias1.y * scl.sc_mid, bias1.z * scl.sc_mid, bias1.w * scl.sc_mid) : make_float4(0.f, 0.f, 0.f, 0.f);
+                const bool has1 = g < 2;
+                const int lo1 = has1 ? HX_NIN / 2 : 0;
+#pragma unroll
+                for (int r = 0; r < HX_MH; ++r) {
+                    const int at0 = (r + (g >> 1)) * (HX_IW / 2) + pr + (g & 1);
+                    const int at1 = has1 ? (r + 2) * (HX_IW / 2) + pr + g : HX_NIN;
+                    const int h8 = ((sN * HX_PLANE + r * HX_HW + pr) << 1) + (g & 1);
+                    const bool yin = (unsigned)(y - 1 + r) < (unsigned)a.H;
+                    b1h_conv1_row(inq, midh, at0, at1, HX_NIN / 2, lo1, h8, 2 * HX_REGION, c1hi, c1lo, unm, bm, yin);
+                }
+                const int gy = y - 1 + pr, gx = x0 - 1 + 2 * 16 + sN;
+                const bool inside = gy >= 0 && gy < a.H && gx >= 0 && gx < a.W;
+                b1h_conv1_pair16<HX_MH, HX_IW, HX_NIN, HX_HW, HX_PLANE, HX_REGION>(inq, midh, pr, g, sN, inside, c1hi, c1lo, scl.un1, bias1, scl.sc_mid);
+            }
+            asm volatile("s_waitcnt lgkmcnt(0)" ::: "memory");
+#pragma unroll
+            for (int kb = 0; kb < 3; ++kb) {
+                bhi[kb] = __builtin_bit_cast(h8v, frag[(4 + kb * 2 + 0) * 64 + lane]);
+                blo[kb] = __builtin_bit_cast(h8v, frag[(4 + kb * 2 + 1) * 64 + lane]);
+            }
+            const float4 v = b1h_conv2_row(mid, (g & 1) * HX_PLANE + pr + (g >> 1), HX_HW, HX_REGION, bhi, blo, scl.un2, bias2);
+            X1w[(g & 1) * 32 + 2 * pr + sN] = v;
+            asm volatile("s_waitcnt lgkmcnt(0)" ::: "memory");
+            x1lo = X1w[p]; x1hi = X1w[32 + p];
+            asm volatile("s_waitcnt lgkmcnt(0)" ::: "memory");
+            if (n1y >= 0) prefetch(n1y, n1t);
+        }
         ++ktile;
         KPB_STAMP(5 + 8 * t);
         Up8Taps taps;
@@ -1477,13 +1626,13 @@
         asm volatile("" : "+s"(xso));
         if (ntile == 2) {
             const int ny = g + 1 < g1 ? y + 4 : -1;
-            if (g == g0) body(std::true_type{}, y, 0, ny, 0);
-            else body(std::false_type{}, y, 0, ny, 0);
-            body(std::false_type{}, y, 1, ny, 1);
+            if (g == g0) body(std::true_type{}, y, 0, ny, 0, y, 1);
+            else body(std::false_type{}, y, 0, ny, 0, y, 1);
+            body(std::false_type{}, y, 1, ny, 1, ny, 0);
         } else {
-            const int ny = g + 2 < g1 ? y + 8 : -1;
-            if (g == g0) body(std::true_type{}, y, 0, ny, 0);
-            else body(std::false_type{}, y, 0, ny, 0);
+            const int ny = g + 2 < g1 ? y + 8 : -1, n1y = g + 1 < g1 ? y + 4 : -1;
+            if (g == g0) body(std::true_type{}, y, 0, ny, 0, n1y, 0);
+            else body(std::false_type{}, y, 0, ny, 0, n1y, 0);
         }
         KPB_STAMP(20);
     }
@@ -1708,17 +1857,20 @@
     const int H = H_, W = W_;
     const size_t P = (size_t)H * W, B = batch;
     const bool h16 = conv_mfma_use_h16();
-    const size_t n_x1 = B * P * 8, n_2 = B * (P / 4) * 16, n_3 = B * (P / 64) * 32, n_a3 = B * (P / 64) * 16,
+    const bool x1mem = !(h16 && desc_out_dev) || ctx->alike_x1_in_memory;
+    const size_t n_eimg = x1mem ? 0 : (B * (size_t)(H / B1H_TH) * (W / B1_TW) + 63) / 64 * 64;
+    const size_t n_x1 = x1mem ? B * P * 8 : 0, n_2 = B * (P / 4) * 16, n_3 = B * (P / 64) * 32, n_a3 = B * (P / 64) * 16,
                  n_4 = B * (P / 1024) * 64, n_a4 = B * (P / 1024) * 16;
     const size_t n_s = B * (P / 4 + P / 64 + P / 1024) + 64;
     const size_t n_e = desc_out_dev ? B * (P / 64 + P / 1024) * ESTRIDE : 0;
     const size_t n_p1 = B * (P / 4) * 8;
     const int nw1 = cdiv(W, B1_TW) * cdiv(H, B1H_TH) * 4, nw2 = cdiv(W / 2, 32) * cdiv(H / 2, 8) * 4;
     const size_t n_rng = (2 * B + B * (nw1 + nw2) + 63) / 64 * 64;
-    const size_t total = n_x1 + n_p1 + 3 * n_2 + 6 * n_3 + n_a3 + 5 * n_4 + n_4 / 2 + n_a4 + n_s + n_e + n_rng;
+    const size_t total = n_x1 + n_p1 + 3 * n_2 + 6 * n_3 + n_a3 + 5 * n_4 + n_4 / 2 + n_a4 + n_s + n_e + n_rng + n_eimg;
     if (int rc = kpb_reserve(ctx, act, total * sizeof(float))) return rc;
     float* p = static_cast<float*>(act.p);
-    x1 = p; p += n_x1;
+    x1 = x1mem ? p : nullptr; p += n_x1;
+    int* eimg = reinterpret_cast<int*>(p); p += n_eimg;
     p1 = p; p += n_p1;
     t2 = p; p += n_2; x2 = p; p += n_2; a2 = p; p += n_2;
     t3 = p; p += n_3; x3 = p; p += n_3; a3 = p; p += n_a3;
@@ -1744,8 +1896,9 @@
     ConvArgs c;
     if (h16) {
         Block1HArgs hb{b1, reinterpret_cast<const uint4*>(wp("b1c1.pairs")), reinterpret_cast<const uint4*>(wp("b1c2.pairs")),
-                       k.at("b1c1.inv_ws"), k.at("b1c2.inv_ws"), k.at("b1c1.l1"), k.at("b1c1.bmax"), wmax_x1, 0};
-        KPB_LAUNCH(ctx, "alike_block1", alike_block1_h, dim3(cdiv(W, B1_TW), cdiv(H, B1H_TH), batch), dim3(256), 0, st, hb);
+                       k.at("b1c1.inv_ws"), k.at("b1c2.inv_ws"), k.at("b1c1.l1"), k.at("b1c1.bmax"), wmax_x1, 0, eimg};
+        if (x1mem) KPB_LAUNCH(ctx, "alike_block1", alike_block1_h<true>, dim3(cdiv(W, B1_TW), cdiv(H, B1H_TH), batch), dim3(256), 0, st, hb);
+        else KPB_LAUNCH(ctx, "alike_block1", alike_block1_h<false>, dim3(cdiv(W, B1_TW), cdiv(H, B1H_TH), batch), dim3(256), 0, st, hb);
         KPB_LAUNCH(ctx, "amax_reduce", amax_reduce, dim3(batch), dim3(256), 0, st, wmax_x1, nw1, amax_x1);
         Block2Args b2{p1, x2, a2, S2, p2, reinterpret_cast<const uint4*>(wp("b2c1.h16")), reinterpret_cast<const uint4*>(wp("b2c2.h16")),
                       reinterpret_cast<const uint4*>(wp("agg2.h16")), wp("b2c1.b"), wp("b2c2.bsum"), wp("head.ws") + 16, H / 2, W / 2,
@@ -1814,8 +1967,17 @@
                 return kpb_fail(ctx, KPB_E_UNSUPPORTED, "alike head: the LDS rings cannot hold the source rows of %d row groups at height %d", HP_LA + 1, H);
             const int bands_ = cdiv(W / 32, HP_TILES), groups_ = H / 4;
             const int hp = std::max(2, std::min(30, (int)(((long long)bands_ * groups_ * batch) / 1536)));
-            KPB_LAUNCH(ctx, "alike_head_dense", alike_head_f16p, dim3(cdiv(W / 32, HP_TILES) * cdiv(H / 4, hp), batch), dim3(256), 0, st, hy,
-                       reinterpret_cast<const uint4*>(wp("head.wh16")), hp);
+            const dim3 grid(cdiv(W / 32, HP_TILES) * cdiv(H / 4, hp), batch);
+            const uint4* wh16 = reinterpret_cast<const uint4*>(wp("head.wh16"));
+            if (x1mem)
+                KPB_LAUNCH(ctx, "alike_head_dense", alike_head_f16p<true>, grid, dim3(256), hp_dyn_bytes(true), st, hy, wh16, hp);
+            else {
+                hy.img = img_dev; hy.eimg = eimg; hy.w1pk = reinterpret_cast<const uint4*>(wp("b1c1.pairs")); hy.w2pk = reinterpret_cast<const uint4*>(wp("b1c2.pairs"));
+                hy.b1b = wp("b1c1.b"); hy.b2b = wp("b1c2.b");
+                hy.inv_ws1 = k.at("b1c1.inv_ws"); hy.inv_ws2 = k.at("b1c2.inv_ws"); hy.l1_c1 = k.at("b1c1.l1"); hy.bmax_c1 = k.at("b1c1.bmax");
+                KPB_HIP(ctx, hipFuncSetAttribute(reinterpret_cast<const void*>(alike_head_f16p<false>), hipFuncAttributeMaxDynamicSharedMemorySize, (int)hp_dyn_bytes(false)));
+                KPB_LAUNCH(ctx, "alike_head_dense", alike_head_f16p<false>, grid, dim3(256), hp_dyn_bytes(false), st, hy, wh16, hp);
+            }
         } else
             KPB_LAUNCH(ctx, "alike_head_dense", alike_head_hyb, dim3(work4, batch), dim3(256), 0, st, hy);
     } else {
@@ -1831,6 +1993,8 @@
 int AlikeNet::desc_at(const float* pts_dev, int pts_cols, int max_n, const int32_t* n_dev, float* out_dev)
 {
     if (B == 0) return kpb_fail(ctx, KPB_E_INVALID, "kpb_net_desc_at: no forward has run");
+    if (!x1) return kpb_fail(ctx, KPB_E_INVALID, "kpb_net_desc_at: the last forward filled a descriptor map and kept no x1; set KPB_OPT_ALIKE_X1_IN_MEMORY to 1 "
+                                                   "(kpb_ctx_set_option) to have both, or sample the map");
     const int kpw = (long long)B * max_n >= 32768 ? 8 : 1;
     DescAtArgs a{head_args(nullptr, nullptr), pts_dev, n_dev, out_dev, pts_cols, max_n, kpw};
     KPB_LAUNCH(ctx, "alike_desc_at", alike_desc_at, dim3(cdiv(max_n, 4 * kpw), B), dim3(256), 0, ctx->stream, a);
diff --git a/keypoint_bench_amd/csrc/api.hip b/keypoint_bench_amd/csrc/api.hip
--- a/keypoint_bench_amd/csrc/api.hip
+++ b/keypoint_bench_amd/csrc/api.hip
@@ -58,6 +58,7 @@
     if (value < 0) return kpb_fail(ctx, KPB_E_INVALID, "kpb_ctx_set_option: negative value");
     switch (option) {
     case KPB_OPT_COVIS_STORE_BYTES: ctx->covis_store_bytes = (size_t)value; return KPB_OK;
+    case KPB_OPT_ALIKE_X1_IN_MEMORY: ctx->alike_x1_in_memory = value != 0; return KPB_OK;
     default: return kpb_fail(ctx, KPB_E_INVALID, "kpb_ctx_set_option: unknown option %d", option);
     }
 }
diff --git a/keypoint_bench_amd/csrc/kpb_common.h b/keypoint_bench_amd/csrc/kpb_common.h
--- a/keypoint_bench_amd/csrc/kpb_common.h
+++ b/keypoint_bench_amd/csrc/kpb_common.h
@@ -139,6 +139,7 @@
     int det_counts_valid = 0, match_counts_valid = 0;
     unsigned lds_attr_done = 0;
     size_t covis_store_bytes = (size_t)4 << 30;
+    bool alike_x1_in_memory = false;
 };
 enum { KPB_ATTR_NMS = 1u, KPB_ATTR_HOMOGRAPHY = 2u, KPB_ATTR_ESSENTIAL = 4u, KPB_ATTR_FUNDAMENTAL = 8u };
 
```

After: 13000. 17.5% lower.
